# vpc-ccg/circminer

Measured on AMD Instinct MI355X. Metric: paired reads/sec (whole node), hg38 k=20, 2x150 bp; circ_report bit-exact, higher is better.
Workload: dtype int32/u8 (chain scores f64)

## Files before the change

### circminer_amd/csrc/cm_core.h

```cpp
#pragma once
#include <stdint.h>

#include "circminer_hot.h"
#if defined(CM_STAGE2_HOST)
#include <vector>
#endif

#if defined(__HIPCC__)
#define CM_HD __host__ __device__
#define CM_NOINLINE inline
#else
#define CM_HD
#define CM_NOINLINE
#endif

#if !defined(CM_HOOK_DP)
#define CM_HOOK_DP(kind, s, n, t, m) ((void)0)
#endif
#if defined(CM_STATS) && !defined(__HIPCC__)
#if !defined(CM_NSTATS)
#define CM_NSTATS 16
#endif
extern "C" unsigned long long cm_stats[CM_NSTATS];
#define CM_STAT(i, n) ((i) < CM_NSTATS ? (void)(cm_stats[(i) < CM_NSTATS ? (i) : 0] += (unsigned long long)(n)) : (void)0)
// ... 310 lines not shown
        beg = (int)A.iv_bucket[b];
        end = (int)A.iv_bucket[b + 1];
        if (beg > 0) --beg;
        if (end < (int)A.n_iv) ++end;
        if (end <= beg) end = beg + 1;
    }
    while (end - beg > 1) {
        const int mid = (beg + end) / 2;
        if (pos < A.iv[mid].spos) end = mid;
        else beg = mid;
    }
    ind = end - 1;
    if (ind < 0 || A.iv[ind].epos < pos) return -1;
    return ind;
}
CM_HD inline int overlap_ind(const Core &c, uint32_t loc, int &ind) {
    int r = iv_find_ind(c.A, loc, ind);
    if (r < 0 || iv_nseg(c.A, r) == 0) return -1;
    return r;
}
CM_HD inline int overlap(const Core &c, uint32_t loc) { int ind; return overlap_ind(c, loc, ind); }

CM_HD inline uint32_t upper_bound_lookup(const Core &c, uint32_t spos, uint32_t mlen, uint32_t rlen, uint32_t &max_end, int &ol) {
    const AnnotV &A = c.A;
    max_end = 0;
    int it_ind = -1;
    int ov = iv_find_ind(A, spos, it_ind);
    const uint32_t epos = spos + mlen - 1;
    if (ov < 0 || iv_nseg(A, ov) == 0) {
        ol = -1;
        int nx = it_ind + 1;
        max_end = ((nx < 0 || nx >= (int)A.n_iv) ? 0u : A.iv[nx].spos) - 1u;
        if (max_end < epos) return 0;
        return cmin(spos + rlen + (uint32_t)c.P.max_ed, max_end - mlen + 1);
    }
    ol = -1;
    uint32_t min_end = 1000000000u, max_next = 0;
    if (epos > A.iv[ov].epos) {
        const uint32_t n = iv_nseg(A, ov);
        for (uint32_t i = 0; i < n; ++i) {
            uint32_t s = iv_segid(A, ov, i);
            uint32_t e = A.seg[s].end;
            if (e >= epos) {
                max_end = cmax(max_end, e);
                min_end = cmin(min_end, e);
                max_next = cmax(max_next, A.seg[s].next_exon_beg);
            }
        }
    } else {
        max_end = A.iv[ov].max_end;
        min_end = A.iv[ov].min_end;
        max_next = A.iv[ov].max_next_exon;
    }
    if (max_end > 0 && max_end >= epos) {
        ol = ov;
        if (min_end < rlen + epos && max_next != 0) return max_next + mlen - 1;
        return max_end - mlen + 1;
    }
    max_end = 0;
    ol = -1;
    return 0;
}
CM_HD inline uint32_t upper_bound(const Core &c, uint32_t spos, uint32_t mlen, uint32_t rlen, uint32_t &max_end, int &ol) {
    if (bit_at(c.A.near_border_bits, c.A.n_bits, spos)) return upper_bound_lookup(c, spos, mlen, rlen, max_end, ol);
    max_end = 0;
    ol = -1;
    return spos + rlen + (uint32_t)c.P.max_ed;
}
CM_HD inline int chr_row(const Core &c, uint32_t loc) {
    uint32_t i;
    for (i = 1; i < c.A.n_chr; ++i)
        if (loc < c.A.chr_shift[i]) return (int)i - 1;
    return (int)i - 1;
}

struct Event { double score; uint32_t cell; uint32_t pad; };
struct ChainWork {
    CM_G double *dp_score;
    CM_G int32_t *dp_prev;
    CM_G uint8_t *pool;
    unsigned long long pool_bytes;
    CM_G unsigned long long *pool_cursor;
    g_err err;
};

#if defined(__HIP_DEVICE_COMPILE__)
CM_HD inline unsigned long long pool_take(CM_G unsigned long long *cur, unsigned long long n) { return atomicAdd((unsigned long long *)cur, n); }
CM_HD inline void flag_err(g_err e, int bits) { atomicOr((int *)e, bits); }
#else
inline unsigned long long pool_take(unsigned long long *cur, unsigned long long n) { return __sync_fetch_and_add(cur, n); }
inline void flag_err(int *e, int bits) { __sync_fetch_and_or(e, bits); }
#endif

CM_HD inline bool check_junction(const Core &c, uint32_t s1, uint32_t s2, int ol, int kmer, int read_dist, int &trans_dist) {
    trans_dist = INF_I;
    if (ol < 0) return false;
    const uint32_t e1 = s1 + kmer - 1;
    if (s2 <= e1) return false;
    int td2intron = -1;
    const AnnotV &A = c.A;
    const uint32_t n = iv_nseg(A, ol);
    for (uint32_t i = 0; i < n; ++i) {
        const uint32_t s = iv_segid(A, ol, i);
        const int e12end = (int)(A.seg[s].end - e1);
        const int beg2s2 = (int)(s2 - A.seg[s].next_exon_beg);
        if (e12end >= 0 && e12end < read_dist && beg2s2 + kmer < 0) td2intron = (int)(s2 - e1 - 1);
        if (e12end < 0 || beg2s2 < 0) continue;
        trans_dist = e12end + beg2s2;
        if (cabs(trans_dist - read_dist) <= c.P.max_ed) return true;
    }
    if (td2intron != -1) {
        trans_dist = td2intron;
        return true;
    }
    trans_dist = INF_I;
    return false;
}

constexpr int SMALL_W = 32;
struct ChainStoreGlobal {
    ChainWork &w;
    g_u32 POS;
    const uint32_t *start;
    const uint32_t *cnt_;
    const uint32_t *base_;
    uint32_t lb_[MAX_SEEDS];
    CM_G Event *ev;
    uint32_t n_ev, cap_ev;
    bool lost;
    static constexpr uint32_t MASK_CELLS = 128;
    uint64_t imp0_, imp1_;
    bool masked_;
    double init_;
    CM_HD ChainStoreGlobal(ChainWork &ww, g_u32 pos, const uint32_t *st, const uint32_t *cn, const uint32_t *bs)
        : w(ww), POS(pos), start(st), cnt_(cn), base_(bs), ev(nullptr), n_ev(0), cap_ev(0), lost(false), imp0_(0), imp1_(0), masked_(false), init_(0) {}
    CM_HD inline bool stored(uint32_t x) const { return !masked_ || (((x < 64u ? imp0_ : imp1_) >> (x & 63u)) & 1ull); }
    CM_HD inline uint32_t cnt(int s) const { return cnt_[s]; }
    CM_HD inline uint32_t base(int s) const { return base_[s]; }
    CM_HD inline uint32_t total(int kc) const { return base_[kc]; }
    CM_HD inline void lb_reset(int kc) { for (int k = 0; k < kc; ++k) lb_[k] = 0; }
    CM_HD inline uint32_t lb(int s) const { return lb_[s]; }
    CM_HD inline void set_lb(int s, uint32_t v) { lb_[s] = v; }
    CM_HD inline void init(uint32_t n_cells, double v) {
        masked_ = n_cells <= MASK_CELLS;
        init_ = v;
        imp0_ = imp1_ = 0;
        if (masked_) return;
        for (uint32_t x = 0; x < n_cells; ++x) {
            w.dp_score[x] = v;
            w.dp_prev[x] = -1;
        }
    }
    CM_HD inline uint32_t pos(int s, uint32_t i) const { return POS[start[s] + i]; }
    CM_HD inline double score(uint32_t x) const { return stored(x) ? w.dp_score[x] : init_; }
    CM_HD inline int32_t prev(uint32_t x) const { return stored(x) ? w.dp_prev[x] : -1; }
    CM_HD inline void set(uint32_t x, double sc, int32_t pv) {
        w.dp_score[x] = sc;
        w.dp_prev[x] = pv;
        if (masked_) {
            if (x < 64u) imp0_ |= 1ull << x;
            else imp1_ |= 1ull << (x & 63u);
        }
    }
    CM_HD inline void push(double sc, uint32_t cell) {
        if (n_ev == cap_ev && !lost) {
            const uint32_t ncap = cap_ev ? cap_ev * 4u : 32u;
            const unsigned long long bytes = (unsigned long long)ncap * sizeof(Event);
            const unsigned long long off = pool_take(w.pool_cursor, bytes);
            if (off + bytes > w.pool_bytes) {
                lost = true;
                flag_err(w.err, ERR_POOL);
            } else {
                CM_G Event *ne = (CM_G Event *)(w.pool + off);
                for (uint32_t q = 0; q < n_ev; ++q) ne[q] = ev[q];
                ev = ne;
                cap_ev = ncap;
            }
        }
        if (n_ev < cap_ev) {
            ev[n_ev].score = sc;
            ev[n_ev].cell = cell;
            ++n_ev;
        }
    }
    CM_HD inline uint32_t n_events() const { return n_ev; }
    CM_HD inline double ev_score(uint32_t q) const { return ev[q].score; }
    CM_HD inline uint32_t ev_cell(uint32_t q) const { return ev[q].cell; }
};
struct ChainStoreSmall {
    double sc[SMALL_W + 2];
    int32_t pv[SMALL_W + 2];
    uint32_t hp[SMALL_W + 2];
    double es[SMALL_W];
    uint32_t ec[SMALL_W];
    const uint32_t *cnt_;
    const uint32_t *base_;
    uint32_t lb_[MAX_SEEDS];
    uint32_t n_ev;
    CM_HD ChainStoreSmall(g_u32 POS, const uint32_t *start, const uint32_t *cn, const uint32_t *bs, int kc) : cnt_(cn), base_(bs), n_ev(0) {
        for (int s = 0; s < kc; ++s)
            for (uint32_t i = 0; i < cn[s]; ++i) hp[bs[s] + i] = POS[start[s] + i];
    }
    CM_HD inline uint32_t cnt(int s) const { return cnt_[s]; }
    CM_HD inline uint32_t base(int s) const { return base_[s]; }
    CM_HD inline uint32_t total(int kc) const { return base_[kc]; }
    CM_HD inline void lb_reset(int kc) { for (int k = 0; k < kc; ++k) lb_[k] = 0; }
    CM_HD inline uint32_t lb(int s) const { return lb_[s]; }
    CM_HD inline void set_lb(int s, uint32_t v) { lb_[s] = v; }
    CM_HD inline void init(uint32_t n_cells, double v) {
        for (uint32_t x = 0; x < n_cells; ++x) {
            sc[x] = v;
            pv[x] = -1;
        }
    }
    CM_HD inline uint32_t pos(int s, uint32_t i) const { return hp[base_[s] + i]; }
    CM_HD inline double score(uint32_t x) const { return sc[x]; }
    CM_HD inline int32_t prev(uint32_t x) const { return pv[x]; }
    CM_HD inline void set(uint32_t x, double v, int32_t p) {
        sc[x] = v;
        pv[x] = p;
    }
    CM_HD inline void push(double v, uint32_t cell) {
        if (n_ev < (uint32_t)SMALL_W) {
            es[n_ev] = v;
            ec[n_ev] = cell;
            ++n_ev;
        }
    }
    CM_HD inline uint32_t n_events() const { return n_ev; }
    CM_HD inline double ev_score(uint32_t q) const { return es[q]; }
    CM_HD inline uint32_t ev_cell(uint32_t q) const { return ec[q]; }
};

template <class ST>
CM_HD inline int chain_kbest_t(const Core &c, int seq_len, int kc, ST &S, CM_G cm_chain *out) {
    const int kmer = c.P.kmer;
    const uint32_t max_best = (uint32_t)c.P.max_chain_len;
    S.init(S.total(kc), (double)kmer);
    uint32_t max_exon_end = 0;
    int ol = -1;

    for (int ii = kc - 2; ii >= 0; --ii) {
        const uint32_t read_remain = (uint32_t)(seq_len - ii * kmer - kmer);
        S.lb_reset(kc);
        const uint32_t cnt_ii = S.cnt(ii), base_ii = S.base(ii);
        for (uint32_t i = 0; i < cnt_ii; ++i) {
            const int32_t cur_info = (int32_t)S.pos(ii, i);
            const uint32_t seg_start = (uint32_t)cur_info, seg_end = (uint32_t)cur_info + kmer - 1;
            uint32_t max_lpos_lim = MAXUB;
            double my_score = S.score(base_ii + i);
            for (int jj = ii + 1; jj < kc; ++jj) {
                const uint32_t pcn = S.cnt(jj);
                uint32_t lb = S.lb(jj);
                if (pcn == 0 || lb >= pcn) continue;
// ... 1957 lines not shown
```

### circminer_amd/csrc/cm_heavy_pipe.h

```cpp

struct HPair {
    cm_mapped_read mr;
    uint32_t t;
    uint32_t task_off, unp_off;
    uint32_t fp, bp, fun, bun;
    int32_t ntask, exf, exb;
    int32_t min_ret1, min_ret2;
    int16_t len1, len2, nf, nb, nfu, nbu;
    int8_t st, first, over, a, g1, g2, gf, gb, do_f, do_b, pad[2];
};
struct HTask { uint32_t h, e; };
struct HUnp { uint32_t h, x; };
enum { HC_TASKS = 0, HC_Q1 = 1, HC_Q1CUR = 2, HC_UNP = 3, HC_Q2 = 4, HC_Q2CUR = 5, HC_LIST2 = 6, HC_FALL = 7, HC_CUR = 8 , HC_WORDS = 16 };
struct HPipe {
    HPair *hp;
    uint32_t *list2, *fall;
    HTask *T;
    cmc::PreDP *pre;
    uint32_t *q;
    HRes *res;
    HUnp *U;
    cmc::PreDP *pre2;
    uint32_t *q2;
    unsigned int *ctr;
// ... 425 lines not shown
        hp.do_f = do_f ? 1 : 0;
        hp.do_b = do_b ? 1 : 0;
        hp.fun = fun;
        hp.bun = bun;
        hp.nfu = (int16_t)nfu;
        hp.nbu = (int16_t)nbu;
        hp.unp_off = off;
        hp.exf = 99;
        hp.exb = 99;
        hp.gf = 0;
        hp.gb = 0;
    }
}

__global__ void __launch_bounds__(BLK_PAIR, 8) k_hp_unp_req(KCore kc, ReadsDev rd, uint64_t pair0, int attempt, const cm_chain *chains, HPipe P, int str_cap) {
    const int lane = threadIdx.x;
    const Core c = cmc::to_core(kc);
    cmc::DpMem sm{cmc::LBuf{nullptr, str_cap}, cmc::LBuf{nullptr, str_cap}, nullptr};
    const cmc::Ext ext(c, sm);
    const int kmer = c.P.kmer;
    const unsigned int n_unp = P.ctr[HC_UNP] < P.unp_cap ? P.ctr[HC_UNP] : P.unp_cap;
    const unsigned int n_req = 2u * n_unp;
    auto take = [&]() { return (unsigned int)__shfl((int)(lane == 0 ? atomicAdd(&P.ctr[HC_CUR + 2], 64u) : 0u), 0); };
    for (unsigned int r0 = take(); r0 < n_req; r0 = take()) {
        const unsigned int r = r0 + (unsigned int)lane;
        cmc::SV sv{}, tv{};
        int n = 0, m = 0;
        bool have = false, in_range = false;
        if (r < n_req) {
            const HUnp u = P.U[r >> 1];
            if (u.h != 0xffffffffu) {
                in_range = true;
                const HPair &hp = P.hp[u.h];
                const HReadsOf R = hp_reads(rd, pair0, hp.t, (attempt == 0) == (hp.first != 0));
                const bool back = (u.x >> 8) & 1u;
                const int ci = (int)(u.x & 0xFFu);
                const cmc::g_chain chp = (cmc::g_chain)(chains + (uint64_t)(back ? R.bset : R.fset) * CM_BESTCHAINLIM) + ci;
                const cmc::Read rdv{back ? R.bseq : R.fseq, back ? R.blen : R.flen, back ? 1 : 0};
                have = hp_side_views(ext, chp, rdv, (r & 1u) != 0u, kmer, sv, n, tv, m);
            }
        }
        hp_answer_or_queue(sm, in_range, have, sv, n, tv, m, P.pre2 + r, r, P.q2, &P.ctr[HC_Q2], lane);
    }
}
__global__ void __launch_bounds__(BLK_PAIR, CM_PAIR_WAVES) k_hp_unp(KCore kc, ReadsDev rd, uint64_t pair0, int attempt, const cm_chain *chains, HPipe P,
                                                                     uint32_t *pair_err, int str_cap) {
    extern __shared__ uint32_t lds_words[];
    const int lane = threadIdx.x;
    cmc::DpMem sm = lane_dp_mem((CM_S uint8_t *)lds_words, lane, str_cap, nullptr);
    const Core c = cmc::to_core(kc);
    const cmc::Ext ext(c, sm);
    const int kmer = c.P.kmer;
    const unsigned int n_unp = P.ctr[HC_UNP] < P.unp_cap ? P.ctr[HC_UNP] : P.unp_cap;
    auto take = [&]() { return (unsigned int)__shfl((int)(lane == 0 ? atomicAdd(&P.ctr[HC_CUR + 3], 64u) : 0u), 0); };
    for (unsigned int x0 = take(); x0 < n_unp; x0 = take()) {
        const unsigned int x = x0 + (unsigned int)lane;
        if (x >= n_unp) continue;
        const HUnp u = P.U[x];
        if (u.h == 0xffffffffu) continue;
        HPair &hp = P.hp[u.h];
        const HReadsOf R = hp_reads(rd, pair0, hp.t, (attempt == 0) == (hp.first != 0));
        const bool back = (u.x >> 8) & 1u;
        const int ci = (int)(u.x & 0xFFu), k = (int)(u.x >> 16);
        const cmc::CH ch{(cmc::g_chain)(chains + (uint64_t)(back ? R.bset : R.fset) * CM_BESTCHAINLIM) + ci, kmer};
        const cmc::Read frd{R.fseq, R.flen, 0}, brd{R.bseq, R.blen, 1};
        cmc::MM m = cmc::mm_init(c);
        sm.err = (cmc::g_err)(pair_err + hp.t);
        sm.pre = (cmc::g_pre)(P.pre2 + (size_t)x * 2);
        sm.n_pre = 2;
        const int ex = ext.chain_both_sides(ch, back ? brd : frd, m, back ? -1 : 1);
        sm.pre = nullptr;
        sm.n_pre = 0;
        atomicMin(back ? &hp.exb : &hp.exf, ex);
        if (k == 0) {
            cmc::overlap_to_spos(c, m);
            cmc::overlap_to_epos(c, m);
            (back ? hp.gb : hp.gf) = (int8_t)((m.exons_spos >= 0) || (m.exons_epos >= 0));
        }
    }
}

__global__ void __launch_bounds__(BLK_PAIR, 8) k_hp_finish(KCore kc, uint64_t pair0, const uint32_t *lst, const unsigned int *n_lst_p, const unsigned int *n_heavy_p,
                                                          int attempt, HPipe P, cm_mapped_read *state, uint8_t *active, int32_t *cat, int is_last,
                                                          unsigned long long *counters, RetryArgs ra, const int32_t *nchain, int second_to_fall) {
    const Core c = cmc::to_core(kc);
    const unsigned int n_items = attempt == 0 ? *n_heavy_p : *n_lst_p;
    const unsigned int x = blockIdx.x * BLK_PAIR + threadIdx.x;
#if defined(CM_HP_DIAG)
    if (x == 0) {
        unsigned long long *o = counters + CN_HP_ATTEMPT + CN_HP_STRIDE * attempt;
        atomicAdd(&o[0], (unsigned long long)n_items);
        atomicAdd(&o[1], (unsigned long long)P.ctr[HC_TASKS]);
        atomicAdd(&o[2], (unsigned long long)P.ctr[HC_UNP]);
        atomicAdd(&o[3], (unsigned long long)P.ctr[HC_Q1]);
        atomicAdd(&o[4], (unsigned long long)P.ctr[HC_Q2]);
        atomicAdd(&o[5], (unsigned long long)*P.fall_ctr);
    }
#endif
    for (unsigned int y = x; y < n_items; y += gridDim.x * BLK_PAIR) {
        const uint32_t h = attempt == 0 ? y : lst[y];
        HPair &hp = P.hp[h];
        if (hp.over) {
            active[pair0 + hp.t] = 1;
            continue;
        }
        cm_mapped_read mr = hp.mr;
        int st = hp.st;
        if (st < 0) {
            int a = hp.a;
            if (a < 0) {
                int min_ret1 = hp.min_ret1, min_ret2 = hp.min_ret2, g1 = hp.g1, g2 = hp.g2;
                if (hp.do_f) {
                    min_ret1 = hp.exf < min_ret1 ? hp.exf : min_ret1;
                    g1 = hp.gf;
                }
                if (hp.do_b) {
                    min_ret2 = hp.exb < min_ret2 ? hp.exb : min_ret2;
                    g2 = hp.gb;
                }
                cmc::mr_update_type(mr, cmc::leftover_type(min_ret1, min_ret2, g1 != 0, g2 != 0));
                a = mr.type;
            }
            if (c.P.scan_level == 0 && a == CM_CONCRD) st = CM_CONCRD;
            if (st < 0 && attempt == 0) {
                const bool r1_fwd2 = hp.first == 0;
                const uint32_t fs = hp.t * 4u + (r1_fwd2 ? 0u : 2u), bs = hp.t * 4u + (r1_fwd2 ? 3u : 1u);
                if (nchain[fs] == 0 && nchain[bs] == 0) {
                    const bool decided = mr.type == CM_CONCRD || mr.type == CM_DISCRD || mr.type == CM_CHIORF || mr.type == CM_CHIBSJ || mr.type == CM_CHI2BSJ;
                    if (!decided && cmc::leftovers_matter(mr.type, CM_ORPHAN, false, CM_ORPHAN, false))
                        cmc::mr_update_type(mr, cmc::leftover_type(CM_ORPHAN, CM_ORPHAN, false, false));
                    st = (c.P.scan_level == 0 && mr.type == CM_CONCRD) ? CM_CONCRD : mr.type;
                } else if (second_to_fall) {
                    P.fall[atomicAdd(P.fall_ctr, 1u)] = hp.t;
                    hp_count_fall(counters, 0);
                    active[pair0 + hp.t] = 1;
                    continue;
                } else {
                    hp.mr = mr;
                    P.list2[atomicAdd(&P.ctr[HC_LIST2], 1u)] = h;
                    continue;
                }
            }
            if (st < 0) st = mr.type;
        }
        const uint32_t t = hp.t;
        const uint64_t p = pair0 + t;
        if (__hip_atomic_load(ra.pair_err + t, __ATOMIC_RELAXED, __HIP_MEMORY_SCOPE_AGENT) != 0u) {
            ra.list[atomicAdd(ra.count, 1u)] = t;
            active[p] = 1;
        } else {
            uint8_t act = 1;
            cmc::finish_round(c, st, is_last, hp.len1, hp.len2, mr, act);
            state[p] = mr;
            active[p] = act;
            cat[p] = st;
            atomicAdd(&counters[CN_PAIR_ROUNDS], 1ull);
        }
    }
}
__global__ void k_hp_reset(unsigned int *ctr) {
    if (threadIdx.x < HC_WORDS && threadIdx.x != HC_LIST2 && threadIdx.x != HC_FALL) ctr[threadIdx.x] = 0u;
}
```

### circminer_amd/csrc/cm_hot.hip

```cpp
#include <chrono>
#include <hip/hip_runtime.h>
#include <rocprim/device/device_radix_sort.hpp>

#include <algorithm>
#include <atomic>
#include <cstdarg>
#include <cstdio>
#include <cstdlib>
#include <cstring>
#include <string>
#include <functional>
#include <thread>
#include <vector>

#include "circminer_hot.h"
#include "cm_core.h"
#include "cm_aos.h"
#include "cm_index_build.h"
#include "cm_fastq_text.h"
#include "cm_pam_text.h"
#include "cm_remain_order.h"
#include "cm_remain_text.h"
#include "cm_sam_text.h"

using cmc::Core;
using cmc::KCore;

namespace {

constexpr int MAX_SLOTS = 16;
constexpr uint32_t TILE_PAIRS = 1u << 20;
constexpr uint32_t TILE_PAIRS_MAX = 1u << 21;
constexpr int BLK = 256;
constexpr int BLK_CHAIN = 64;
#include "cm_dp_engine.h"

enum ProfClass { PC_NONE = -1, PC_SEED = 0, PC_CHAIN = 1, PC_PAIR = 2, PC_SCAN = 3, PC_HEAVY = 4, PC_ORDER = 5, PC_CHAIN_HEAVY = 6, PC_PREFETCH = 7,
                 PC_ROWS = 7 , PC_COUNT = 8 };
enum Counter {
    CN_PROBES = 0 , CN_PAIR_ROUNDS = 3, CN_RERUN = 4 ,
    CN_FALL = 5, CN_FALL_2ND = 6,
    CN_DEAD_CHAINS = 7,
    CN_CD_LANE = 8, CN_CD_PHASE = 13, CN_CD_WAVE = 16, CN_CD_EVENTS = 20, CN_CD_LEVELS = 21, CN_CD_PROBLEMS = 22, CN_CD_PASSES = 23, CN_CD_CELLS = 24,
    CN_CD_REGLOG = 25, CN_CD_BATCHES = 26, CN_CD_PRE_USED = 27, CN_CD_PRE_UNUSED = 28,
    CN_HP_ATTEMPT = 8, CN_HP_STRIDE = 8, CN_HP_UNPAIRED = 24, CN_HP_CHAINS = 25, CN_HP_SEQ_TASKS = 26, CN_HP_EARLY = 27, CN_HP_EARLY_FIRST = 28,
    CN_WORDS = 32
};
static_assert(CN_CD_CELLS < CN_WORDS && CN_HP_EARLY_FIRST < CN_WORDS && CN_HP_ATTEMPT + CN_HP_STRIDE + 5 < CN_HP_UNPAIRED, "d_counters has CN_WORDS words");
enum Pin {
    PIN_COLLECT_N = 0, PIN_COLLECT_ERR = 1,
    PIN_DEV_ERR = 0,
    PIN_POOL_ERR = 2,
    PIN_HEAVY_LOAD = 4,
    PIN_CELLS = 8,
    PIN_RERUN_N = 12, PIN_FALL_N = 14,
    PIN_TEXT = 16,
    PIN_ROWS = 26,
    PIN_TIES = 28,
    PIN_WORDS = 32
};
constexpr size_t PIN_BYTES = PIN_WORDS * sizeof(unsigned long long);
static_assert(PIN_BYTES == 256 && PIN_FALL_N + 1 < PIN_TEXT && PIN_CELLS + 3 < PIN_RERUN_N && PIN_TEXT + cmft::RES_WORDS <= PIN_ROWS && PIN_ROWS + 1 < PIN_TIES && PIN_TIES + 1 < PIN_WORDS,
              "the landing zone has 32 words");
struct ReadsDev {
    const uint8_t *seq1, *seq2;
    const uint64_t *off1, *off2;
};

__global__ void __launch_bounds__(BLK) k_seed(KCore kc, ReadsDev rd, const uint8_t *active, uint64_t pair0, uint32_t n_tile, int S,
                                              uint32_t *sstart, uint32_t *scnt, uint32_t *sraw, unsigned long long *counters) {
    const Core c = cmc::to_core(kc);
    __shared__ unsigned int sh[3];
    if (threadIdx.x < 3) sh[threadIdx.x] = 0;
    __syncthreads();
    const uint64_t q = (uint64_t)blockIdx.x * BLK + threadIdx.x;
    const uint64_t total = (uint64_t)n_tile * 4u * (uint64_t)S;
    const bool in = q < total;
    const uint64_t qc = in ? q : total - 1;
    uint32_t s;
    uint64_t r;
    if ((total >> 32) == 0) {
        s = (uint32_t)qc % (uint32_t)S;
        r = (uint32_t)qc / (uint32_t)S;
    } else {
        s = (uint32_t)(qc % (uint64_t)S);
        r = qc / (uint64_t)S;
    }
    const int orient = (int)(r & 1u), mate = (int)((r >> 1) & 1u);
    const uint64_t p = pair0 + (r >> 2);
    const uint8_t act = active[p];
    uint64_t o[2];
    __builtin_memcpy(o, (mate ? rd.off2 : rd.off1) + p, sizeof(o));
    const int len = (int)(o[1] - o[0]);
    const int k = c.P.kmer;
    uint32_t st = 0, cn = 0, rw = 0, pt = 0;
    if ((int)in & (int)(act != 0) & (int)((int)(s + 1) * k <= len)) {
        const cmc::Read R{(cmc::g_u8)((mate ? rd.seq2 : rd.seq1) + o[0]), len, orient};
        const cmc::Probe pr = cmc::seed_probe(c, R.view(), (int)s * k);
        st = pr.start;
        rw = pr.raw;
        cn = (pr.raw > (uint32_t)c.P.seed_lim) ? 0u : pr.raw;
        pt = 0x10000u | pr.touches;
    }
    if (in) {
        sstart[q] = st;
        scnt[q] = cn;
        sraw[q] = rw;
    }
    uint32_t a = pt, b = cn;
#define CM_ROW_ADD(v, n) v += (uint32_t)__builtin_amdgcn_update_dpp(0, (int)v, 0x120 | (n), 0xF, 0xF, false)
    CM_ROW_ADD(a, 1); CM_ROW_ADD(b, 1);
    CM_ROW_ADD(a, 2); CM_ROW_ADD(b, 2);
    CM_ROW_ADD(a, 4); CM_ROW_ADD(b, 4);
    CM_ROW_ADD(a, 8); CM_ROW_ADD(b, 8);
#undef CM_ROW_ADD
    uint32_t wa = 0, wb = 0;
#pragma unroll
    for (int row = 0; row < 4; ++row) {
        wa += (uint32_t)__builtin_amdgcn_readlane((int)a, 16 * row);
        wb += (uint32_t)__builtin_amdgcn_readlane((int)b, 16 * row);
    }
    if ((threadIdx.x & 63u) == 0 && wa) {
        atomicAdd(&sh[0], wa >> 16);
        atomicAdd(&sh[1], wa & 0xFFFFu);
        if (wb) atomicAdd(&sh[2], wb);
    }
    __syncthreads();
    if (threadIdx.x < 3 && sh[threadIdx.x]) atomicAdd(&counters[CN_PROBES + threadIdx.x], (unsigned long long)sh[threadIdx.x]);
}

constexpr int SCAN_T = 256;
constexpr int SCAN_ELEMS = 1024;
constexpr int CHAIN_CLS_NONE = -2;
constexpr int CHAIN_CLS_DEAD = -3;
__device__ inline bool quad_dead(uint32_t cells) {
    const uint32_t mate = cells + (uint32_t)__shfl_xor((int)cells, 1);
    const uint32_t other = (uint32_t)__shfl_xor((int)mate, 2);
    return cells > 0 && other == 0;
}
static_assert(SCAN_T % 4 == 0 && SCAN_ELEMS % SCAN_T == 0 && BLK % 4 == 0, "a pair's four problems are one aligned quad of lanes in k_scan_a and k_chain_cls");
__global__ void __launch_bounds__(SCAN_T) k_scan_a(const uint32_t *scnt, int S, uint32_t n, unsigned long long *out, unsigned long long *bsum,
                                                   unsigned int *bmax, int skip_dead) {
    __shared__ unsigned long long sh[SCAN_T];
    __shared__ unsigned int shmax;
    const uint32_t base = blockIdx.x * SCAN_ELEMS;
    unsigned long long run = 0;
    unsigned int my_max = 0;
    if (threadIdx.x == 0) shmax = 0;
#pragma unroll
    for (int k = 0; k < SCAN_ELEMS / SCAN_T; ++k) {
        const uint32_t r = base + k * SCAN_T + threadIdx.x;
        uint32_t c = 0;
        if (r < n)
            for (int s = 0; s < S; ++s) c += scnt[(uint64_t)r * S + s];
        if (skip_dead && quad_dead(c)) c = 0;
        my_max = c > my_max ? c : my_max;
        sh[threadIdx.x] = c;
        __syncthreads();
        for (int d = 1; d < SCAN_T; d <<= 1) {
            const unsigned long long x = (threadIdx.x >= (unsigned)d) ? sh[threadIdx.x - d] : 0ull;
            __syncthreads();
            sh[threadIdx.x] += x;
            __syncthreads();
        }
        if (r < n) out[r] = run + sh[threadIdx.x] - c;
        run += sh[SCAN_T - 1];
        __syncthreads();
    }
    atomicMax(&shmax, my_max);
    __syncthreads();
    if (threadIdx.x == 0) {
        bsum[blockIdx.x] = run;
        bmax[blockIdx.x] = shmax;
    }
}
template <class T, bool WITH_MAX>
__global__ void __launch_bounds__(1024) k_scan_mid(T *bsum, uint32_t nb, T *total, const unsigned int *bmax) {
    __shared__ T part[1024];
    __shared__ unsigned int gmax;
    const uint32_t t = threadIdx.x;
    const uint32_t chunk = (nb + 1023u) / 1024u;
    const uint32_t a = t * chunk, b = (a + chunk < nb) ? a + chunk : nb;
    T s = 0;
    unsigned int m = 0;
    if (WITH_MAX && t == 0) gmax = 0;
    if constexpr (WITH_MAX) __syncthreads();
    for (uint32_t i = a; i < b; ++i) {
        s += bsum[i];
        if constexpr (WITH_MAX) m = bmax[i] > m ? bmax[i] : m;
    }
    if constexpr (WITH_MAX) atomicMax(&gmax, m);
    part[t] = s;
    __syncthreads();
    for (uint32_t d = 1; d < 1024; d <<= 1) {
        const T v = (t >= d) ? part[t - d] : (T)0;
        __syncthreads();
        part[t] += v;
        __syncthreads();
    }
    T run = t ? part[t - 1] : (T)0;
    for (uint32_t i = a; i < b; ++i) {
        const T x = bsum[i];
        bsum[i] = run;
        run += x;
    }
    if (WITH_MAX && t == 1023) {
        total[0] = part[1023];
        total[1] = gmax;
    }
}
__global__ void __launch_bounds__(SCAN_T) k_scan_c(unsigned long long *out, const unsigned long long *bsum, uint32_t n) {
    const uint32_t i = blockIdx.x * SCAN_T + threadIdx.x;
    if (i < n) out[i] += bsum[i / SCAN_ELEMS];
}

__device__ inline int pack_resid(int left, int right) {
    left = left < 0 ? 0 : (left > 255 ? 255 : left);
    right = right < 0 ? 0 : (right > 255 ? 255 : right);
    return left | (right << 8);
}
#ifndef CM_CHAIN_WAVES
#define CM_CHAIN_WAVES 5
#endif
__global__ void __launch_bounds__(BLK_CHAIN, CM_CHAIN_WAVES) k_chain(KCore kc, ReadsDev rd, const uint8_t *active, uint64_t pair0, uint32_t r0, uint32_t r1, int S,
                                                     const uint32_t *sstart, const uint32_t *scnt, const uint32_t *sraw,
                                                     const unsigned long long *celloff, unsigned long long cellbase, double *dp_score,
                                                     int32_t *dp_prev, uint8_t *pool, unsigned long long pool_bytes,
                                                     unsigned long long *pool_cursor, cm_chain *chains, int32_t *nchain, int32_t *high, int *err,
                                                     uint16_t *resid, const uint32_t *perm, const unsigned int *perm_lo, const unsigned int *perm_hi,
                                                     const int8_t *cls) {
    uint32_t r = r0 + blockIdx.x * BLK_CHAIN + threadIdx.x;
    if (perm) {
        r += *perm_lo;
        if (r >= *perm_hi) return;
        r = perm[r];
    } else if (r >= r1 || (cls && cls[r] == CHAIN_CLS_DEAD)) return;
    const Core c = cmc::to_core(kc);
    const uint64_t p = pair0 + (r >> 2);
    int n = 0, hh = 0, rs = 0;
    if (active[p]) {
        const int mate = (int)((r >> 1) & 1u);
        const uint64_t o0 = mate ? rd.off2[p] : rd.off1[p], o1 = mate ? rd.off2[p + 1] : rd.off1[p + 1];
        const int len = (int)(o1 - o0);
        uint32_t st[cmc::MAX_SEEDS], cn[cmc::MAX_SEEDS];
        for (int s = 0; s < S; ++s) {
            st[s] = sstart[(uint64_t)r * S + s];
            cn[s] = scnt[(uint64_t)r * S + s];
            if (sraw[(uint64_t)r * S + s] > 0 && cn[s] == 0) ++hh;
        }
        cmc::ChainWork w;
        w.dp_score = (CM_G double *)(dp_score + (celloff[r] - cellbase));
        w.dp_prev = (CM_G int32_t *)(dp_prev + (celloff[r] - cellbase));
        w.pool = (CM_G uint8_t *)pool;
        w.pool_bytes = pool_bytes;
        w.pool_cursor = (CM_G unsigned long long *)pool_cursor;
        w.err = (cmc::g_err)err;
        n = cmc::chain_kbest(c, len, S, st, cn, w, (CM_G cm_chain *)(chains + (uint64_t)r * CM_BESTCHAINLIM));
        if (n > 0) {
            const cm_chain &b = chains[(uint64_t)r * CM_BESTCHAINLIM];
            rs = pack_resid(b.qpos[0], len - (b.qpos[b.chain_len - 1] + c.P.kmer));
        }
    }
    nchain[r] = n;
    high[r] = hh;
    resid[r] = (uint16_t)rs;
}

struct RetryArgs {
    uint32_t *pair_err;
    uint32_t *list;
    unsigned int *count;
    cmc::MemoSpill *spill;
    int spill_cap;
    int first;
};

template <bool FIRST>
__device__ __forceinline__ void pair_kernel(const KCore &kc, const ReadsDev &rd, uint64_t pair0, uint32_t n_tile, const cm_chain *chains, const int32_t *nchain,
                                            const int32_t *high, cm_mapped_read *state, uint8_t *active, int32_t *cat, int is_last,
                                            int *err, unsigned long long *counters, int str_cap, unsigned long long *lane_clk,
                                            const uint32_t *perm, const unsigned int *n_light, unsigned int *next_chunk,
                                            const RetryArgs &ra) {
    const unsigned long long clk0 = lane_clk ? wall_clock64() : 0ull;
    extern __shared__ uint32_t lds_words[];
#if defined(CM_DIAG)
    __shared__ unsigned long long tick_w[65];
    cmc::Tick tick;
    for (int i = 0; i < 32; ++i) tick.acc[i] = 0;
    tick.last = wall_clock64();
    tick.w = (CM_L unsigned long long *)tick_w;
    tick.wave_on = 1;
    for (int i = threadIdx.x; i < 65; i += BLK_PAIR) tick_w[i] = i == 0 ? tick.last : 0ull;
    __syncthreads();
    cmc::DpMem sm = lane_dp_mem((CM_S uint8_t *)lds_words, threadIdx.x, str_cap, (cmc::g_err)err, &tick);
#else
    cmc::DpMem sm = lane_dp_mem((CM_S uint8_t *)lds_words, threadIdx.x, str_cap, (cmc::g_err)err);
#endif
    if (ra.spill) {
        sm.spill = (cmc::g_spill)(ra.spill + ((size_t)blockIdx.x * BLK_PAIR + threadIdx.x) * (size_t)ra.spill_cap);
        sm.spill_cap = ra.spill_cap;
    }
    const Core c = cmc::to_core(kc);
    const uint32_t n_l = *n_light;
    auto take = [&]() { return (uint32_t)__shfl((int)(threadIdx.x == 0 ? atomicAdd(next_chunk, 1u) : 0u), 0); };
    for (uint32_t chunk = take(); (uint64_t)chunk * BLK_PAIR < n_l; chunk = take()) {
    const uint32_t slot = chunk * BLK_PAIR + threadIdx.x;
    if (slot >= n_l) continue;
    const unsigned long long it0 = lane_clk ? wall_clock64() : 0ull;
    const uint32_t t = perm[slot];
    const uint64_t p = pair0 + t;
    const uint64_t a0 = rd.off1[p], a1 = rd.off1[p + 1], b0 = rd.off2[p], b1 = rd.off2[p + 1];
    cmc::ChainSet sets[4];
    int hh[4];
    for (int x = 0; x < 4; ++x) {
        const uint64_t r = (uint64_t)t * 4 + x;
        sets[x].ch = (cmc::g_chain)(chains + r * CM_BESTCHAINLIM);
        sets[x].n = nchain[r];
        hh[x] = high[r];
    }
    cm_mapped_read mr = state[p];
#if defined(CM_AB_GLOBAL_ERR)
    int *perr = err;
#else
    int *perr = FIRST ? (int *)(ra.pair_err + t) : err;
    sm.err = (cmc::g_err)perr;
#endif
    const int st = cmc::process_read(c, sm, (cmc::g_u8)(rd.seq1 + a0), (int)(a1 - a0), (cmc::g_u8)(rd.seq2 + b0), (int)(b1 - b0), sets, hh, mr, (cmc::g_err)perr);
    bool keep = true;
    if (FIRST) {
        if (__hip_atomic_load(ra.pair_err + t, __ATOMIC_RELAXED, __HIP_MEMORY_SCOPE_AGENT) != 0u) {
            ra.list[atomicAdd(ra.count, 1u)] = t;
            active[pair0 + t] = 1;
            keep = false;
        }
    } else ra.pair_err[t] = 0u;
    if (keep) {
        uint8_t act = 1;
        cmc::finish_round(c, st, is_last, (int)(a1 - a0), (int)(b1 - b0), mr, act);
        state[p] = mr;
        active[p] = act;
        cat[p] = st;
    }
    {
        const unsigned long long m = __ballot(1), mk = __ballot(keep);
        if ((threadIdx.x & 63) == (unsigned)__ffsll((long long)m) - 1 && mk) {
            atomicAdd(&counters[CN_PAIR_ROUNDS], (unsigned long long)__popcll(mk));
            if (!FIRST) atomicAdd(&counters[CN_RERUN], (unsigned long long)__popcll(mk));
        }
    }
#if defined(CM_DIAG)
    CM_TICK(sm, 13);
    if (lane_clk) {
        for (int i = 0; i < 15; ++i) lane_clk[p * 16 + i] = tick.acc[i];
        lane_clk[p * 16 + 15] = wall_clock64() - clk0;
        const unsigned long long m = __ballot(1);
        if ((threadIdx.x & 63) == (unsigned)__ffsll((long long)m) - 1) {
            unsigned long long *wr = lane_clk + (unsigned long long)n_tile * 16 + (unsigned long long)blockIdx.x * 64;
            for (int i = 0; i < 64; ++i) wr[i] = tick_w[1 + i];
        }
    }
#else
    if (lane_clk) lane_clk[slot] = ((wall_clock64() - it0) & 0xFFFFFFFFull) | ((unsigned long long)t << 32);
#endif
    }
}


__global__ void __launch_bounds__(BLK_PAIR, CM_PAIR_WAVES) k_pair(KCore kc, ReadsDev rd, uint64_t pair0, uint32_t n_tile, const cm_chain *chains, const int32_t *nchain,
                                                   const int32_t *high, cm_mapped_read *state, uint8_t *active, int32_t *cat, int is_last,
                                                   int *err, unsigned long long *counters, int str_cap, unsigned long long *lane_clk,
                                                   const uint32_t *perm, const unsigned int *n_light, unsigned int *next_chunk,
                                                   RetryArgs ra) {
    pair_kernel<true>(kc, rd, pair0, n_tile, chains, nchain, high, state, active, cat, is_last, err, counters, str_cap, lane_clk, perm, n_light, next_chunk, ra);
}
__global__ void __launch_bounds__(BLK_PAIR, CM_PAIR_WAVES) k_pair_rerun(KCore kc, ReadsDev rd, uint64_t pair0, uint32_t n_tile, const cm_chain *chains,
                                                         const int32_t *nchain, const int32_t *high, cm_mapped_read *state, uint8_t *active, int32_t *cat,
                                                         int is_last, int *err, unsigned long long *counters, int str_cap,
                                                         unsigned long long *lane_clk, const uint32_t *perm, const unsigned int *n_light,
                                                         unsigned int *next_chunk, RetryArgs ra) {
    pair_kernel<false>(kc, rd, pair0, n_tile, chains, nchain, high, state, active, cat, is_last, err, counters, str_cap, lane_clk, perm, n_light, next_chunk, ra);
}

template <class T> __device__ inline T wave_excl_scan(T v, int lane, T &total) {
    T x = v;
    for (int o = 1; o < 64; o <<= 1) {
        const T y = __shfl_up(x, o);
        if (lane >= o) x += y;
    }
    total = __shfl(x, 63);
    return x - v;
}
#ifndef CM_CHEAVY_LOG_REGS
#define CM_CHEAVY_LOG_REGS 4
#endif
struct HeavyChainCtx {
#if defined(CM_CHAIN_DIAG)
    unsigned long long *tk;
#endif
    const Core *c;
    CM_L const uint32_t *LP;
    CM_L const uint32_t *NB;
    CM_L const uint32_t *IM;
    const uint32_t *base, *cnt;
    int kc, seq_len;
    CM_G double *dps;
    CM_G int32_t *dpp;
};
__device__ inline uint32_t heavy_im_word(uint32_t base_s, uint32_t s) { return 2u * ((base_s >> 6) + s); }
__host__ __device__ inline uint32_t heavy_im_words(uint32_t ncell, uint32_t kc) { return 2u * ((ncell >> 6) + kc + 1u); }
__device__ inline uint32_t heavy_cell(const HeavyChainCtx &h, int ii, uint32_t i, CM_G cmc::Event *ev, double &out_score, int32_t &out_prev,
                                     double &e0, double &e1) {
    const Core &c = *h.c;
    const int kmer = c.P.kmer;
    const uint32_t read_remain = (uint32_t)(h.seq_len - ii * kmer - kmer);
    const int32_t cur_info = (int32_t)h.LP[h.base[ii] + i];
    const uint32_t seg_start = (uint32_t)cur_info, seg_end = (uint32_t)cur_info + kmer - 1;
    uint32_t max_lpos_lim = cmc::MAXUB, max_exon_end = 0;
    int ol = -1;
    double my_score = (double)kmer;
    int32_t my_prev = -1;
    uint32_t n = 0;
    const uint32_t cell = h.base[ii] + i;
    const bool near = (h.NB[cell >> 5] >> (cell & 31)) & 1u;
    uint2 parked = make_uint2(0u, 0u);
    int parked_ol = -1;
    if (near) {
        parked = *(CM_G const uint2 *)(h.dps + cell);
        parked_ol = h.dpp[cell];
    }
#if defined(CM_CHAIN_DIAG)
    if (!ev) h.tk[3] += 1;
#define CD_T0 const unsigned long long cd_t = wall_clock64()
#define CD_ADD(k) h.tk[k] += wall_clock64() - cd_t
#else
#define CD_T0
#define CD_ADD(k)
#endif
    const uint32_t own_lim = seg_start + read_remain + (uint32_t)c.P.max_ed;
    for (int j0 = ii + 1; j0 < h.kc; j0 += 4) {
    uint32_t g_lo[4];
    double g_sc[4];
    bool g_ok[4];
#if defined(CM_CHAIN_DIAG)
    bool g_ld[4];
#endif
#pragma unroll
    for (int g = 0; g < 4; ++g) {
// ... 36 lines not shown
        const int jj = j0 + g;
        const uint32_t pcn = h.cnt[jj];
        CM_L const uint32_t *pp = h.LP + h.base[jj];
        CM_L const uint32_t *im = h.IM + heavy_im_word(h.base[jj], (uint32_t)jj);
        const uint32_t lo = g_lo[g];
#if defined(CM_CHAIN_DIAG)
        bool g_used = false;
#endif
        if (max_lpos_lim == cmc::MAXUB) {
            CD_T0;
            if (near) {
                max_lpos_lim = parked.x;
                max_exon_end = parked.y;
                ol = parked_ol;
            } else {
                max_exon_end = 0;
                ol = -1;
                max_lpos_lim = seg_start + read_remain + (uint32_t)c.P.max_ed;
            }
            CD_ADD(1);
        }
        const int distr = (jj - ii) * kmer - kmer;
        CD_T0;
        for (uint32_t j = lo; j < pcn && pp[j] <= max_lpos_lim; ++j) {
#if defined(CM_CHAIN_DIAG)
            if (!ev) h.tk[4] += 1;
#endif
            const uint32_t pinfo = pp[j];
            int genome_dist, distt, trans_dist;
            if (max_exon_end == 0 || (pinfo + kmer - 1) <= max_exon_end) genome_dist = (int)(pinfo - seg_end - 1);
            else genome_dist = cmc::INF_I;
            if (cmc::cabs(genome_dist - distr) <= c.P.max_ed) distt = genome_dist;
            else if (cmc::check_junction(c, seg_start, pinfo, ol, kmer, distr, trans_dist)) distt = trans_dist;
            else continue;
            const int maxd = distr < distt ? distt : distr, mind = distr < distt ? distr : distt;
            const double beta = 0.1 * (double)(maxd - mind);
            const double alpha = 2e4 * (double)kmer;
            const double prev_score = j == lo ? g_sc[g] : ((im[j >> 5] >> (j & 31)) & 1u) ? h.dps[h.base[jj] + j] : (double)kmer;
#if defined(CM_CHAIN_DIAG)
            if (j == lo) g_used = true;
#endif
            const double t1 = prev_score + alpha;
            const double temp_score = t1 - beta;
            if (temp_score > my_score) {
                my_score = temp_score;
                my_prev = (int32_t)(((uint32_t)jj << 16) | j);
                if (ev) {
                    ev[n].score = temp_score;
                    ev[n].cell = ((uint32_t)ii << 16) | i;
                }
                e1 = n == 1 ? temp_score : e1;
                e0 = n == 0 ? temp_score : e0;
                ++n;
            }
        }
        CD_ADD(2);
#if defined(CM_CHAIN_DIAG)
        if (!ev && g_ld[g]) h.tk[g_used ? 5 : 6] += 1;
#endif
    }
    }
    out_score = my_score;
    out_prev = my_prev;
    return n;
}

struct HeavyBackTrack {
    uint32_t base[cmc::MAX_SEEDS + 1];
    uint32_t cand[CM_BESTCHAINLIM + 2];
    uint16_t cidx[CM_BESTCHAINLIM][CM_MAX_CHAIN_FRAGS];
    uint8_t cbl[CM_BESTCHAINLIM][CM_MAX_CHAIN_FRAGS];
    uint8_t clen[CM_BESTCHAINLIM + 2];
    uint8_t emit[CM_BESTCHAINLIM + 2];
    uint32_t rep[CM_BESTCHAINLIM * (CM_MAX_CHAIN_FRAGS - 1)];
};

#ifndef CM_CHEAVY_WAVES
#define CM_CHEAVY_WAVES 3
#endif
__global__ void __launch_bounds__(64, CM_CHEAVY_WAVES) k_chain_heavy(KCore kc_, ReadsDev rd, uint64_t pair0, int S, const uint32_t *sstart, const uint32_t *scnt,
                                                    const unsigned long long *celloff, double *dp_score, int32_t *dp_prev, uint8_t *pool,
                                                    unsigned long long pool_bytes, unsigned long long *pool_cursor, cm_chain *chains, int32_t *nchain,
                                                    int *err, uint16_t *resid, const uint32_t *perm, const unsigned int *n_perm, unsigned int *next_problem,
                                                    unsigned long long *counters) {
    extern __shared__ uint32_t lds_words[];
    CM_L uint32_t *LP = (CM_L uint32_t *)lds_words;
    __shared__ HeavyBackTrack BT;
    const int lane = threadIdx.x;
    const Core c = cmc::to_core(kc_);
    const int kmer = c.P.kmer;
    const uint32_t max_best = (uint32_t)c.P.max_chain_len;
    const unsigned int n_heavy = *n_perm;
    auto take_raw = [&]() { return lane == 0 ? atomicAdd(next_problem, 1u) : 0u; };
    uint32_t nx_r = 0, nx_st = 0, nx_cn = 0;
    unsigned long long nx_coff = 0, nx_o0 = 0, nx_o1 = 0;
    auto ask_header = [&](uint32_t rr) {
        nx_st = lane < S ? sstart[(uint64_t)rr * S + lane] : 0u;
        nx_cn = lane < S ? scnt[(uint64_t)rr * S + lane] : 0u;
        nx_coff = celloff[rr];
        const uint64_t pp = pair0 + (rr >> 2);
        const uint64_t *of = ((rr >> 1) & 1u) ? rd.off2 : rd.off1;
        nx_o0 = of[pp];
        nx_o1 = of[pp + 1];
    };
    unsigned int hidx = (unsigned int)__builtin_amdgcn_readfirstlane((int)take_raw());
    if (hidx < n_heavy) {
        nx_r = perm[hidx];
        ask_header(nx_r);
    }
    while (hidx < n_heavy) {
        const uint32_t r = (uint32_t)__builtin_amdgcn_readfirstlane((int)nx_r);
        const unsigned int nx_raw = take_raw();
        const int len = __builtin_amdgcn_readfirstlane((int)(nx_o1 - nx_o0));
        const unsigned long long coff = ((unsigned long long)(uint32_t)__builtin_amdgcn_readfirstlane((int)(nx_coff >> 32)) << 32) |
                                        (unsigned long long)(uint32_t)__builtin_amdgcn_readfirstlane((int)nx_coff);
#if defined(CM_CHAIN_DIAG)
        const unsigned long long dg0 = wall_clock64();
#endif
        uint32_t st[cmc::MAX_SEEDS], cn[cmc::MAX_SEEDS], base[cmc::MAX_SEEDS + 1];
        int kc = S;
#pragma unroll
        for (int s = 0; s < cmc::MAX_SEEDS; ++s) {
            st[s] = (uint32_t)__builtin_amdgcn_readlane((int)nx_st, s);
            cn[s] = (uint32_t)__builtin_amdgcn_readlane((int)nx_cn, s);
        }
        while (kc >= 1 && cn[kc - 1] == 0) --kc;
        base[0] = 0;
        for (int s = 0; s < kc; ++s) base[s + 1] = base[s] + cn[s];
        const uint32_t ncell = base[kc];
        CM_G double *dps = (CM_G double *)(dp_score + coff);
        CM_G int32_t *dpp = (CM_G int32_t *)(dp_prev + coff);
        CM_L uint32_t *NB = LP + ncell;
        CM_L uint16_t *Q = (CM_L uint16_t *)(NB + 2 * ((ncell + 63) >> 6));
        CM_L uint32_t *IM = (CM_L uint32_t *)(Q + 320);
        const bool by_entry = c.entry_near != nullptr;
        for (int s = 0; s < kc; ++s)
            for (uint32_t i = lane; i < cn[s]; i += 64) {
                const uint32_t e = st[s] + i;
                uint32_t v = c.X.pos[e];
                if (by_entry && s < kc - 1) v |= (uint32_t)((c.entry_near[e >> 6] >> (e & 63)) & 1ull) << 31;
                LP[base[s] + i] = v;
            }
        for (uint32_t x = lane; x < heavy_im_words(ncell, (uint32_t)kc); x += 64) IM[x] = 0u;
        __threadfence_block();
        __syncthreads();
        {
            const uint32_t n_pre = kc >= 1 ? base[kc - 1] : 0u;
            const unsigned long long lt = (1ull << lane) - 1ull;
            uint32_t qn = 0;
            auto look_up = [&](uint32_t cnt) {
                if ((uint32_t)lane < cnt) {
                    const uint32_t x = Q[lane];
                    int ii = 0;
                    for (int s = 1; s < kc; ++s) ii += x >= base[s] ? 1 : 0;
                    const uint32_t read_remain = (uint32_t)(len - ii * kmer - kmer);
                    uint32_t mx = 0;
                    int ol = -1;
                    const uint32_t lim = cmc::upper_bound_lookup(c, LP[x], (uint32_t)kmer, read_remain, mx, ol);
                    *(CM_G uint2 *)(dps + x) = make_uint2(lim, mx);
                    dpp[x] = ol;
                }
            };
            for (uint32_t x0 = 0; x0 < n_pre; x0 += 256) {
                bool nr[4];
#pragma unroll
                for (int u = 0; u < 4; ++u) {
                    const uint32_t x = x0 + 64 * u + lane;
                    if (by_entry) {
                        nr[u] = x < n_pre && (LP[x] >> 31);
                        if (nr[u]) LP[x] &= 0x7fffffffu;
                    } else nr[u] = x < n_pre && cmc::bit_at(c.A.near_border_bits, c.A.n_bits, LP[x]);
                }
#pragma unroll
                for (int u = 0; u < 4; ++u) {
                    const uint32_t xb = x0 + 64 * u;
                    if (xb >= n_pre) break;
                    const unsigned long long m = __ballot(nr[u]);
                    if (lane == 0) NB[xb >> 5] = (uint32_t)m;
                    if (lane == 32) NB[(xb >> 5) + 1] = (uint32_t)(m >> 32);
                    if (nr[u]) Q[qn + __popcll(m & lt)] = (uint16_t)(xb + lane);
                    qn += (uint32_t)__popcll(m);
                }
                __syncthreads();
                while (qn >= 64) {
                    look_up(64);
                    uint16_t keep[4];
#pragma unroll
                    for (int u = 0; u < 4; ++u) keep[u] = 64u * u + (uint32_t)lane < qn - 64 ? Q[64 + 64 * u + lane] : (uint16_t)0;
                    __syncthreads();
#pragma unroll
                    for (int u = 0; u < 4; ++u)
                        if (64u * u + (uint32_t)lane < qn - 64) Q[64 * u + lane] = keep[u];
                    qn -= 64;
                    __syncthreads();
                }
            }
            if (qn) look_up(qn);
        }
        __threadfence_block();
        __syncthreads();
#if defined(CM_CHAIN_DIAG)
        const unsigned long long dg1 = wall_clock64();
#endif
#if defined(CM_CHAIN_DIAG)
        unsigned long long tk[7] = {0, 0, 0, 0, 0, 0, 0};
        unsigned long long wv[4] = {0, 0, 0, 0};
        HeavyChainCtx H{tk, &c, LP, NB, IM, base, cn, kc, len, dps, dpp};
#else
        HeavyChainCtx H{&c, LP, NB, IM, base, cn, kc, len, dps, dpp};
#endif
        const unsigned int hnext = (unsigned int)__builtin_amdgcn_readfirstlane((int)nx_raw);
        if (hnext < n_heavy) nx_r = perm[hnext];
        CM_G cmc::Event *ev = nullptr;
        uint32_t n_ev = 0, cap_ev = 0;
        bool lost = false;
        double lane_best = -1.0;
        for (int ii = kc - 2; ii >= 0; --ii) {
            for (uint32_t i0 = 0; i0 < cn[ii]; i0 += 64) {
                const uint32_t i = i0 + lane;
                const bool on = i < cn[ii];
                double sc = 0, e0 = 0, e1 = 0;
                int32_t pv = -1;
#if defined(CM_CHAIN_DIAG)
                const unsigned long long w0 = wall_clock64();
#endif
                const uint32_t mine = on ? heavy_cell(H, ii, i, (CM_G cmc::Event *)nullptr, sc, pv, e0, e1) : 0u;
#if defined(CM_CHAIN_DIAG)
                const unsigned long long w1 = wall_clock64();
#endif
                {
                    const unsigned long long m = __ballot(mine > 0u);
                    const uint32_t w = heavy_im_word(base[ii], (uint32_t)ii) + (i0 >> 5);
                    if (lane == 0) IM[w] = (uint32_t)m;
                    if (lane == 32) IM[w + 1] = (uint32_t)(m >> 32);
                }
                uint32_t total;
                const uint32_t off = wave_excl_scan(mine, lane, total);
                if (n_ev + total > cap_ev && !lost) {
                    uint32_t ncap = cap_ev ? cap_ev : 256u;
                    while (ncap < n_ev + total) ncap *= 4u;
                    const unsigned long long bytes = (unsigned long long)ncap * sizeof(cmc::Event);
                    unsigned long long o = 0;
                    if (lane == 0) o = atomicAdd(pool_cursor, bytes);
                    o = ((unsigned long long)__shfl((unsigned int)(o >> 32), 0) << 32) | (unsigned long long)__shfl((unsigned int)o, 0);
                    if (o + bytes > pool_bytes) {
                        lost = true;
                        if (lane == 0) atomicOr(err, cmc::ERR_POOL);
                    } else {
                        CM_G cmc::Event *ne = (CM_G cmc::Event *)((CM_G uint8_t *)pool + o);
                        for (uint32_t q = lane; q < n_ev; q += 64) ne[q] = ev[q];
                        ev = ne;
                        cap_ev = ncap;
                    }
                }
                if (on && mine) {
                    if (!lost) {
                        CM_G cmc::Event *dst = ev + n_ev + off;
                        if (mine <= 2) {
                            dst[0].score = e0;
                            dst[0].cell = ((uint32_t)ii << 16) | i;
                            if (mine == 2) {
                                dst[1].score = e1;
                                dst[1].cell = ((uint32_t)ii << 16) | i;
                            }
                        } else heavy_cell(H, ii, i, dst, sc, pv, e0, e1);
                    }
                    dps[base[ii] + i] = sc;
                    dpp[base[ii] + i] = pv;
                    lane_best = sc > lane_best ? sc : lane_best;
                }
                if (!lost) n_ev += total;
#if defined(CM_CHAIN_DIAG)
                const unsigned long long w3 = wall_clock64();
                wv[0] += w1 - w0;
                wv[2] += w3 - w1;
#endif
            }
#if defined(CM_CHAIN_DIAG)
            const unsigned long long w4 = wall_clock64();
#endif
            __threadfence_block();
            __syncthreads();
#if defined(CM_CHAIN_DIAG)
            wv[3] += wall_clock64() - w4;
#endif
        }
#if defined(CM_CHAIN_DIAG)
        for (int k = 0; k < 5; ++k) atomicAdd(&counters[CN_CD_LANE + k], tk[k]);
        atomicAdd(&counters[CN_CD_PRE_USED], tk[5]);
        atomicAdd(&counters[CN_CD_PRE_UNUSED], tk[6]);
        if (lane == 0)
            for (int k = 0; k < 4; ++k) atomicAdd(&counters[CN_CD_WAVE + k], wv[k]);
#endif
        CM_G cm_chain *out = (CM_G cm_chain *)(chains + (uint64_t)r * CM_BESTCHAINLIM);
        uint32_t best_count = 0;
        int first_q0 = 0, first_qlast = 0;
        if (lane <= kc) BT.base[lane] = base[lane];
        __threadfence_block();
        __syncthreads();
#if defined(CM_CHAIN_DIAG)
        const unsigned long long dg2 = wall_clock64();
#endif
        if (hnext < n_heavy) ask_header((uint32_t)__builtin_amdgcn_readfirstlane((int)nx_r));
        if (n_ev > 0) {
            constexpr int LR = CM_CHEAVY_LOG_REGS;
            constexpr uint32_t CAP = CM_BESTCHAINLIM;
            const unsigned long long lt = (1ull << lane) - 1ull;
            double best_score = lane_best;
            for (int o = 32; o >= 1; o >>= 1) {
                const double u = __shfl_xor(best_score, o);
                best_score = u > best_score ? u : best_score;
            }
            const bool in_regs = n_ev <= 64u * (uint32_t)LR;
            const int n_u = (int)((n_ev + 63u) >> 6);
            double es[LR];
            uint32_t ec[LR];
#pragma unroll
            for (int u = 0; u < LR; ++u) {
                es[u] = -1.0;
                ec[u] = 0u;
                const uint32_t q = (uint32_t)lane + 64u * (uint32_t)u;
                if (in_regs && q < n_ev) {
                    const cmc::Event e = ev[q];
                    es[u] = e.score;
                    ec[u] = e.cell;
                }
            }
            double cur = best_score;
            bool have = true;
            uint32_t n_rep = 0;
// ... 177 lines not shown
            int rs = 0;
            if (best_count > 0) rs = pack_resid(first_q0, len - (first_qlast + kmer));
            resid[r] = (uint16_t)rs;
#if defined(CM_CHAIN_DIAG)
            const unsigned long long dg3 = wall_clock64();
            atomicAdd(&counters[CN_CD_PHASE + 0], dg1 - dg0);
            atomicAdd(&counters[CN_CD_PHASE + 1], dg2 - dg1);
            atomicAdd(&counters[CN_CD_PHASE + 2], dg3 - dg2);
#endif
        }
        __syncthreads();
        hidx = hnext;
    }
}

constexpr int HEAVY_COST = 6;
constexpr int N_BUCKETS = 7;
constexpr int HEAVY_CLS = 15;
__device__ inline int pair_class(const Core &c, const cm_chain *chains, const uint16_t *resid4, const int32_t *nchain,
                                 const uint8_t *active, uint64_t pair0, uint32_t t, int heavy_cost, int *sub) {
    const uint64_t p = pair0 + t;
    if (sub) *sub = 0;
    if (!active[p]) return -2;
    const int32_t *nc = nchain + 4 * (uint64_t)t;
    const int a = nc[0], b = nc[1], cc = nc[2], d = nc[3];
    if ((a + b) > 0 && (cc + d) > 0 && (a * d + cc * b + a + b + cc + d) > heavy_cost) {
        if (sub) {
            const int cost = a * d + cc * b + a + b + cc + d;
            const int lv = cost <= 12 ? 0 : cost <= 16 ? 1 : cost <= 24 ? 2 : cost <= 32 ? 3 : cost <= 48 ? 4 : cost <= 64 ? 5 : cost <= 96 ? 6 : cost <= 128 ? 7
                           : cost <= 192 ? 8 : cost <= 256 ? 9 : cost <= 384 ? 10 : cost <= 512 ? 11 : cost <= 768 ? 12 : 13;
            *sub = lv << 4;
        }
        return HEAVY_CLS;
    }
    if ((a + b) <= 0 || (cc + d) <= 0) return 0;
    const uint16_t *q = resid4 + 4 * (uint64_t)t;
    int resid = 0;
    for (int x = 0; x < 4; ++x) resid += (q[x] & 0xff) + (q[x] >> 8);
    if (sub) {
        const bool main0 = a > 0 && d > 0;
        const uint16_t f = q[main0 ? 0 : 2], bk = q[main0 ? 3 : 1];
        *sub = ((f & 0xff) ? 1 : 0) | ((f >> 8) ? 2 : 0) | ((bk & 0xff) ? 4 : 0) | ((bk >> 8) ? 8 : 0);
        int mx = f & 0xff;
        mx = (f >> 8) > mx ? (f >> 8) : mx;
        mx = (bk & 0xff) > mx ? (bk & 0xff) : mx;
        mx = (bk >> 8) > mx ? (bk >> 8) : mx;
        const int lv = mx < 5 ? 0 : mx < 10 ? 1 : mx < 15 ? 2 : mx < 20 ? 3 : mx < 25 ? 4 : mx < 30 ? 5 : mx < 40 ? 6 : mx < 50 ? 7 : mx < 60 ? 8 : mx < 70 ? 9
                       : mx < 80 ? 10 : mx < 90 ? 11 : mx < 100 ? 12 : mx < 115 ? 13 : mx < 130 ? 14 : 15;
        *sub |= lv << 4;
    }
    const int bucket = resid < 25 ? 0 : resid < 50 ? 1 : resid < 100 ? 2 : resid < 150 ? 3 : resid < 200 ? 4 : resid < 300 ? 5 : 6;
    bool genic = false;
    for (int x = 0; x < 4 && !genic; ++x) {
        if (nc[x] <= 0) continue;
        genic = cmc::overlap(c, chains[((uint64_t)t * 4 + x) * CM_BESTCHAINLIM].rpos[0]) >= 0;
    }
    return (genic ? N_BUCKETS : 0) + bucket;
}
constexpr int CHAIN_LIGHT_CLS = 12;
constexpr int CLS_T = 1024;
constexpr int CLS_W = 256;
constexpr int CLS_REP = CLS_T / CLS_W;
constexpr int N_CLS = 16;
constexpr int CTR_SUM = 16, CTR_BASE = 32, CTR_WORDS = 64;
constexpr int CTR_NEXT = 48;
constexpr int CTR_RETRY = 50;
constexpr int CTR_CHAIN_NEXT = 48;
static_assert(CTR_CHAIN_NEXT >= CTR_BASE + N_CLS && CTR_CHAIN_NEXT < CTR_WORDS && CTR_NEXT >= CTR_BASE + N_CLS && CTR_RETRY + 1 < CTR_WORDS, "spare words");
constexpr unsigned HEAVY_GRID_MAX = 4096;
constexpr int RETRY_GRID = 8;
constexpr int RETRY_SPILL = 2040;
__device__ inline void block_class_ranks(int k, unsigned int (*wcnt)[N_CLS], unsigned int &rank_in_wave, int lane, int wave) {
    rank_in_wave = 0;
#pragma unroll
    for (int c = 0; c < N_CLS; ++c) {
        const unsigned long long m = __ballot(k == c);
        if (lane == 0) wcnt[wave][c] = (unsigned int)__popcll(m);
        if (k == c) rank_in_wave = (unsigned int)__popcll(m & ((1ull << lane) - 1ull));
    }
}
constexpr int HEAVY_COST_WIDE = 16;
constexpr unsigned long long HEAVY_LOAD = 16;
__global__ void __launch_bounds__(BLK) k_pair_cost(const int32_t *nchain, const uint8_t *active, uint64_t pair0, uint32_t n_tile, int base_cost,
                                                  unsigned long long *sum) {
    __shared__ unsigned long long sh[BLK / 64];
    const uint32_t t = blockIdx.x * BLK + threadIdx.x;
    unsigned long long v = 0;
    if (t < n_tile && active[pair0 + t]) {
        const int32_t *nc = nchain + 4 * (uint64_t)t;
        const int a = nc[0], b = nc[1], cc = nc[2], d = nc[3];
        const int cost = a * d + cc * b + a + b + cc + d;
        if ((a + b) > 0 && (cc + d) > 0 && cost > base_cost) v = (unsigned long long)cost;
    }
    for (int o = 32; o >= 1; o >>= 1) v += __shfl_xor(v, o);
    if ((threadIdx.x & 63) == 0) sh[threadIdx.x >> 6] = v;
    __syncthreads();
    if (threadIdx.x == 0) {
        unsigned long long s2 = 0;
        for (int w = 0; w < BLK / 64; ++w) s2 += sh[w];
        if (s2) atomicAdd(sum, s2);
    }
}
__global__ void __launch_bounds__(BLK) k_pair_cls(KCore kc, const cm_chain *chains, const uint16_t *resid, const int32_t *nchain,
                                                 const uint8_t *active, uint64_t pair0, uint32_t n_tile, int8_t *cls, int32_t *cat, int heavy_cost,
                                                 int8_t *cls_sub, int8_t *cls_sub2, uint8_t *act_out, const unsigned long long *heavy_load) {
    const uint32_t t = blockIdx.x * BLK + threadIdx.x;
    if (t >= n_tile) return;
    const Core c = cmc::to_core(kc);
    if (heavy_load && *heavy_load > HEAVY_LOAD * (unsigned long long)n_tile) heavy_cost = HEAVY_COST_WIDE;
    int sub = 0;
    const int k = pair_class(c, chains, resid, nchain, active, pair0, t, heavy_cost, &sub);
    cls[t] = (int8_t)k;
    cls_sub[t] = (int8_t)(k < 0 ? -2 : (k == HEAVY_CLS ? 0 : (sub & 15)));
    cls_sub2[t] = (int8_t)(k < 0 ? -2 : (sub >> 4));
    if (k == -2) {
        cat[pair0 + t] = -1;
        act_out[pair0 + t] = 0;
    }
}
__global__ void __launch_bounds__(BLK) k_chain_cls(const uint32_t *scnt, const uint32_t *sraw, int S, uint32_t n_prob, int8_t *cls, int32_t *high,
                                                  unsigned long long light_w, unsigned int light_cells, int32_t *nchain, uint16_t *resid,
                                                  cm_chain *chains, const uint8_t *active, uint64_t pair0, int skip_dead,
                                                  unsigned long long *counters) {
    __shared__ unsigned int n_dead;
    const uint32_t r = blockIdx.x * BLK + threadIdx.x;
    if (threadIdx.x == 0) n_dead = 0;
    __syncthreads();
    const bool on = r < n_prob && active[pair0 + (r >> 2)];
    if (r < n_prob && !on) {
        high[r] = 0;
        if (nchain) {
            nchain[r] = 0;
            resid[r] = 0;
        }
        cls[r] = CHAIN_CLS_NONE;
    }
    unsigned long long w = 0, suffix = 0;
    int hh = 0;
    if (on)
        for (int s = S - 1; s >= 0; --s) {
            const unsigned long long c = scnt[(uint64_t)r * S + s];
            w += c * suffix;
            suffix += c;
            if (sraw[(uint64_t)r * S + s] > 0 && c == 0) ++hh;
        }
    const bool dead = skip_dead && quad_dead((uint32_t)suffix);
    if (skip_dead) {
        const unsigned long long md = __ballot(dead);
        if ((threadIdx.x & 63) == 0 && md) atomicAdd(&n_dead, (unsigned int)__popcll(md));
        __syncthreads();
        if (threadIdx.x == 0 && n_dead) atomicAdd(&counters[CN_DEAD_CHAINS], (unsigned long long)n_dead);
    }
    if (!on) return;
    high[r] = hh;
    if ((suffix == 0 || dead) && nchain) {
        nchain[r] = dead ? 1 : 0;
        resid[r] = 0;
        if (dead) chains[(uint64_t)r * CM_BESTCHAINLIM].chain_len = 0;
    }
    const bool light = w <= light_w && suffix <= light_cells;
    const unsigned int n = (unsigned int)suffix;
    cls[r] = (int8_t)(suffix == 0 ? CHAIN_CLS_NONE
                      : dead ? CHAIN_CLS_DEAD
                      : light ? (n <= 3 ? 0 : n <= 6 ? 1 : n <= 7 ? 2 : n <= 9 ? 3 : n <= 12 ? 4 : n <= 16 ? 5 : n <= 24 ? 6 : n <= 32 ? 7 : n <= 48 ? 8 : n <= 64 ? 9
                                 : n <= 96 ? 10 : 11)
                      : w <= 4096 ? 12 : w <= 65536 ? 13 : w <= 1048576 ? 14 : 15);
}
__global__ void __launch_bounds__(BLK) k_chain_apply(uint32_t n_prob, const int8_t *cls, const int32_t *thigh, int32_t *high, int32_t *nchain, uint16_t *resid,
                                                    cm_chain *chains) {
    const uint32_t r = blockIdx.x * BLK + threadIdx.x;
    if (r >= n_prob) return;
    high[r] = thigh[r];
    const int k = cls[r];
    if (k == CHAIN_CLS_NONE || k == CHAIN_CLS_DEAD) {
        nchain[r] = k == CHAIN_CLS_DEAD ? 1 : 0;
        resid[r] = 0;
        if (k == CHAIN_CLS_DEAD) chains[(uint64_t)r * CM_BESTCHAINLIM].chain_len = 0;
    }
}
__global__ void __launch_bounds__(CLS_W) k_cls_hist(const int8_t *cls, uint32_t n, unsigned int *blk_cnt, uint32_t nb, const uint32_t *order,
                                                    const unsigned int *n_order) {
    __shared__ unsigned int wcnt[CLS_T / 64][N_CLS];
    const uint32_t lim = n_order ? (*n_order < n || order ? *n_order : n) : n;
    const int lane = threadIdx.x & 63, wave = threadIdx.x >> 6;
// ... 350 lines not shown
                else {
                    const uint32_t fun = ~s.fp & (s.nf >= 32 ? 0xffffffffu : ((1u << s.nf) - 1u));
                    const uint32_t bun = ~s.bp & (s.nb >= 32 ? 0xffffffffu : ((1u << s.nb) - 1u));
                    do_f = min_ret1 != CM_CONCRD && fun != 0;
                    do_b = min_ret2 != CM_CONCRD && bun != 0;
                    if (!cmc::leftovers_matter(mr.type, min_ret1, do_f, min_ret2, do_b)) a = mr.type;
                    else {
                        s.fun = fun;
                        s.bun = bun;
                        s.nfu = (int16_t)(do_f ? __popc(fun) : 0);
                        s.nbu = (int16_t)(do_b ? __popc(bun) : 0);
                        s.exf = 99;
                        s.exb = 99;
                        s.gf = 0;
                        s.gb = 0;
                    }
                }
            }
            __syncthreads();
            pre[0] = 0;
#pragma unroll
            for (int g = 0; g < HG; ++g) pre[g + 1] = pre[g] + S[g].nfu + S[g].nbu;
            for (int x = lane; x < pre[HG]; x += 64) {
                int g, u;
                locate(pre, x, g, u);
                CM_L HSlot &s = S[g];
                const bool back = u >= s.nfu;
                const int k = back ? u - s.nfu : u;
                const int ci = nth_set_bit(back ? s.bun : s.fun, k);
                const cmc::CH ch{(back ? slot_bch(s, chains) : slot_fch(s, chains)) + ci, kmer};
                const cmc::Read frd{s.fseq, s.flen, 0}, brd{s.bseq, s.blen, 1};
                cmc::MM m = cmc::mm_init(c);
                sm.err = slot_perr(s, ra.pair_err);
                const int ex = ext.chain_both_sides(ch, back ? brd : frd, m, back ? -1 : 1);
                atomicMin((int *)(back ? &s.exb : &s.exf), ex);
                if (k == 0) {
                    cmc::overlap_to_spos(c, m);
                    cmc::overlap_to_epos(c, m);
                    (back ? s.gb : s.gf) = (int8_t)((m.exons_spos >= 0) || (m.exons_epos >= 0));
                }
            }
            __syncthreads();
            CM_TICK(sm, 15);
            if (on) {
                if (a < 0) {
                    CM_L HSlot &s = S[lane];
                    if (do_f) {
                        min_ret1 = s.exf < min_ret1 ? s.exf : min_ret1;
                        g1 = s.gf;
                    }
                    if (do_b) {
                        min_ret2 = s.exb < min_ret2 ? s.exb : min_ret2;
                        g2 = s.gb;
                    }
                    cmc::mr_update_type(mr, cmc::leftover_type(min_ret1, min_ret2, g1 != 0, g2 != 0));
                    a = mr.type;
                }
                if (c.P.scan_level == 0 && a == CM_CONCRD) st = CM_CONCRD;
            }
            __syncthreads();
        }
        __threadfence_block();
        if (owner) {
            if (st < 0) st = mr.type;
            if (__hip_atomic_load(ra.pair_err + t, __ATOMIC_RELAXED, __HIP_MEMORY_SCOPE_AGENT) != 0u) {
                ra.list[atomicAdd(ra.count, 1u)] = t;
                active[p] = 1;
            } else {
                uint8_t act = 1;
                cmc::finish_round(c, st, is_last, len1, len2, mr, act);
                state[p] = mr;
                active[p] = act;
                cat[p] = st;
                atomicAdd(&counters[CN_PAIR_ROUNDS], 1ull);
            }
        }
        __syncthreads();
        CM_TICK(sm, 13);
    }
#if defined(CM_DIAG)
    if (dbg_rows && lane == 0)
        for (int i = 0; i < 64; ++i) dbg_rows[(size_t)blockIdx.x * 64 + i] = tick_w[1 + i];
#endif
}

#include "cm_heavy_pipe.h"

__global__ void __launch_bounds__(BLK) k_active_cls(const uint8_t *active, uint64_t n, int8_t *cls) {
    const uint64_t i = (uint64_t)blockIdx.x * BLK + threadIdx.x;
    if (i < n) cls[i] = active[i] ? 0 : -2;
}
__global__ void __launch_bounds__(BLK) k_gather_active(const uint32_t *perm, const unsigned int *count, unsigned long long cap, const cm_mapped_read *state,
                                                       unsigned long long *out_idx, cm_mapped_read *out_state) {
    const uint64_t i = (uint64_t)blockIdx.x * BLK + threadIdx.x;
    if (i >= *count || i >= cap) return;
    const uint32_t p = perm[i];
    out_idx[i] = p;
    out_state[i] = state[p];
}

__global__ void __launch_bounds__(BLK) k_gather_records(const uint32_t *perm, const unsigned int *count, unsigned long long cap, const cm_mapped_read *state,
                                                        unsigned long long index_base, cm_record *out) {
    const uint64_t i = (uint64_t)blockIdx.x * BLK + threadIdx.x;
    if (i >= *count || i >= cap) return;
    const uint32_t p = perm[i];
    out[i].pair = index_base + p;
    out[i].state = state[p];
}

__global__ void __launch_bounds__(BLK) k_type_hist(const cm_mapped_read *state, uint64_t n, unsigned long long *hist) {
    __shared__ unsigned int h[16];
    if (threadIdx.x < 16) h[threadIdx.x] = 0;
    __syncthreads();
    for (uint64_t i = (uint64_t)blockIdx.x * BLK + threadIdx.x; i < n; i += (uint64_t)gridDim.x * BLK) {
        const int t = state[i].type;
        if (t >= 0 && t < 14) atomicAdd(&h[t], 1u);
    }
    __syncthreads();
    if (threadIdx.x < 14 && h[threadIdx.x]) atomicAdd(&hist[threadIdx.x], (unsigned long long)h[threadIdx.x]);
}
__global__ void k_err_clear(int *err, int mask) {
    if (threadIdx.x == 0 && blockIdx.x == 0) atomicAnd(err, ~mask);
}
__global__ void __launch_bounds__(BLK) k_build_desc(const uint32_t *bucket_off, const uint16_t *checksum, uint64_t n_buckets, int kmer, uint32_t *desc) {
    const uint64_t hv = (uint64_t)blockIdx.x * BLK + threadIdx.x;
    if (hv >= n_buckets) return;
    const uint32_t b0 = bucket_off[hv], n = bucket_off[hv + 1] - b0;
    uint32_t out[cmc::DESC_WORDS];
    cmc::desc_pack(b0, n, [&](uint32_t i) { return (uint32_t)checksum[b0 + i]; }, kmer, out);
    uint4 v;
    v.x = out[0]; v.y = out[1]; v.z = out[2]; v.w = out[3];
    ((uint4 *)desc)[hv] = v;
}
constexpr int S32_T = 1024, S32_E = 8, S32_B = S32_T * S32_E;
__global__ void __launch_bounds__(S32_T) k_scan32_a(const uint32_t *in, uint64_t n, uint32_t *out, uint32_t *bsum, uint32_t add, int inclusive) {
    __shared__ uint32_t wsum[S32_T / 64];
    const uint64_t base = (uint64_t)blockIdx.x * S32_B + (uint64_t)threadIdx.x * S32_E;
    uint32_t v[S32_E], run = 0;
#pragma unroll
    for (int k = 0; k < S32_E; ++k) {
        const uint64_t i = base + k;
        v[k] = i < n ? in[i] + add : 0u;
        run += v[k];
    }
    const int lane = threadIdx.x & 63, wave = threadIdx.x >> 6;
    uint32_t incl = run;
    for (int o = 1; o < 64; o <<= 1) {
        const uint32_t y = __shfl_up(incl, o);
        if (lane >= o) incl += y;
    }
    if (lane == 63) wsum[wave] = incl;
    __syncthreads();
    uint32_t wbase = 0;
    for (int w = 0; w < wave; ++w) wbase += wsum[w];
    uint32_t pre = wbase + incl - run;
#pragma unroll
    for (int k = 0; k < S32_E; ++k) {
        const uint64_t i = base + k;
        if (i < n) out[i] = inclusive ? pre + v[k] : pre;
        pre += v[k];
    }
    if (threadIdx.x == S32_T - 1) bsum[blockIdx.x] = pre;
}
__global__ void __launch_bounds__(S32_T) k_scan32_c(uint32_t *out, uint64_t n, const uint32_t *bsum) {
    const uint32_t add = bsum[blockIdx.x];
    const uint64_t base = (uint64_t)blockIdx.x * S32_B + (uint64_t)threadIdx.x * S32_E;
// ... 484 lines not shown
struct RowsBufs {
    ChrColumn<uint8_t> chr_text;
    ChrColumn<uint32_t> chr_off, chr_shift;
    CtxBuf<unsigned long long> total;
    BatchBuf<uint32_t> tmp;
    RowsFileBufs file[2];
    std::vector<uint8_t> h_path;
    BatchBuf<int64_t> keys;
    BatchBuf<uint64_t> rkey0, rkey1;
    BatchBuf<uint32_t> pair0, by_key, heads, gstart, list1, list2;
    BatchBuf<uint8_t> sort_ws;
    CtxBuf<unsigned int> ties;
};

struct Streams {
    hipStream_t B = nullptr;
    hipStream_t B2 = nullptr;
    hipStream_t C = nullptr;
    hipStream_t P = nullptr, P2 = nullptr;
    hipStream_t R = nullptr;
    hipStream_t O = nullptr;
    hipStream_t S = nullptr;
};
enum StreamKind { BLOCKING, NON_BLOCKING, NON_BLOCKING_LOWEST };
struct StreamDef {
    hipStream_t Streams::*st;
    const char *name;
    StreamKind kind;
};
constexpr StreamDef STREAMS[] = {
    {&Streams::B, "main", BLOCKING},           {&Streams::B2, "heavy chains", BLOCKING},     {&Streams::C, "copy", NON_BLOCKING},
    {&Streams::P, "pairs", NON_BLOCKING_LOWEST}, {&Streams::P2, "heavy pairs", NON_BLOCKING}, {&Streams::R, "re-run", NON_BLOCKING},
    {&Streams::O, "pair ordering", NON_BLOCKING}, {&Streams::S, "seeding", NON_BLOCKING},
};
struct Events {
    hipEvent_t fork = nullptr, join = nullptr;
    hipEvent_t join_p = nullptr, tail = nullptr;
    hipEvent_t flags = nullptr;
    hipEvent_t staged = nullptr, retired = nullptr;
    hipEvent_t order[2] = {nullptr, nullptr};
    hipEvent_t seed[2] = {nullptr, nullptr};
    hipEvent_t first[2] = {nullptr, nullptr};
    hipEvent_t prep[2] = {nullptr, nullptr}, pair[2] = {nullptr, nullptr};
    hipEvent_t *begin() { return &fork; }
    hipEvent_t *end() { return begin() + sizeof(Events) / sizeof(hipEvent_t); }
};
static_assert(sizeof(Events) == 17 * sizeof(hipEvent_t), "Events holds events only");

}

struct cm_ctx {
    cm_params P{};
    unsigned id = 0;
    int teardown_errors = 0;
    Streams st;
    Events ev;
    std::vector<DevMem *> bufs[2];
    struct Rerun {
        bool deferred = false;
        cmc::KCore core;
        ReadsDev rd;
        uint64_t p0 = 0;
        uint32_t nt = 0;
        cm_chain *chains = nullptr;
        int32_t *nchain = nullptr, *high = nullptr;
        uint8_t *act_out = nullptr;
        int is_last = 0, cap2 = 0;
        size_t lds2 = 0;
        bool fall = false;
        size_t lds_heavy = 0;
        int str_cap = 0;
        unsigned fall_grid = 0;
    } rerun[2];
    bool pair_pending[2] = {false, false};
    int item_base = 0;
    bool pre_launched = false;
    bool pre_ready = false;
    int pre_slot = -1, pre_b = 0;
    uint64_t pre_gen = 0, pre_n = 0;
    uint32_t pre_nt = 0;
    BatchBuf<uint8_t> d_ones;
    uint64_t ones_cap = 0;
    unsigned long long *h_pin = nullptr;
    uint32_t h_pin_nt = 0;
    std::string err = "";
    Slot slots[MAX_SLOTS];
    uint64_t n_pairs = 0;
    ReadBufs rd;
    BatchBuf<cm_mapped_read> d_state;
    BatchBuf<uint8_t> d_active;
    BatchBuf<uint8_t> d_active_b;
    BatchBuf<int32_t> d_cat;
    int n_seeds = 0, max_len = 0;
    struct Staged {
        bool ready = false, has_prior = false;
        uint64_t n_pairs = 0;
        int max_len = 0;
        ReadBufs rd;
        BatchBuf<cm_mapped_read> prior;
        void reset() { commit(0, 0, false, false), rd.keep_nothing(); }
        void commit(uint64_t n, int len, bool carried, bool is_ready = true) { n_pairs = n, max_len = len, has_prior = carried, ready = is_ready; }
    } staged;
    TextStage ft;
    RowsBufs rows;
    uint32_t tile = 0;
    SeedSet seed[2];
    ChainRecs rec[2];
    PairSetMem pair_mem;
    PairSet pset[2];
    PairSort sort;
    ChainWork dp;
    HeavyPipe hp;
    Collect col;
    BatchBuf<unsigned long long> d_lane_clk;
    BatchBuf<HRes> d_hres;
    BatchBuf<unsigned long long> d_type_hist;
    BatchBuf<unsigned long long> d_heavy_load;
    BatchBuf<cmc::MemoSpill> d_spill;
    CtxBuf<unsigned long long> d_pool_cursor;
    unsigned long long *pool_cursor(int s) const { return d_pool_cursor + s; }
    CtxBuf<int> d_err;
    CtxBuf<unsigned long long> d_counters;
    std::vector<unsigned long long> h_celloff;
    bool prof = false;
    std::vector<ProfRec> recs;
    std::vector<hipEvent_t> ev_free;
    double ms[PC_COUNT] = {};
    uint64_t launches[PC_COUNT] = {};
};

namespace {

int fail(cm_ctx *ctx, int code, const char *fmt, ...) {
    char buf[512];
    va_list ap;
    va_start(ap, fmt);
    vsnprintf(buf, sizeof buf, fmt, ap);
    va_end(ap);
    if (ctx) ctx->err = buf;
    return code;
}
#define HIPCHK(ctx, call)                                                                             \
    do {                                                                                              \
        hipError_t e_ = (call);                                                                       \
        if (e_ != hipSuccess) return fail(ctx, (e_ == hipErrorOutOfMemory) ? CM_ENOMEM : CM_EHIP, "%s: %s", #call, hipGetErrorString(e_)); \
    } while (0)

void report_hip(cm_ctx *ctx, const char *what, hipError_t e) {
    if (e == hipSuccess) return;
    const int k = ctx ? ctx->teardown_errors++ : 0;
    if (k < 8) fprintf(stderr, "[cmhot] context #%u: %s failed: %s (%d)\n", ctx ? ctx->id : 0u, what, hipGetErrorString(e), (int)e);
}

template <class T>
int up(cm_ctx *ctx, std::vector<void *> &allocs, const T *host, size_t n, const T **dev) {
    void *d = nullptr;
    size_t bytes = (n ? n : 1) * sizeof(T);
    HIPCHK(ctx, hipMalloc(&d, bytes));
    allocs.push_back(d);
    if (n) HIPCHK(ctx, hipMemcpyAsync(d, host, n * sizeof(T), hipMemcpyHostToDevice, ctx->st.B));
    *dev = (const T *)d;
    return CM_OK;
}
void free_all(cm_ctx *ctx, std::vector<void *> &v) {
    for (void *p : v) report_hip(ctx, "hipFree", hipFree(p));
    v.clear();
// ... 87 lines not shown
    const unsigned int *n_order = nullptr;
    const unsigned int *n_dev = nullptr;
    uint32_t grid_cap = 0;
};
void counting_sort(cm_ctx *ctx, ProfClass pc, const CountingSort &a) {
    const dim3 grid(a.grid_cap && a.grid_cap < a.nb ? a.grid_cap : a.nb);
    const unsigned int *count = a.order ? a.n_order : a.n_dev;
    launch(ctx, pc, k_cls_hist, grid, dim3(CLS_W), 0, a.st, a.cls, a.n, a.blk, a.nb, a.order, count);
    launch(ctx, pc, k_cls_scan, dim3(1), dim3(SCAN_CLS_T), 0, a.st, a.blk, a.nb, a.ctr, a.separate, a.n_used, a.n_dev);
    launch(ctx, pc, k_cls_place, grid, dim3(CLS_W), 0, a.st, a.cls, a.n, a.blk, a.nb, a.ctr, a.perm, a.hlist, a.order, count);
}

KCore make_core(const cm_ctx *c, const Slot &s) {
    KCore k;
    k.P = c->P;
    k.X = s.X;
    k.A = s.A;
    k.desc = s.d_desc;
    k.entry_near = s.entry_near;
    return k;
}

int check_slot(cm_ctx *ctx, int slot, bool need_annot) {
    if (slot < 0 || slot >= MAX_SLOTS) return fail(ctx, CM_EINVAL, "slot %d out of range", slot);
    if (!ctx->slots[slot].loaded) return fail(ctx, CM_ESTATE, "contig slot %d not loaded", slot);
    if (need_annot && !ctx->slots[slot].has_annot) return fail(ctx, CM_ESTATE, "annotation of slot %d not loaded", slot);
    return CM_OK;
}

ReadsDev reads_dev(const ReadBufs &r) { return ReadsDev{r.file[0].seq(), r.file[1].seq(), r.file[0].off, r.file[1].off}; }
ReadsDev current_reads(const cm_ctx *ctx) { return reads_dev(ctx->rd); }

constexpr unsigned HP_PLAN_GRID = 2048;
static bool heavy_pipeline() {
    static const bool v = !(getenv("CM_HEAVY_PIPELINE") && getenv("CM_HEAVY_PIPELINE")[0] == '0');
    return v;
}
static unsigned long long chain_light_w() {
    static const unsigned long long v = getenv("CM_CHAIN_LIGHT_W") ? strtoull(getenv("CM_CHAIN_LIGHT_W"), nullptr, 10) : 256ull;
    return v;
}
static unsigned int chain_light_cells() {
    static const unsigned int v = getenv("CM_CHAIN_LIGHT_CELLS") ? (unsigned)atoi(getenv("CM_CHAIN_LIGHT_CELLS")) : 96u;
    return v;
}

static bool skip_dead_chains(const cm_ctx *ctx) { return ctx->P.max_chain_len >= 1; }

static int seed_classes(cm_ctx *ctx, uint64_t pair0, uint32_t n_tile, const uint8_t *act, int s, hipStream_t st, const ChainRecs *rb, bool skip_dead,
                        bool defer = false) {
    const int S = ctx->n_seeds;
    const uint32_t n_prob = n_tile * 4u;
    if ((uint64_t)n_prob * (uint64_t)S == 0) return CM_OK;
    const SeedSet &sb = ctx->seed[s];
    if (sb.skip_dead != skip_dead) return fail(ctx, CM_ESTATE, "seed set %d: cell offsets and classes disagree about unchained problems", s);
    Timer t(ctx, PC_ORDER, st);
    launch(ctx, PC_ORDER, k_chain_cls, dim3((n_prob + BLK - 1) / BLK), dim3(BLK), 0, st, sb.scnt, sb.sraw, S, n_prob, sb.cls4, defer ? sb.thigh : rb->high,
           chain_light_w(), chain_light_cells(), defer ? (int32_t *)nullptr : rb->nchain, defer ? (uint16_t *)nullptr : rb->resid,
           defer ? (cm_chain *)nullptr : rb->chains, act, pair0, skip_dead ? 1 : 0, ctx->d_counters);
    ctx->seed[s].cls_deferred = defer;
    counting_sort(ctx, PC_ORDER, {st, sb.cls4, n_prob, sb.cblk, (n_prob + CLS_T - 1) / CLS_T, sb.cctr, sb.perm4});
    HIPCHK(ctx, hipMemsetAsync(ctx->pool_cursor(s), 0, sizeof(unsigned long long), st));
    HIPCHK(ctx, hipMemsetAsync(sb.cctr + CTR_CHAIN_NEXT, 0, sizeof(unsigned int), st));
    HIPCHK(ctx, hipGetLastError());
    return CM_OK;
}
int run_seed_tile(cm_ctx *ctx, const KCore &core, const ReadsDev &rd, uint64_t pair0, uint32_t n_tile, const uint8_t *act, int s, hipStream_t st,
                  const ChainRecs *rb, bool skip_dead, bool defer_rb = false) {
    const int S = ctx->n_seeds;
    const uint64_t total = (uint64_t)n_tile * 4u * (uint64_t)S;
    if (total == 0) return CM_OK;
    const SeedSet &sb = ctx->seed[s];
    {
        Timer t(ctx, PC_SEED, st);
        launch(ctx, PC_SEED, k_seed, dim3((unsigned)((total + BLK - 1) / BLK)), dim3(BLK), 0, st, core, rd, act, pair0, n_tile, S, sb.sstart, sb.scnt, sb.sraw,
               ctx->d_counters);
    }
    const uint32_t n_prob = n_tile * 4u;
    {
        Timer t(ctx, PC_SCAN, st);
        const uint32_t nb = (n_prob + SCAN_ELEMS - 1) / SCAN_ELEMS;
        launch(ctx, PC_SCAN, k_scan_a, dim3(nb), dim3(SCAN_T), 0, st, sb.scnt, S, n_prob, sb.celloff, sb.bsum, sb.bmax, skip_dead ? 1 : 0);
        ctx->seed[s].skip_dead = skip_dead;
        launch(ctx, PC_SCAN, k_scan_mid<unsigned long long, true>, dim3(1), dim3(1024), 0, st, sb.bsum, nb, sb.celloff + n_prob, sb.bmax);
        launch(ctx, PC_SCAN, k_scan_c, dim3((n_prob + SCAN_T - 1) / SCAN_T), dim3(SCAN_T), 0, st, sb.celloff, sb.bsum, n_prob);
    }
    HIPCHK(ctx, hipMemcpyAsync(ctx->h_pin + PIN_CELLS + 2 * s, sb.celloff + n_prob, 2 * sizeof(unsigned long long), hipMemcpyDeviceToHost, st));
    if (rb) {
        const int rc = seed_classes(ctx, pair0, n_tile, act, s, st, rb, skip_dead, defer_rb);
        if (rc) return rc;
    }
    HIPCHK(ctx, hipEventRecord(ctx->ev.seed[s], st));
    HIPCHK(ctx, hipGetLastError());
    return CM_OK;
}

int run_chain_tile(cm_ctx *ctx, const KCore &core, const ReadsDev &rd, uint64_t pair0, uint32_t n_tile, bool parallel_ok, const uint8_t *act,
                   const ChainRecs &rb, int s, const std::function<int()> &after_launch = {}) {
    const int S = ctx->n_seeds;
    const uint32_t n_prob = n_tile * 4u;
    if (n_prob == 0 || S == 0) return after_launch ? after_launch() : CM_OK;
    const SeedSet &sb = ctx->seed[s];
    HIPCHK(ctx, hipStreamWaitEvent(ctx->st.B, ctx->ev.seed[s], 0));
    HIPCHK(ctx, hipEventSynchronize(ctx->ev.seed[s]));
    if (ctx->seed[s].cls_deferred) {
        hipLaunchKernelGGL(k_chain_apply, dim3((n_prob + BLK - 1) / BLK), dim3(BLK), 0, ctx->st.B, n_prob, (const int8_t *)sb.cls4, (const int32_t *)sb.thigh,
                           rb.high, rb.nchain, rb.resid, rb.chains);
        ctx->seed[s].cls_deferred = false;
    }
    const unsigned long long total = ctx->h_pin[PIN_CELLS + 2 * s];
    const unsigned long long max_cells = ctx->h_pin[PIN_CELLS + 2 * s + 1];
    std::vector<std::pair<uint32_t, uint32_t>> ranges;
    if (total <= ctx->dp.cells_cap) {
        ranges.push_back({0u, n_prob});
    } else {
        ctx->h_celloff.resize((size_t)n_prob + 1);
        HIPCHK(ctx, hipMemcpyAsync(ctx->h_celloff.data(), sb.celloff, ((size_t)n_prob + 1) * sizeof(unsigned long long), hipMemcpyDeviceToHost,
                                   ctx->st.B));
        HIPCHK(ctx, hipStreamSynchronize(ctx->st.B));
        uint32_t a = 0;
        while (a < n_prob) {
            uint32_t b = a;
            while (b < n_prob && ctx->h_celloff[b + 1] - ctx->h_celloff[a] <= ctx->dp.cells_cap) ++b;
            if (b == a) return fail(ctx, CM_ELIMIT, "one chaining problem needs %llu DP cells (> workspace %llu)",
                                    ctx->h_celloff[a + 1] - ctx->h_celloff[a], ctx->dp.cells_cap);
            ranges.push_back({a, b});
            a = b;
        }
    }
    const size_t lds_extra = ((size_t)max_cells / 64 + 2) * 8 + 640;
    const size_t lds_need = (size_t)max_cells * sizeof(uint32_t) + lds_extra + (size_t)heavy_im_words((uint32_t)max_cells, (uint32_t)S) * sizeof(uint32_t);
    const size_t heavy_lds = std::max<size_t>(std::min<size_t>((size_t)S * (size_t)ctx->P.seed_lim * sizeof(uint32_t),
                                                               ((size_t)max_cells * sizeof(uint32_t) + 2047) / 2048 * 2048 + 2048) + (lds_extra + 255) / 256 * 256,
                                              (lds_need + 255) / 256 * 256);
#if defined(CM_CHAIN_DIAG)
    fprintf(stderr, "heavy_lds %zu (largest problem %llu cells)\n", heavy_lds, max_cells);
#endif
    const bool split = ranges.size() == 1 && parallel_ok && heavy_lds <= 152u * 1024u;
    bool fresh = true;
    auto launch_group = [&](uint32_t a, uint32_t b, unsigned long long base, bool use_split) -> int {
        const uint32_t n = b - a;
        if (!fresh) {
            HIPCHK(ctx, hipMemsetAsync(ctx->pool_cursor(s), 0, sizeof(unsigned long long), ctx->st.B));
            HIPCHK(ctx, hipMemsetAsync(sb.cctr + CTR_CHAIN_NEXT, 0, sizeof(unsigned int), ctx->st.B));
        }
        fresh = false;
        if (use_split) {
            HIPCHK(ctx, hipEventRecord(ctx->ev.fork, ctx->st.B));
            HIPCHK(ctx, hipStreamWaitEvent(ctx->st.B2, ctx->ev.fork, 0));
            {
            Timer t(ctx, PC_CHAIN_HEAVY, ctx->st.B2);
            static std::atomic<size_t> heavy_attr{64u * 1024u};
            if (heavy_lds > heavy_attr.load()) {
                HIPCHK(ctx, hipFuncSetAttribute((const void *)k_chain_heavy, hipFuncAttributeMaxDynamicSharedMemorySize, (int)heavy_lds));
                heavy_attr.store(heavy_lds);
            }
            const uint32_t hb = n < 8192u ? n : 8192u;
            launch(ctx, PC_CHAIN_HEAVY, k_chain_heavy, dim3(hb), dim3(64), heavy_lds, ctx->st.B2, core, rd, pair0, S, sb.sstart, sb.scnt, sb.celloff,
                   ctx->dp.score, ctx->dp.prev, ctx->dp.pool, ctx->dp.pool_bytes, ctx->pool_cursor(s), rb.chains, rb.nchain, ctx->d_err, rb.resid, sb.perm4,
                   sb.cctr + CTR_BASE + CHAIN_LIGHT_CLS - 1, sb.cctr + CTR_CHAIN_NEXT, ctx->d_counters);
            }
            HIPCHK(ctx, hipEventRecord(ctx->ev.join, ctx->st.B2));
        }
        Timer t(ctx, PC_CHAIN);
        launch(ctx, PC_CHAIN, k_chain, dim3((n + BLK_CHAIN - 1) / BLK_CHAIN), dim3(BLK_CHAIN), 0, ctx->st.B, core, rd, act, pair0, a, b, S, sb.sstart, sb.scnt,
               sb.sraw, sb.celloff, base, ctx->dp.score, ctx->dp.prev, ctx->dp.pool, ctx->dp.pool_bytes, ctx->pool_cursor(s), rb.chains, rb.nchain, rb.high,
               ctx->d_err, rb.resid, use_split ? sb.perm4 : (const uint32_t *)nullptr, sb.cctr + CTR_BASE + CHAIN_LIGHT_CLS - 1, sb.cctr + CTR_SUM,
               sb.skip_dead ? (const int8_t *)sb.cls4 : (const int8_t *)nullptr);
        if (use_split) HIPCHK(ctx, hipStreamWaitEvent(ctx->st.B, ctx->ev.join, 0));
        HIPCHK(ctx, hipGetLastError());
        return CM_OK;
    };
    auto pool_lost = [&](bool *lost) -> int {
        HIPCHK(ctx, hipMemcpyAsync(ctx->h_pin + PIN_POOL_ERR, ctx->d_err, sizeof(int), hipMemcpyDeviceToHost, ctx->st.B));
        HIPCHK(ctx, hipStreamSynchronize(ctx->st.B));
        const int e = *(const int *)(ctx->h_pin + PIN_POOL_ERR);
        *lost = (e & cmc::ERR_POOL) != 0;
        if (*lost) {
            hipLaunchKernelGGL(k_err_clear, dim3(1), dim3(64), 0, ctx->st.B, ctx->d_err, (int)cmc::ERR_POOL);
            HIPCHK(ctx, hipStreamSynchronize(ctx->st.B));
        }
        return CM_OK;
    };
    const unsigned long long pool_max = getenv("CM_POOL_MAX") ? strtoull(getenv("CM_POOL_MAX"), nullptr, 10) : (48ull << 30);
    bool told = false;
    for (auto &rg : ranges) {
        unsigned long long base = 0;
        if (rg.first != 0) base = ctx->h_celloff[rg.first];
        int rc = launch_group(rg.first, rg.second, base, split);
        if (rc) return rc;
        if (!told && after_launch && (rc = after_launch())) return rc;
        told = true;
        bool lost = false;
        if ((rc = pool_lost(&lost))) return rc;
        while (lost && ctx->dp.pool_bytes < pool_max) {
            unsigned long long want = ctx->dp.pool_bytes * 4ull;
            if (want > pool_max) want = pool_max;
            HIPCHK(ctx, hipStreamSynchronize(ctx->st.B2));
            if (ensure(ctx, ctx->dp.pool, want) != hipSuccess) {
                (void)hipGetLastError();
                HIPCHK(ctx, ensure(ctx, ctx->dp.pool, ctx->dp.pool_bytes));
                break;
            }
            ctx->dp.pool_bytes = want;
            if ((rc = launch_group(rg.first, rg.second, base, split))) return rc;
            if ((rc = pool_lost(&lost))) return rc;
        }
        if (lost) {
            std::vector<std::pair<uint32_t, uint32_t>> todo{{rg.first, rg.second}};
            while (!todo.empty()) {
                const auto pc = todo.back();
                todo.pop_back();
                if ((rc = launch_group(pc.first, pc.second, base, false))) return rc;
                if ((rc = pool_lost(&lost))) return rc;
                if (!lost) continue;
                if (pc.second - pc.first <= 1)
                    return fail(ctx, CM_ELIMIT, "one chaining problem's improvement log does not fit %llu bytes", ctx->dp.pool_bytes);
                const uint32_t mid = pc.first + (pc.second - pc.first) / 2;
                todo.push_back({mid, pc.second});
                todo.push_back({pc.first, mid});
            }
        }
    }
    return CM_OK;
}

int check_dev_err(cm_ctx *ctx) {
    HIPCHK(ctx, hipMemcpyAsync(ctx->h_pin + PIN_DEV_ERR, ctx->d_err, sizeof(int), hipMemcpyDeviceToHost, ctx->st.B));
    HIPCHK(ctx, hipStreamSynchronize(ctx->st.B));
    const int e = *(const int *)(ctx->h_pin + PIN_DEV_ERR);
    if (e) {
        (void)hipMemsetAsync(ctx->d_err, 0, sizeof(int), ctx->st.B);
        return fail(ctx, CM_ELIMIT, "device capacity limit hit:%s%s%s", (e & cmc::ERR_POOL) ? " chain improvement-log pool exhausted;" : "",
                    (e & (cmc::ERR_SEEDS | cmc::ERR_BAND)) ? " DP string longer than the staging buffer;" : "",
                    (e & cmc::ERR_MEMO) ? " extension memo overflowed where the reference's memo would have served a colliding key" : "");
    }
    return CM_OK;
}

}

extern "C" {

int cm_create(const cm_params *p, cm_ctx **out) {
    if (!p || !out) return CM_EINVAL;
    *out = nullptr;
    const int c = p->kmer - CM_WINDOW_SIZE;
    if (p->kmer < CM_WINDOW_SIZE || c > 8) return CM_EINVAL;
    if (p->max_chain_len < 1 || p->max_chain_len > CM_BESTCHAINLIM) return CM_EINVAL;
    if (p->band < 0 || p->band > cmc::MAX_BAND) return CM_EINVAL;
    if (p->seed_lim < 1 || p->seed_lim > 65535) return CM_EINVAL;
    if (p->max_ed < 0 || p->max_sc < 0 || p->max_read_len < p->kmer) return CM_EINVAL;
    const char *hwq = getenv("GPU_MAX_HW_QUEUES");
    const bool hwq_low = !hwq || atoi(hwq) < 16;
    setenv("GPU_MAX_HW_QUEUES", "16", 0);
    int ndev = 0;
    if (hipGetDeviceCount(&ndev) != hipSuccess || ndev <= 0) return CM_ENODEV;
    if (p->device < 0 || p->device >= ndev) return CM_ENODEV;
    if (hipSetDevice(p->device) != hipSuccess) return CM_ENODEV;
    cm_ctx *ctx = new cm_ctx();
    ctx->P = *p;
    {
        static std::atomic<unsigned> serial{0};
        ctx->id = ++serial;
    }
    int prio_lo = 0, prio_hi = 0;
    (void)hipDeviceGetStreamPriorityRange(&prio_lo, &prio_hi);
    for (const StreamDef &d : STREAMS) {
        hipStream_t *st = &(ctx->st.*d.st);
        if ((d.kind == BLOCKING              ? hipStreamCreate(st)
             : d.kind == NON_BLOCKING_LOWEST ? hipStreamCreateWithPriority(st, hipStreamNonBlocking, prio_lo)
                                             : hipStreamCreateWithFlags(st, hipStreamNonBlocking)) != hipSuccess) {
            cm_destroy(ctx);
            return CM_EHIP;
        }
    }
    for (hipEvent_t &e : ctx->ev)
        if (hipEventCreateWithFlags(&e, hipEventDisableTiming) != hipSuccess) {
            cm_destroy(ctx);
            return CM_EHIP;
        }
    if (ensure(ctx, ctx->d_pool_cursor, 2 * sizeof(unsigned long long)) != hipSuccess ||
        ensure(ctx, ctx->d_err, sizeof(int)) != hipSuccess ||
        ensure(ctx, ctx->d_counters, CN_WORDS * sizeof(unsigned long long)) != hipSuccess ||
        hipHostMalloc((void **)&ctx->h_pin, PIN_BYTES, hipHostMallocDefault) != hipSuccess) {
        cm_destroy(ctx);
        return CM_ENOMEM;
    }
    memset(ctx->h_pin, 0, PIN_BYTES);
    (void)hipMemsetAsync(ctx->d_err, 0, sizeof(int), ctx->st.B);
    (void)hipMemsetAsync(ctx->d_counters, 0, CN_WORDS * sizeof(unsigned long long), ctx->st.B);
    if (hwq_low) {
        ctx->err = "note: GPU_MAX_HW_QUEUES was " + std::string(hwq ? hwq : "unset") +
                   " when this context was created; if HIP was initialised earlier in this process the seven streams of a context share the "
                   "default 4 hardware queues (pipelined rounds run slower). Export GPU_MAX_HW_QUEUES=16 before the first HIP call.";
        static std::atomic<bool> said{false};
        if (hwq && !said.exchange(true) && !getenv("CM_QUIET")) fprintf(stderr, "[cmhot] %s\n", ctx->err.c_str());
    }
    *out = ctx;
    return CM_OK;
}

void cm_destroy(cm_ctx *ctx) {
    if (!ctx) return;
    report_hip(ctx, "hipSetDevice", hipSetDevice(ctx->P.device));
    for (const StreamDef &d : STREAMS)
        if (ctx->st.*d.st) report_hip(ctx, (std::string("hipStreamSynchronize(") + d.name + ")").c_str(), hipStreamSynchronize(ctx->st.*d.st));
    report_hip(ctx, "hipGetLastError at teardown", hipGetLastError());
    for (auto e : ctx->ev_free) report_hip(ctx, "hipEventDestroy", hipEventDestroy(e));
    ctx->ev_free.clear();
    for (auto &r : ctx->recs) {
        report_hip(ctx, "hipEventDestroy", hipEventDestroy(r.a));
        report_hip(ctx, "hipEventDestroy", hipEventDestroy(r.b));
    }
    ctx->recs.clear();
    free_reads(ctx);
    for (auto &s : ctx->slots) {
        free_all(ctx, s.idx_allocs);
        free_all(ctx, s.ann_allocs);
        drop_entry_near(ctx, s);
    }
    release(ctx, CONTEXT);
    if (ctx->h_pin) report_hip(ctx, "hipHostFree", hipHostFree(ctx->h_pin));
    for (hipEvent_t e : ctx->ev)
        if (e) report_hip(ctx, "hipEventDestroy", hipEventDestroy(e));
    for (const StreamDef &d : STREAMS)
        if (ctx->st.*d.st) report_hip(ctx, "hipStreamDestroy", hipStreamDestroy(ctx->st.*d.st));
    delete ctx;
}

const char *cm_last_error(const cm_ctx *ctx) { return ctx ? ctx->err.c_str() : "null context"; }

static int make_entry_near(cm_ctx *ctx, Slot &s) {
    drop_entry_near(ctx, s);
    if (!s.loaded || !s.has_annot || s.X.n_entries == 0) return CM_OK;
    if (s.X.ref_len > 0x80000000u) return CM_OK;
    const uint64_t n = s.X.n_entries;
    uint64_t *d = nullptr;
    if (hipMalloc((void **)&d, (size_t)((n + 63) / 64) * sizeof(uint64_t)) != hipSuccess) {
        (void)hipGetLastError();
        return CM_OK;
    }
    s.entry_near = d;
    hipLaunchKernelGGL(k_entry_near, dim3((unsigned)((n + BLK - 1) / BLK)), dim3(BLK), 0, ctx->st.B, s.X.pos, n, s.A.near_border_bits, (uint64_t)s.A.n_bits, d);
    hipError_t e = hipGetLastError();
    if (e == hipSuccess) e = hipStreamSynchronize(ctx->st.B);
    if (e != hipSuccess) drop_entry_near(ctx, s);
    HIPCHK(ctx, e);
    return CM_OK;
}

static int finish_contig(cm_ctx *ctx, Slot &s) {
    const size_t nb = ((size_t)1 << (2 * CM_WINDOW_SIZE)) + 1;
    s.d_desc = nullptr;
    static const bool use_desc = !(getenv("CM_SEED_DESC") && getenv("CM_SEED_DESC")[0] == '0');
    if (use_desc) {
        const uint64_t n_buckets = nb - 1;
        uint32_t *d = nullptr;
        if (hipMalloc((void **)&d, n_buckets * cmc::DESC_WORDS * sizeof(uint32_t)) == hipSuccess) {
            s.idx_allocs.push_back(d);
            hipLaunchKernelGGL(k_build_desc, dim3((unsigned)((n_buckets + BLK - 1) / BLK)), dim3(BLK), 0, ctx->st.B, s.X.bucket_off, s.X.checksum, n_buckets,
                               ctx->P.kmer, d);
            HIPCHK(ctx, hipGetLastError());
            s.d_desc = d;
        } else (void)hipGetLastError();
    }
    HIPCHK(ctx, hipStreamSynchronize(ctx->st.B));
    s.loaded = true;
    return make_entry_near(ctx, s);
}

int cm_load_contig(cm_ctx *ctx, int slot, const cm_index_view *iv) {
    if (!ctx || !iv) return CM_EINVAL;
    if (slot < 0 || slot >= MAX_SLOTS) return fail(ctx, CM_EINVAL, "slot %d out of range", slot);
    if (!iv->genome || !iv->bucket_off || !iv->checksum || !iv->pos) return fail(ctx, CM_EINVAL, "null index array");
    HIPCHK(ctx, hipSetDevice(ctx->P.device));
    Slot &s = ctx->slots[slot];
    free_all(ctx, s.idx_allocs);
    drop_entry_near(ctx, s);
    s.d_desc = nullptr;
    s.loaded = false;
    ++s.gen;
    const size_t nb = ((size_t)1 << (2 * CM_WINDOW_SIZE)) + 1;
    s.X = *iv;
    int rc;
    {
        uint8_t *g = nullptr;
        const size_t pad = cmc::CM_STAGE_PAD;
        HIPCHK(ctx, hipMalloc((void **)&g, (size_t)iv->ref_len + 2 * pad));
        s.idx_allocs.push_back(g);
        HIPCHK(ctx, hipMemsetAsync(g, 0, (size_t)iv->ref_len + 2 * pad, ctx->st.B));
        HIPCHK(ctx, hipMemcpyAsync(g + pad, iv->genome, (size_t)iv->ref_len, hipMemcpyHostToDevice, ctx->st.B));
        s.X.genome = g + pad;
    }
    if ((rc = up(ctx, s.idx_allocs, iv->bucket_off, nb, &s.X.bucket_off))) return rc;
    if ((rc = up(ctx, s.idx_allocs, iv->checksum, (size_t)iv->n_entries, &s.X.checksum))) return rc;
    if ((rc = up(ctx, s.idx_allocs, iv->pos, (size_t)iv->n_entries, &s.X.pos))) return rc;
    return finish_contig(ctx, s);
}

static int scan32_on(cm_ctx *ctx, hipStream_t st, const uint32_t *in, uint64_t n, uint32_t *out, uint32_t *tmp, uint32_t add, int inclusive) {
    const uint32_t nb = (uint32_t)((n + S32_B - 1) / S32_B);
    if (nb == 0) return CM_OK;
    hipLaunchKernelGGL(k_scan32_a, dim3(nb), dim3(S32_T), 0, st, in, n, out, tmp, add, inclusive);
    hipLaunchKernelGGL((k_scan_mid<uint32_t, false>), dim3(1), dim3(1024), 0, st, tmp, nb, (uint32_t *)nullptr, (const unsigned int *)nullptr);
    hipLaunchKernelGGL(k_scan32_c, dim3(nb), dim3(S32_T), 0, st, out, n, (const uint32_t *)tmp);
    HIPCHK(ctx, hipGetLastError());
    return CM_OK;
}
static int scan32(cm_ctx *ctx, const uint32_t *in, uint64_t n, uint32_t *out, uint32_t *tmp, uint32_t add, int inclusive) {
    return scan32_on(ctx, ctx->st.B, in, n, out, tmp, add, inclusive);
}

int cm_load_contig_raw(cm_ctx *ctx, int slot, const cm_index_raw *raw) {
    if (!ctx || !raw) return CM_EINVAL;
    if (slot < 0 || slot >= MAX_SLOTS) return fail(ctx, CM_EINVAL, "slot %d out of range", slot);
    if (!raw->genome || (raw->n_buckets && (!raw->hv || !raw->count14 || !raw->table))) return fail(ctx, CM_EINVAL, "null array in the raw record");
    if (raw->table_slots > 0xffffffffull) return fail(ctx, CM_ELIMIT, "table of %llu slots", (unsigned long long)raw->table_slots);
    HIPCHK(ctx, hipSetDevice(ctx->P.device));
    Slot &s = ctx->slots[slot];
    free_all(ctx, s.idx_allocs);
    drop_entry_near(ctx, s);
    s.d_desc = nullptr;
    s.loaded = false;
    ++s.gen;
    const uint64_t n_all = (uint64_t)1 << (2 * CM_WINDOW_SIZE);
    const uint32_t n_b = raw->n_buckets;
    s.X = cm_index_view{};
    s.X.contig_num = raw->contig_num;
    s.X.ref_len = raw->ref_len;
    int rc;
    {
        uint8_t *g = nullptr;
        const size_t pad = cmc::CM_STAGE_PAD;
        HIPCHK(ctx, hipMalloc((void **)&g, (size_t)raw->ref_len + 2 * pad));
        s.idx_allocs.push_back(g);
        HIPCHK(ctx, hipMemsetAsync(g, 0, (size_t)raw->ref_len + 2 * pad, ctx->st.B));
        HIPCHK(ctx, hipMemcpyAsync(g + pad, raw->genome, (size_t)raw->ref_len, hipMemcpyHostToDevice, ctx->st.B));
        s.X.genome = g + pad;
    }
    std::vector<void *> tmp;
    struct FreeTmp {
        cm_ctx *c;
        std::vector<void *> &v;
        ~FreeTmp() { free_all(c, v); }
    } free_tmp{ctx, tmp};
    const RawEntry *d_tab = nullptr;
    const uint32_t *d_hv = nullptr, *d_cnt = nullptr;
    if ((rc = up(ctx, tmp, (const RawEntry *)raw->table, (size_t)raw->table_slots, &d_tab))) return rc;
    if ((rc = up(ctx, tmp, raw->hv, (size_t)n_b, &d_hv))) return rc;
    if ((rc = up(ctx, tmp, raw->count14, (size_t)n_b, &d_cnt))) return rc;
    uint32_t *d_start = nullptr, *d_bs = nullptr, *d_off = nullptr;
    int *d_bad = nullptr;
    HIPCHK(ctx, hipMalloc((void **)&d_start, ((size_t)n_b + 1) * sizeof(uint32_t)));
    tmp.push_back(d_start);
    HIPCHK(ctx, hipMalloc((void **)&d_bs, ((size_t)(n_all / S32_B) + 4) * sizeof(uint32_t)));
    tmp.push_back(d_bs);
    HIPCHK(ctx, hipMalloc((void **)&d_bad, sizeof(int)));
    tmp.push_back(d_bad);
    HIPCHK(ctx, hipMemsetAsync(d_bad, 0, sizeof(int), ctx->st.B));
    HIPCHK(ctx, hipMalloc((void **)&d_off, (n_all + 1) * sizeof(uint32_t)));
    s.idx_allocs.push_back(d_off);
    HIPCHK(ctx, hipMemsetAsync(d_off, 0, (n_all + 1) * sizeof(uint32_t), ctx->st.B));
    if ((rc = scan32(ctx, d_cnt, n_b, d_start, d_bs, 1u, 0))) return rc;
    if (n_b) {
        hipLaunchKernelGGL(k_raw_counts, dim3((n_b + BLK - 1) / BLK), dim3(BLK), 0, ctx->st.B, d_tab, (const uint32_t *)d_start, d_hv, d_cnt, n_b, n_all, d_off, d_bad);
        HIPCHK(ctx, hipGetLastError());
    }
    if ((rc = scan32(ctx, d_off, n_all + 1, d_off, d_bs, 0u, 1))) return rc;
    unsigned long long landing[2] = {0, 0};
    HIPCHK(ctx, hipMemcpyAsync(&landing[0], d_off + n_all, sizeof(uint32_t), hipMemcpyDeviceToHost, ctx->st.B));
    HIPCHK(ctx, hipMemcpyAsync(&landing[1], d_bad, sizeof(int), hipMemcpyDeviceToHost, ctx->st.B));
    HIPCHK(ctx, hipStreamSynchronize(ctx->st.B));
    if ((int)landing[1]) return fail(ctx, CM_EINVAL, "malformed index table: a bucket header is out of range");
    const uint64_t total = (uint32_t)landing[0];
    uint16_t *d_cs = nullptr;
    uint32_t *d_ps = nullptr;
    HIPCHK(ctx, hipMalloc((void **)&d_cs, (total ? total : 1) * sizeof(uint16_t)));
    s.idx_allocs.push_back(d_cs);
    HIPCHK(ctx, hipMalloc((void **)&d_ps, (total ? total : 1) * sizeof(uint32_t)));
    s.idx_allocs.push_back(d_ps);
    if (n_b) {
        hipLaunchKernelGGL(k_raw_scatter, dim3((n_b + BLK - 1) / BLK), dim3(BLK), 0, ctx->st.B, d_tab, (const uint32_t *)d_start, d_hv, n_b, (const uint32_t *)d_off, d_cs, d_ps);
        HIPCHK(ctx, hipGetLastError());
    }
    s.X.bucket_off = d_off;
    s.X.checksum = d_cs;
    s.X.pos = d_ps;
// ... 286 lines not shown
    unsigned started = 1;
    try {
        for (; started < n_thr; ++started) th[started] = std::thread(scan, n * started / n_thr, n * (started + 1) / n_thr, &bd[started], &lg[started]);
    } catch (...) {
    }
    scan(0, n / n_thr, &bd[0], &lg[0]);
    for (unsigned k = started; k < n_thr; ++k) scan(n * k / n_thr, n * (k + 1) / n_thr, &bd[k], &lg[k]);
    for (unsigned k = 1; k < started; ++k) th[k].join();
    for (unsigned k = 0; k < n_thr; ++k) {
        if (bd[k] && !bad) bad = bd[k];
        if (lg[k] > longest) longest = lg[k];
    }
    if (bad) {
        const uint64_t i = bad - 1;
        if (rd->off1[i + 1] < rd->off1[i] || rd->off2[i + 1] < rd->off2[i]) return fail(ctx, CM_EINVAL, "read offsets not monotone at pair %llu", (unsigned long long)i);
        return fail(ctx, CM_EINVAL, "pair %llu longer than max_read_len %d", (unsigned long long)i, ctx->P.max_read_len);
    }
    *max_len_out = (int)longest;
    return check_seeds(ctx, (int)longest);
}

static uint32_t tile_for(uint64_t n) {
    uint32_t tile_cap = TILE_PAIRS;
    if (n > 2ull * TILE_PAIRS) {
        const uint64_t half = ((n + 1) / 2 + 65535) / 65536 * 65536;
        tile_cap = (uint32_t)std::min<uint64_t>(half, TILE_PAIRS_MAX);
    }
    if (const char *e = getenv("CM_TILE_PAIRS")) {
        const long v = atol(e);
        if (v >= 64 && v <= (1l << 24)) tile_cap = (uint32_t)v;
    }
    return (uint32_t)(n < tile_cap ? n : tile_cap);
}

static int prepare_resident(cm_ctx *ctx, uint64_t n, int max_len) {
    ctx->n_seeds = max_len / ctx->P.kmer;
    ctx->max_len = max_len;
    HIPCHK(ctx, ensure(ctx, ctx->d_state, n * sizeof(cm_mapped_read)));
    HIPCHK(ctx, ensure(ctx, ctx->d_active, n));
    HIPCHK(ctx, ensure(ctx, ctx->d_active_b, n));
    HIPCHK(ctx, ensure(ctx, ctx->d_cat, n * sizeof(int32_t)));
    const uint32_t tile = tile_for(n);
    ctx->tile = tile;
    const size_t nprob = (size_t)tile * 4, nprobe = nprob * (size_t)(ctx->n_seeds ? ctx->n_seeds : 1);
    for (SeedSet &sd : ctx->seed) {
        HIPCHK(ctx, ensure(ctx, sd.sstart, nprobe * 4));
        HIPCHK(ctx, ensure(ctx, sd.scnt, nprobe * 4));
        HIPCHK(ctx, ensure(ctx, sd.sraw, nprobe * 4));
        HIPCHK(ctx, ensure(ctx, sd.celloff, (nprob + 2) * 8));
        HIPCHK(ctx, ensure(ctx, sd.bmax, (nprob / SCAN_ELEMS + 2) * 4));
        HIPCHK(ctx, ensure(ctx, sd.bsum, (nprob / SCAN_ELEMS + 2) * 8));
        HIPCHK(ctx, ensure(ctx, sd.cctr, CTR_WORDS * sizeof(unsigned int)));
        HIPCHK(ctx, ensure(ctx, sd.cblk, (size_t)N_CLS * (4 * (size_t)tile / CLS_T + 2) * sizeof(unsigned int)));
        HIPCHK(ctx, ensure(ctx, sd.cls4, (size_t)tile * 4));
        HIPCHK(ctx, ensure(ctx, sd.perm4, (size_t)tile * 4 * 4));
        HIPCHK(ctx, ensure(ctx, sd.thigh, (size_t)tile * 4 * sizeof(int32_t)));
    }
    for (ChainRecs &cr : ctx->rec) {
        HIPCHK(ctx, ensure(ctx, cr.chains, nprob * CM_BESTCHAINLIM * sizeof(cm_chain)));
        HIPCHK(ctx, ensure(ctx, cr.nchain, nprob * 4));
        HIPCHK(ctx, ensure(ctx, cr.high, nprob * 4));
        HIPCHK(ctx, ensure(ctx, cr.resid, (size_t)tile * 4 * sizeof(uint16_t)));
    }
    unsigned long long cap = (unsigned long long)nprob * 64ull;
    const unsigned long long worst = (unsigned long long)ctx->P.seed_lim * (unsigned long long)(ctx->n_seeds ? ctx->n_seeds : 1);
    if (cap < (8ull << 20)) cap = 8ull << 20;
    if (cap < worst) cap = worst;
    if (cap > ctx->dp.cells_cap || !ctx->dp.score) ctx->dp.cells_cap = cap;
    HIPCHK(ctx, ensure(ctx, ctx->dp.score, ctx->dp.cells_cap * sizeof(double)));
    HIPCHK(ctx, ensure(ctx, ctx->dp.prev, ctx->dp.cells_cap * sizeof(int32_t)));
    HIPCHK(ctx, ensure(ctx, ctx->sort.cls, (size_t)tile));
    PairSetMem &pm = ctx->pair_mem;
    HIPCHK(ctx, ensure(ctx, pm.perm, (size_t)tile * 4 * 2));
    HIPCHK(ctx, ensure(ctx, pm.hlist, (size_t)tile * 4 * 2));
    HIPCHK(ctx, ensure(ctx, ctx->d_hres, (size_t)HEAVY_GRID_MAX * (64 * sizeof(HRes) + HEAVY_SCRATCH)));
    if (heavy_pipeline()) {
        const size_t tc = getenv("CM_HP_TASKS_CAP") ? (size_t)std::max(1, atoi(getenv("CM_HP_TASKS_CAP"))) : std::max<size_t>((size_t)tile * 6, 4096);
        const size_t uc = getenv("CM_HP_UNP_CAP") ? (size_t)std::max(1, atoi(getenv("CM_HP_UNP_CAP"))) : std::max<size_t>((size_t)tile * 4, 4096);
        ctx->hp.tasks_cap = (uint32_t)tc;
        ctx->hp.unp_cap = (uint32_t)uc;
        HIPCHK(ctx, ensure(ctx, ctx->hp.pairs, (size_t)tile * sizeof(HPair)));
        HIPCHK(ctx, ensure(ctx, ctx->hp.list2, (size_t)tile * 4));
        HIPCHK(ctx, ensure(ctx, pm.hp_fall, (size_t)tile * 4 * 2));
        HIPCHK(ctx, ensure(ctx, pm.hp_fallctr, 2 * sizeof(unsigned int)));
        HIPCHK(ctx, ensure(ctx, ctx->hp.T, tc * sizeof(HTask)));
        HIPCHK(ctx, ensure(ctx, ctx->hp.tcls, tc));
        HIPCHK(ctx, ensure(ctx, ctx->hp.tperm, tc * 4));
        HIPCHK(ctx, ensure(ctx, ctx->hp.tblk, (size_t)N_CLS * (tc / CLS_T + 2) * sizeof(unsigned int)));
        HIPCHK(ctx, ensure(ctx, ctx->hp.tctr, CTR_WORDS * sizeof(unsigned int)));
        HIPCHK(ctx, ensure(ctx, ctx->hp.pre, tc * 4 * sizeof(cmc::PreDP)));
        HIPCHK(ctx, ensure(ctx, ctx->hp.q, tc * 4 * 4));
        HIPCHK(ctx, ensure(ctx, ctx->hp.res, tc * sizeof(HRes)));
        HIPCHK(ctx, ensure(ctx, ctx->hp.U, uc * sizeof(HUnp)));
        HIPCHK(ctx, ensure(ctx, ctx->hp.pre2, uc * 2 * sizeof(cmc::PreDP)));
        HIPCHK(ctx, ensure(ctx, ctx->hp.q2, uc * 2 * 4));
        HIPCHK(ctx, ensure(ctx, ctx->hp.lists, (size_t)HP_PLAN_GRID * HEAVY_LIST * 2));
        HIPCHK(ctx, ensure(ctx, ctx->hp.ctr, HC_WORDS * sizeof(unsigned int)));
    }
    {
        const uint32_t *before = pm.pair_err;
        HIPCHK(ctx, ensure(ctx, pm.pair_err, (size_t)tile * 4 * 2));
        if (pm.pair_err != before) HIPCHK(ctx, hipMemsetAsync(pm.pair_err, 0, (size_t)tile * 4 * 2, ctx->st.P));
    }
    HIPCHK(ctx, ensure(ctx, pm.retry_list, (size_t)tile * 4 * 2));
    HIPCHK(ctx, ensure(ctx, pm.retry_ctr, 4 * sizeof(unsigned int)));
    HIPCHK(ctx, ensure(ctx, ctx->d_heavy_load, sizeof(unsigned long long)));
    HIPCHK(ctx, ensure(ctx, ctx->d_spill, (size_t)RETRY_GRID * BLK_PAIR * RETRY_SPILL * sizeof(cmc::MemoSpill)));
    HIPCHK(ctx, ensure(ctx, pm.cls_ctr, 2 * CTR_WORDS * sizeof(unsigned int)));
    HIPCHK(ctx, ensure(ctx, ctx->sort.ctr2, CTR_WORDS * sizeof(unsigned int)));
    HIPCHK(ctx, ensure(ctx, ctx->sort.sub, (size_t)tile));
    HIPCHK(ctx, ensure(ctx, ctx->sort.perm1, (size_t)tile * 4));
    HIPCHK(ctx, ensure(ctx, ctx->sort.ctr3, CTR_WORDS * sizeof(unsigned int)));
    HIPCHK(ctx, ensure(ctx, ctx->sort.sub2, (size_t)tile));
    HIPCHK(ctx, ensure(ctx, ctx->sort.perm0, (size_t)tile * 4));
    HIPCHK(ctx, ensure(ctx, ctx->sort.blk_cnt, (size_t)N_CLS * (4 * (size_t)tile / CLS_T + 2) * sizeof(unsigned int)));
    if (getenv("CM_LANE_CLK")) {
#if defined(CM_DIAG)
        const size_t clk_words = 16 * 2 + 1;
#else
        const size_t clk_words = 1;
#endif
        HIPCHK(ctx, ensure(ctx, ctx->d_lane_clk, n * 8 * clk_words));
        HIPCHK(ctx, hipMemsetAsync(ctx->d_lane_clk, 0, n * 8 * clk_words, ctx->st.B));
    }
    unsigned long long pool = (unsigned long long)nprob * 2048ull;
    if (pool < (256ull << 20)) pool = 256ull << 20;
    if (pool > (8ull << 30)) pool = 8ull << 30;
    if (const char *e = getenv("CM_POOL_BYTES")) {
        const unsigned long long v = strtoull(e, nullptr, 10);
        if (v >= 4096 && !ctx->dp.pool) pool = v;
    }
    if (pool > ctx->dp.pool_bytes || !ctx->dp.pool) ctx->dp.pool_bytes = pool;
    HIPCHK(ctx, ensure(ctx, ctx->dp.pool, ctx->dp.pool_bytes));
    for (int b = 0; b < 2; ++b) {
        const size_t at = (size_t)b * tile;
        ctx->pset[b] = PairSet{pm.perm + at,       pm.hlist + at,      pm.cls_ctr + (size_t)b * CTR_WORDS,
                               pm.pair_err + at,   pm.retry_list + at, pm.retry_ctr + 2 * b,
                               pm.hp_fall ? pm.hp_fall + at : nullptr, pm.hp_fallctr ? pm.hp_fallctr + b : nullptr};
    }
    return CM_OK;
}

static int copy_reads(cm_ctx *ctx, const cm_reads *rd, hipStream_t st, ReadBufs &to) {
    const uint64_t n = rd->n_pairs;
    const uint8_t *const seq[2] = {rd->seq1, rd->seq2};
    const uint64_t *const off[2] = {rd->off1, rd->off2};
    const size_t bytes[2] = {(size_t)off[0][n] - (size_t)off[0][0], (size_t)off[1][n] - (size_t)off[1][0]};
    if (off[0][0] != 0 || off[1][0] != 0) return fail(ctx, CM_EINVAL, "read offsets must start at 0");
    const size_t pad = cmc::CM_STAGE_PAD;
    for (int f = 0; f < 2; ++f) HIPCHK(ctx, ensure(ctx, to.file[f].seq_base, bytes[f] + 2 * pad));
    for (int f = 0; f < 2; ++f) HIPCHK(ctx, ensure(ctx, to.file[f].off, (n + 1) * sizeof(uint64_t)));
    for (int f = 0; f < 2; ++f) {
        HIPCHK(ctx, hipMemsetAsync(to.file[f].seq_base, 0, pad, st));
        HIPCHK(ctx, hipMemsetAsync(to.file[f].seq_base + pad + bytes[f], 0, pad, st));
    }
    for (int f = 0; f < 2; ++f)
        if (bytes[f]) HIPCHK(ctx, hipMemcpyAsync(to.file[f].seq(), seq[f], bytes[f], hipMemcpyHostToDevice, st));
    for (int f = 0; f < 2; ++f) HIPCHK(ctx, hipMemcpyAsync(to.file[f].off, off[f], (n + 1) * sizeof(uint64_t), hipMemcpyHostToDevice, st));
    return CM_OK;
}

static int make_resident(cm_ctx *ctx, uint64_t n, int max_len, hipEvent_t after, const cm_mapped_read *prior, hipMemcpyKind kind) {
    if (int rc = prepare_resident(ctx, n, max_len)) return rc;
    ctx->n_pairs = n;
    if (after) HIPCHK(ctx, hipStreamWaitEvent(ctx->st.B, after, 0));
    KCore k{};
    k.P = ctx->P;
    hipLaunchKernelGGL(k_init_state, dim3((unsigned)((n + BLK - 1) / BLK)), dim3(BLK), 0, ctx->st.B, k, ctx->d_state, ctx->d_active, ctx->d_cat, n);
    if (prior) HIPCHK(ctx, hipMemcpyAsync(ctx->d_state, prior, n * sizeof(cm_mapped_read), kind, ctx->st.B));
    return CM_OK;
}

int cm_reads_upload(cm_ctx *ctx, const cm_reads *rd, const cm_mapped_read *prior) {
    if (!ctx || !rd) return CM_EINVAL;
    HIPCHK(ctx, hipSetDevice(ctx->P.device));
    HIPCHK(ctx, hipStreamSynchronize(ctx->st.B));
    const uint64_t n = rd->n_pairs;
    ctx->pre_ready = false;
    ctx->n_pairs = 0;
    ctx->tile = 0;
    if (n == 0) {
        free_reads(ctx);
        return CM_OK;
    }
    int max_len = 0, rc = check_reads(ctx, rd, &max_len);
    if (rc) return rc;
    ctx->rd.keep_nothing();
    if ((rc = copy_reads(ctx, rd, ctx->st.B, ctx->rd)) || (rc = make_resident(ctx, n, max_len, nullptr, prior, hipMemcpyHostToDevice))) return rc;
    HIPCHK(ctx, hipStreamSynchronize(ctx->st.B));
    return CM_OK;
}

static int stage_open(cm_ctx *ctx) {
    HIPCHK(ctx, hipStreamSynchronize(ctx->st.C));
    ctx->staged.reset();
    ctx->pre_launched = false;
    return CM_OK;
}

int cm_reads_stage(cm_ctx *ctx, const cm_reads *rd, const cm_mapped_read *prior) {
    if (!ctx || !rd) return CM_EINVAL;
    HIPCHK(ctx, hipSetDevice(ctx->P.device));
    if (rd->n_pairs == 0) return fail(ctx, CM_EINVAL, "cm_reads_stage: empty batch");
    int max_len = 0, rc = check_reads(ctx, rd, &max_len);
    if (rc || (rc = stage_open(ctx)) || (rc = copy_reads(ctx, rd, ctx->st.C, ctx->staged.rd))) return rc;
    if (prior) {
        HIPCHK(ctx, ensure(ctx, ctx->staged.prior, rd->n_pairs * sizeof(cm_mapped_read)));
        HIPCHK(ctx, hipMemcpyAsync(ctx->staged.prior, prior, rd->n_pairs * sizeof(cm_mapped_read), hipMemcpyHostToDevice, ctx->st.C));
    }
    HIPCHK(ctx, hipEventRecord(ctx->ev.staged, ctx->st.C));
    ctx->staged.commit(rd->n_pairs, max_len, prior != nullptr);
    return CM_OK;
}

static int ft_begin(cm_ctx *ctx, const cmft::Sizes &S, const uint8_t *const text[2], const uint64_t len[2]) {
    TextStage &T = ctx->ft;
    const size_t words = (size_t)S.nb + 1;
    for (int f = 0; f < 2; ++f) HIPCHK(ctx, ensure(ctx, ctx->staged.rd.file[f].seq_base, len[f] + 2 * cmc::CM_STAGE_PAD));
    for (int f = 0; f < 2; ++f) HIPCHK(ctx, ensure(ctx, ctx->staged.rd.file[f].off, words * sizeof(uint64_t)));
    HIPCHK(ctx, ensure(ctx, T.res, cmft::RES_WORDS * sizeof(unsigned long long)));
    for (int f = 0; f < 2; ++f) {
// ... 173 lines not shown
    HIPCHK(ctx, hipStreamWaitEvent(ctx->st.C, ctx->ev.retired, 0));
    HIPCHK(ctx, hipGetLastError());
    return CM_OK;
}

static int launch_rerun(cm_ctx *ctx, int b) {
    const cm_ctx::Rerun &q = ctx->rerun[b];
    const PairSet &ps = ctx->pset[b];
    const RetryArgs ra2{ps.pair_err, ps.retry_list, ps.retry_ctr, ctx->d_spill, RETRY_SPILL, 0};
    hipLaunchKernelGGL(k_pair_rerun, dim3(RETRY_GRID), dim3(BLK_PAIR), q.lds2, ctx->st.R, q.core, q.rd, q.p0, q.nt, q.chains, q.nchain, q.high,
                       ctx->d_state, q.act_out, ctx->d_cat, q.is_last, ctx->d_err, ctx->d_counters, q.cap2, (unsigned long long *)nullptr,
                       (const uint32_t *)ps.retry_list, (const unsigned int *)ps.retry_ctr, ps.retry_ctr + 1, ra2);
    HIPCHK(ctx, hipGetLastError());
    return CM_OK;
}
static int launch_fall_back(cm_ctx *ctx, int b, hipStream_t st) {
    const cm_ctx::Rerun &q = ctx->rerun[b];
    const PairSet &ps = ctx->pset[b];
    const RetryArgs ra1{ps.pair_err, ps.retry_list, ps.retry_ctr, nullptr, 0, 1};
    launch(ctx, PC_HEAVY, k_pair_heavy, dim3(q.fall_grid), dim3(BLK_PAIR), q.lds_heavy, st, q.core, q.rd, q.p0, ps.hp_fall, ps.hp_fallctr, q.chains, q.nchain, q.high,
           ctx->d_state, q.act_out, ctx->d_cat, q.is_last, ctx->d_err, ctx->d_counters, q.str_cap, nullptr, ctx->d_hres, ps.cls_ctr + CTR_NEXT + 1, ra1);
    HIPCHK(ctx, hipGetLastError());
    return CM_OK;
}
static int settle_pair(cm_ctx *ctx, int b, bool wait = true) {
    if (!ctx->rerun[b].deferred) return CM_OK;
    ctx->rerun[b].deferred = false;
    if (wait) HIPCHK(ctx, hipEventSynchronize(ctx->ev.first[b]));
    HIPCHK(ctx, hipStreamWaitEvent(ctx->st.R, ctx->ev.first[b], 0));
    bool fell = false;
    if (ctx->rerun[b].fall && (!wait || *(const volatile unsigned int *)(ctx->h_pin + PIN_FALL_N + b) != 0u)) {
        const int rc = launch_fall_back(ctx, b, ctx->st.R);
        if (rc) return rc;
        fell = true;
    }
    if (!wait || fell || *(const volatile unsigned int *)(ctx->h_pin + PIN_RERUN_N + b) != 0u) {
        const int rc = launch_rerun(ctx, b);
        if (rc) return rc;
    }
    HIPCHK(ctx, hipEventRecord(ctx->ev.pair[b], ctx->st.R));
    return CM_OK;
}

static int run_pair_tile(cm_ctx *ctx, const KCore &core, uint64_t p0, uint32_t nt, int is_last_round, const uint8_t *act_in, uint8_t *act_out,
                         const ChainRecs &rb, int b, bool same_tile_as_prev, bool defer) {
    const ReadsDev rd = current_reads(ctx);
    hipStream_t sp = ctx->st.P, sp2 = ctx->st.P2, sp3 = ctx->st.R;
    {
        int rc;
        if ((rc = settle_pair(ctx, b))) return rc;
        if (same_tile_as_prev && (rc = settle_pair(ctx, b ^ 1))) return rc;
    }
    hipStream_t so = ctx->st.O;
    HIPCHK(ctx, hipStreamWaitEvent(so, ctx->ev.prep[b], 0));
    if (same_tile_as_prev && ctx->pair_pending[b ^ 1]) HIPCHK(ctx, hipStreamWaitEvent(so, ctx->ev.pair[b ^ 1], 0));
    const PairSet &ps = ctx->pset[b];
    uint32_t *const perm = ps.perm, *const hlist = ps.hlist, *const pair_err = ps.pair_err;
    unsigned int *const cls_ctr = ps.cls_ctr, *const retry_ctr = ps.retry_ctr;
    constexpr int str_slack = 4;
    const int str_cap = ((ctx->max_len - ctx->P.kmer + ctx->P.band + str_slack + 7) / 8) * 8;
    constexpr unsigned slots_per_simd = 4;
    const size_t lds_bytes = (size_t)2 * lbuf_bytes(str_cap) * BLK_PAIR;
    const size_t lds_heavy = lds_bytes + HG * sizeof(HSlot);
    const int cap2 = std::min(((2 * ctx->max_len + 64 + 7) / 8) * 8, 1016);
    const size_t lds2 = (size_t)2 * lbuf_bytes(cap2) * BLK_PAIR;
    {
        static std::atomic<size_t> lim[3] = {{48u * 1024u}, {48u * 1024u}, {48u * 1024u}};
        const void *fn[3] = {(const void *)k_pair, (const void *)k_pair_rerun, (const void *)k_pair_heavy};
        const size_t want[3] = {lds_bytes, lds2, lds_heavy};
        for (int k = 0; k < 3; ++k)
            if (want[k] > lim[k].load()) {
                HIPCHK(ctx, hipFuncSetAttribute(fn[k], hipFuncAttributeMaxDynamicSharedMemorySize, (int)want[k]));
                lim[k].store(want[k]);
            }
    }
    {
        Timer t(ctx, PC_ORDER, so);
        const uint32_t nbk = (nt + CLS_T - 1) / CLS_T;
        static const bool fixed_cost = getenv("CM_HEAVY_COST") != nullptr;
        static const int heavy_cost = fixed_cost ? atoi(getenv("CM_HEAVY_COST")) : HEAVY_COST;
        unsigned long long *load = nullptr;
        if (!fixed_cost) {
            load = ctx->d_heavy_load;
            HIPCHK(ctx, hipMemsetAsync(load, 0, sizeof(unsigned long long), so));
            launch(ctx, PC_NONE, k_pair_cost, dim3((nt + BLK - 1) / BLK), dim3(BLK), 0, so, rb.nchain, act_in, p0, nt, HEAVY_COST, load);
            HIPCHK(ctx, hipMemcpyAsync((void *)(ctx->h_pin + PIN_HEAVY_LOAD), load, sizeof(unsigned long long), hipMemcpyDeviceToHost, so));
            ctx->h_pin_nt = nt;
        }
        launch(ctx, PC_ORDER, k_pair_cls, dim3((nt + BLK - 1) / BLK), dim3(BLK), 0, so, core, rb.chains, rb.resid, rb.nchain, act_in, p0, nt, ctx->sort.cls, ctx->d_cat,
               heavy_cost, ctx->sort.sub, ctx->sort.sub2, act_out, load);
        const PairSort &w = ctx->sort;
        counting_sort(ctx, PC_ORDER, {so, w.sub2, nt, w.blk_cnt, nbk, w.ctr3, w.perm0});
        counting_sort(ctx, PC_ORDER, {so, w.sub, nt, w.blk_cnt, nbk, w.ctr2, w.perm1, N_CLS, nullptr, -1, w.perm0, w.ctr3 + CTR_SUM});
        counting_sort(ctx, PC_ORDER, {so, w.cls, nt, w.blk_cnt, nbk, cls_ctr, perm, N_CLS, hlist, 1 << HEAVY_CLS, w.perm1, w.ctr2 + CTR_SUM});
    }
    HIPCHK(ctx, hipMemsetAsync(cls_ctr + CTR_NEXT, 0, 2 * sizeof(unsigned int), so));
    HIPCHK(ctx, hipMemsetAsync(retry_ctr, 0, 2 * sizeof(unsigned int), so));
    HIPCHK(ctx, hipEventRecord(ctx->ev.order[b], so));
    HIPCHK(ctx, hipStreamWaitEvent(sp, ctx->ev.prep[b], 0));
    HIPCHK(ctx, hipStreamWaitEvent(sp, ctx->ev.order[b], 0));
    const RetryArgs ra1{pair_err, ps.retry_list, retry_ctr, nullptr, 0, 1};
    {
        cm_ctx::Rerun &q = ctx->rerun[b];
        q.core = core; q.rd = rd; q.p0 = p0; q.nt = nt;
        q.chains = rb.chains; q.nchain = rb.nchain; q.high = rb.high;
        q.act_out = act_out; q.is_last = is_last_round; q.cap2 = cap2; q.lds2 = lds2;
        q.fall = false;
    }
    HIPCHK(ctx, hipStreamWaitEvent(sp2, ctx->ev.prep[b], 0));
    HIPCHK(ctx, hipStreamWaitEvent(sp2, ctx->ev.order[b], 0));
    {
        Timer t(ctx, PC_HEAVY, sp2);
        const unsigned cap = 256u * 4u * slots_per_simd;
        const volatile unsigned long long *seen = (const volatile unsigned long long *)(ctx->h_pin + PIN_HEAVY_LOAD);
        const bool loaded_run = ctx->h_pin_nt && *seen > HEAVY_LOAD * (unsigned long long)ctx->h_pin_nt;
        const unsigned heavy_cap = cap / (loaded_run ? 1u : 2u);
        const unsigned heavy_lim = std::min(heavy_cap, HEAVY_GRID_MAX);
        const unsigned heavy_grid = nt < heavy_lim ? (nt ? nt : 1u) : heavy_lim;
        if (heavy_pipeline() && ctx->P.band == 3) {
            const HPipe hp{ctx->hp.pairs, ctx->hp.list2, ps.hp_fall, ctx->hp.T, ctx->hp.pre, ctx->hp.q, ctx->hp.res, ctx->hp.U, ctx->hp.pre2,
                           ctx->hp.q2, ctx->hp.ctr, ctx->hp.tasks_cap, ctx->hp.unp_cap, ps.hp_fallctr, ctx->hp.tcls};
            const unsigned int *n_heavy = cls_ctr + HEAVY_CLS, *n_list2 = ctx->hp.ctr + HC_LIST2;
            constexpr unsigned pipe_grid = 2048u;
            const size_t lds_slots = HG * sizeof(HSlot);
            HIPCHK(ctx, hipMemsetAsync(ctx->hp.ctr, 0, HC_WORDS * sizeof(unsigned int), sp2));
            HIPCHK(ctx, hipMemsetAsync(ps.hp_fallctr, 0, sizeof(unsigned int), sp2));
            const dim3 g(pipe_grid), wg(BLK_PAIR);
            static const bool task_order = !(getenv("CM_HP_TASK_ORDER") && getenv("CM_HP_TASK_ORDER")[0] == '0');
            static const int n_attempts = (getenv("CM_HP_ATTEMPTS") && atoi(getenv("CM_HP_ATTEMPTS")) == 1) ? 1 : 2;
            for (int attempt = 0; attempt < n_attempts; ++attempt) {
                if (attempt) launch(ctx, PC_HEAVY, k_hp_reset, dim3(1), dim3(64), 0, sp2, ctx->hp.ctr);
                else ++ctx->launches[PC_HEAVY];
                launch(ctx, PC_HEAVY, k_hp_plan, dim3(HP_PLAN_GRID), wg, lds_slots, sp2, core, rd, p0, hlist, n_heavy, ctx->hp.list2, n_list2, attempt,
                       rb.chains, rb.nchain, rb.high, ctx->d_state, hp, ctx->hp.lists, str_cap, ctx->d_counters);
                launch(ctx, PC_HEAVY, k_hp_dp, g, wg, lds_bytes, sp2, core, rd, p0, attempt, hp, 0, str_cap);
                const bool ordered = task_order && attempt == 0;
                if (ordered) {
                    const unsigned int *n_t = ctx->hp.ctr + HC_TASKS;
                    CountingSort ts{sp2, ctx->hp.tcls, ctx->hp.tasks_cap, ctx->hp.tblk, (ctx->hp.tasks_cap + CLS_T - 1) / CLS_T, ctx->hp.tctr, ctx->hp.tperm};
                    ts.n_dev = n_t, ts.grid_cap = 2048u;
                    counting_sort(ctx, PC_NONE, ts);
                }
                launch(ctx, PC_HEAVY, k_hp_tasks, g, wg, lds_bytes, sp2, core, rd, p0, attempt, rb.chains, rb.nchain, hp, pair_err, str_cap, ordered ? (uint32_t *)ctx->hp.tperm : nullptr,
                     ctx->hp.tctr + CTR_SUM);
                launch(ctx, PC_HEAVY, k_hp_fold, g, wg, 0, sp2, core, p0, ctx->hp.list2, n_list2, n_heavy, attempt, hp, ctx->d_counters);
                launch(ctx, PC_HEAVY, k_hp_unp_req, g, wg, 0, sp2, core, rd, p0, attempt, rb.chains, hp, str_cap);
                launch(ctx, PC_HEAVY, k_hp_dp, g, wg, lds_bytes, sp2, core, rd, p0, attempt, hp, 1, str_cap);
                launch(ctx, PC_HEAVY, k_hp_unp, g, wg, lds_bytes, sp2, core, rd, p0, attempt, rb.chains, hp, pair_err, str_cap);
                launch(ctx, PC_HEAVY, k_hp_finish, g, wg, 0, sp2, core, p0, ctx->hp.list2, n_list2, n_heavy, attempt, hp, ctx->d_state, act_out, ctx->d_cat, is_last_round, ctx->d_counters, ra1,
                     rb.nchain, n_attempts == 1 ? 1 : 0);
            }
            HIPCHK(ctx, hipMemcpyAsync((void *)(ctx->h_pin + PIN_FALL_N + b), ps.hp_fallctr, sizeof(unsigned int), hipMemcpyDeviceToHost, sp2));
            {
                cm_ctx::Rerun &q = ctx->rerun[b];
                q.fall = true;
                q.lds_heavy = lds_heavy;
                q.str_cap = str_cap;
                q.fall_grid = std::min(heavy_grid, 256u);
            }
            if (!defer) {
                int rc;
                if ((rc = launch_fall_back(ctx, b, sp2))) return rc;
                ctx->rerun[b].fall = false;
            }
        } else {
            launch(ctx, PC_HEAVY, k_pair_heavy, dim3(heavy_grid), dim3(BLK_PAIR), lds_heavy, sp2, core, rd, p0, hlist, cls_ctr + HEAVY_CLS, rb.chains, rb.nchain, rb.high,
                   ctx->d_state, act_out, ctx->d_cat, is_last_round, ctx->d_err, ctx->d_counters, str_cap,
                   ctx->d_lane_clk ? ctx->d_lane_clk + (size_t)nt * 16 + (size_t)(nt / 64 + 1) * 64 : nullptr, ctx->d_hres, cls_ctr + CTR_NEXT + 1, ra1);
        }
    }
    HIPCHK(ctx, hipEventRecord(ctx->ev.join_p, sp2));
    {
        Timer t(ctx, PC_PAIR, sp);
        const unsigned want = (nt + BLK_PAIR - 1) / BLK_PAIR, cap = (heavy_pipeline() && ctx->P.band == 3) ? 2048u
                                                                                                           : 256u * 4u * slots_per_simd;
        launch(ctx, PC_PAIR, k_pair, dim3(want < cap ? want : cap), dim3(BLK_PAIR), lds_bytes, sp, core, rd, p0, nt, rb.chains, rb.nchain, rb.high, ctx->d_state,
               act_out, ctx->d_cat, is_last_round, ctx->d_err, ctx->d_counters, str_cap, ctx->d_lane_clk, perm, cls_ctr + CTR_SUM, cls_ctr + CTR_NEXT, ra1);
        HIPCHK(ctx, hipStreamWaitEvent(sp, ctx->ev.join_p, 0));
    }
    HIPCHK(ctx, hipMemcpyAsync((void *)(ctx->h_pin + PIN_RERUN_N + b), retry_ctr, sizeof(unsigned int), hipMemcpyDeviceToHost, sp));
    HIPCHK(ctx, hipEventRecord(ctx->ev.first[b], sp));
    ctx->rerun[b].deferred = defer;
    if (!defer) {
        HIPCHK(ctx, hipStreamWaitEvent(sp3, ctx->ev.first[b], 0));
        int rc;
        if ((rc = launch_rerun(ctx, b))) return rc;
        HIPCHK(ctx, hipEventRecord(ctx->ev.pair[b], sp3));
    }
    ctx->pair_pending[b] = true;
    HIPCHK(ctx, hipGetLastError());
    return CM_OK;
}

static int map_rounds_issue(cm_ctx *ctx, const int *slots, int n_rounds, int last_is_final, int *items_done, int *rounds_done) {
    int rc;
    const bool prefetch = last_is_final && ctx->staged.ready && ctx->staged.n_pairs <= ctx->n_pairs && ctx->staged.max_len <= ctx->max_len;
    if (prefetch && ctx->ones_cap < ctx->staged.n_pairs) {
        HIPCHK(ctx, ensure(ctx, ctx->d_ones, ctx->n_pairs));
        HIPCHK(ctx, hipMemsetAsync(ctx->d_ones, 1, ctx->n_pairs, ctx->st.B));
        ctx->ones_cap = ctx->n_pairs;
    }
    HIPCHK(ctx, hipEventRecord(ctx->ev.tail, ctx->st.B));
    HIPCHK(ctx, hipStreamWaitEvent(ctx->st.P, ctx->ev.tail, 0));
    HIPCHK(ctx, hipStreamWaitEvent(ctx->st.S, ctx->ev.tail, 0));
    HIPCHK(ctx, hipStreamWaitEvent(ctx->st.O, ctx->ev.tail, 0));
    HIPCHK(ctx, hipEventRecord(ctx->ev.flags, ctx->st.B));
    uint8_t *A[2] = {ctx->d_active, ctx->d_active_b};
    struct Item { uint64_t p0; uint32_t nt; int r; };
    std::vector<Item> items;
    const uint64_t n_tiles = (ctx->n_pairs + ctx->tile - 1) / ctx->tile;
    const bool round_major = n_tiles >= 2;
    auto tile_nt = [&](uint64_t t) { return (uint32_t)((ctx->n_pairs - t * ctx->tile < ctx->tile) ? ctx->n_pairs - t * ctx->tile : ctx->tile); };
    if (round_major) {
        for (int r = 0; r < n_rounds; ++r)
            for (uint64_t t = 0; t < n_tiles; ++t) items.push_back(Item{t * ctx->tile, tile_nt(t), r});
    } else {
        for (uint64_t t = 0; t < n_tiles; ++t)
            for (int r = 0; r < n_rounds; ++r) items.push_back(Item{t * ctx->tile, tile_nt(t), r});
    }
    const int n_items = (int)items.size();
    std::vector<int> tiles_of_round((size_t)n_rounds, 0);
    const bool use_pre = ctx->pre_ready && slots[0] == ctx->pre_slot && ctx->slots[slots[0]].gen == ctx->pre_gen && ctx->n_pairs == ctx->pre_n &&
                         items[0].nt == ctx->pre_nt && (ctx->item_base & 1) == ctx->pre_b;
    ctx->pre_ready = ctx->pre_launched = false;
    if (use_pre) ++ctx->launches[PC_PREFETCH];
    const ReadsDev rd_cur = current_reads(ctx);
    auto prep_flags = [&](int i) -> const uint8_t * {
        const int r = items[i].r;
        return round_major ? A[r & 1] : ((r == 0) ? A[0] : A[(r - 1) & 1]);
    };
    std::vector<char> seeded((size_t)n_items, 0);
    bool pre_seeded = false;
    const bool early_ok = round_major;
    auto issue_seed_early = [&](int i) -> int {
        HIPCHK(ctx, hipStreamWaitEvent(ctx->st.S, ctx->ev.flags, 0));
        if (n_tiles == 2 && i >= 2) HIPCHK(ctx, hipStreamWaitEvent(ctx->st.S, ctx->ev.first[(ctx->item_base + i) & 1], 0));
        const ChainRecs &rbe = ctx->rec[(ctx->item_base + i) & 1];
        const int e = run_seed_tile(ctx, make_core(ctx, ctx->slots[slots[items[i].r]]), rd_cur, items[i].p0, items[i].nt, prep_flags(i), i & 1, ctx->st.S, &rbe, skip_dead_chains(ctx), true);
        seeded[(size_t)i] = 1;
        return e;
    };
    auto issue_seed = [&](int i, hipStream_t st) -> int {
        const int b = (ctx->item_base + i) & 1;
        int e;
        if ((e = settle_pair(ctx, b))) return e;
        if (ctx->pair_pending[b]) HIPCHK(ctx, hipStreamWaitEvent(st, ctx->ev.pair[b], 0));
        const ChainRecs &rbi = ctx->rec[b];
        e = run_seed_tile(ctx, make_core(ctx, ctx->slots[slots[items[i].r]]), rd_cur, items[i].p0, items[i].nt, prep_flags(i), i & 1, st, &rbi, skip_dead_chains(ctx));
        seeded[(size_t)i] = 1;
        return e;
    };
    for (int i = 0; i < n_items; ++i) {
        const uint64_t p0 = items[i].p0;
        const uint32_t nt = items[i].nt;
        const int r = items[i].r, b = (ctx->item_base + i) & 1;
        const Slot &sl = ctx->slots[slots[r]];
        const KCore core = make_core(ctx, sl);
        const ChainRecs &rb = ctx->rec[b];
        const uint8_t *act_prep = prep_flags(i);
        auto ahead = [&]() -> int {
            if (i + 1 >= n_items || seeded[(size_t)i + 1]) return CM_OK;
            if (early_ok) return issue_seed_early(i + 1);
            const int bn = (ctx->item_base + i + 1) & 1;
// ... 559 lines not shown

int cm_map_batch(cm_ctx *ctx, int slot, int is_last_round, const cm_reads *reads, const cm_mapped_read *prior, cm_mapped_read *out_state,
                 int32_t *out_category) {
    int rc = cm_reads_upload(ctx, reads, prior);
    if (rc) return rc;
    if ((rc = cm_map_round(ctx, slot, is_last_round))) return rc;
    return cm_reads_download(ctx, out_state, out_category, nullptr);
}

int cm_seed_batch(cm_ctx *ctx, int slot, uint32_t *out_start, uint32_t *out_cnt, uint32_t *out_raw, uint32_t cap_probes, uint32_t *out_n_slots) {
    if (!ctx || !out_start || !out_cnt || !out_raw || !out_n_slots) return CM_EINVAL;
    int rc = check_slot(ctx, slot, false);
    if (rc) return rc;
    HIPCHK(ctx, hipSetDevice(ctx->P.device));
    *out_n_slots = (uint32_t)ctx->n_seeds;
    const uint64_t need = ctx->n_pairs * 4ull * (uint64_t)ctx->n_seeds;
    if (need > cap_probes) return fail(ctx, CM_EINVAL, "cm_seed_batch: need room for %llu probes", (unsigned long long)need);
    const KCore core = make_core(ctx, ctx->slots[slot]);
    for (uint64_t p0 = 0; p0 < ctx->n_pairs; p0 += ctx->tile) {
        const uint32_t nt = (uint32_t)((ctx->n_pairs - p0 < ctx->tile) ? ctx->n_pairs - p0 : ctx->tile);
        if ((rc = run_seed_tile(ctx, core, current_reads(ctx), p0, nt, ctx->d_active, 0, ctx->st.B, nullptr, false))) return rc;
        const size_t cnt = (size_t)nt * 4 * ctx->n_seeds, o = (size_t)p0 * 4 * ctx->n_seeds;
        HIPCHK(ctx, hipMemcpyAsync(out_start + o, ctx->seed[0].sstart, cnt * 4, hipMemcpyDeviceToHost, ctx->st.B));
        HIPCHK(ctx, hipMemcpyAsync(out_cnt + o, ctx->seed[0].scnt, cnt * 4, hipMemcpyDeviceToHost, ctx->st.B));
        HIPCHK(ctx, hipMemcpyAsync(out_raw + o, ctx->seed[0].sraw, cnt * 4, hipMemcpyDeviceToHost, ctx->st.B));
        HIPCHK(ctx, hipStreamSynchronize(ctx->st.B));
    }
    return CM_OK;
}

int cm_chain_batch(cm_ctx *ctx, int slot, cm_chain *out_chains, int32_t *out_nchain, int32_t *out_high) {
    if (!ctx || !out_chains || !out_nchain || !out_high) return CM_EINVAL;
    int rc = check_slot(ctx, slot, true);
    if (rc) return rc;
    HIPCHK(ctx, hipSetDevice(ctx->P.device));
    const KCore core = make_core(ctx, ctx->slots[slot]);
    for (uint64_t p0 = 0; p0 < ctx->n_pairs; p0 += ctx->tile) {
        const uint32_t nt = (uint32_t)((ctx->n_pairs - p0 < ctx->tile) ? ctx->n_pairs - p0 : ctx->tile);
        HIPCHK(ctx, hipMemsetAsync(ctx->rec[0].chains, 0, (size_t)nt * 4 * CM_BESTCHAINLIM * sizeof(cm_chain), ctx->st.B));
        const ChainRecs &rb0 = ctx->rec[0];
        if ((rc = run_seed_tile(ctx, core, current_reads(ctx), p0, nt, ctx->d_active, 0, ctx->st.B, &rb0, false))) return rc;
        if ((rc = run_chain_tile(ctx, core, current_reads(ctx), p0, nt, ctx->slots[slot].chain_parallel_ok, ctx->d_active, rb0, 0))) return rc;
        const size_t np = (size_t)nt * 4, o = (size_t)p0 * 4;
        HIPCHK(ctx, hipMemcpyAsync(out_chains + o * CM_BESTCHAINLIM, ctx->rec[0].chains, np * CM_BESTCHAINLIM * sizeof(cm_chain), hipMemcpyDeviceToHost,
                                   ctx->st.B));
        HIPCHK(ctx, hipMemcpyAsync(out_nchain + o, ctx->rec[0].nchain, np * 4, hipMemcpyDeviceToHost, ctx->st.B));
        HIPCHK(ctx, hipMemcpyAsync(out_high + o, ctx->rec[0].high, np * 4, hipMemcpyDeviceToHost, ctx->st.B));
        HIPCHK(ctx, hipStreamSynchronize(ctx->st.B));
    }
    return check_dev_err(ctx);
}

extern "C" int cm_dp_probe_run(hipStream_t so, const cm_params *P, const uint8_t *arena, uint64_t arena_len, const cm_dp_req *req, uint32_t n_req,
                               int str_cap, uint32_t lds_fill, int arrangement, uint32_t grid, cm_dp_res *out, char *err, size_t err_cap);
int cm_dp_batch(cm_ctx *ctx, const cm_params *P, const uint8_t *arena, uint64_t arena_len, const cm_dp_req *req, uint32_t n_req, int str_cap,
                uint32_t lds_fill, int arrangement, uint32_t grid, cm_dp_res *out) {
    if (!ctx) return CM_EINVAL;
    HIPCHK(ctx, hipSetDevice(ctx->P.device));
    char msg[256] = "";
    const int rc = cm_dp_probe_run(ctx->st.B, P, arena, arena_len, req, n_req, str_cap, lds_fill, arrangement, grid, out, msg, sizeof msg);
    return rc == CM_OK ? CM_OK : fail(ctx, rc, "cm_dp_batch: %s", msg);
}

extern "C" int cm_annot_probe_run(hipStream_t so, const cm_params *P, const void *annot, size_t annot_bytes, const cm_annot_req *req, uint32_t n_req,
                                  cm_annot_res *out, uint32_t *out_tids, char *err, size_t err_cap);
int cm_annot_batch(cm_ctx *ctx, int slot, const cm_params *P, const cm_annot_req *req, uint32_t n_req, cm_annot_res *out, uint32_t *out_tids) {
    if (!ctx) return CM_EINVAL;
    if (slot < 0 || slot >= MAX_SLOTS) return fail(ctx, CM_EINVAL, "slot %d out of range", slot);
    if (!ctx->slots[slot].has_annot) return fail(ctx, CM_ESTATE, "annotation of slot %d not loaded", slot);
    HIPCHK(ctx, hipSetDevice(ctx->P.device));
    char msg[256] = "";
    const int rc = cm_annot_probe_run(ctx->st.B, P, &ctx->slots[slot].A, sizeof(cmc::AnnotDev), req, n_req, out, out_tids, msg, sizeof msg);
    return rc == CM_OK ? CM_OK : fail(ctx, rc, "cm_annot_batch: %s", msg);
}

int cm_debug_counters(cm_ctx *ctx, unsigned long long *out) {
    if (!ctx || !out) return CM_EINVAL;
    HIPCHK(ctx, hipSetDevice(ctx->P.device));
    HIPCHK(ctx, hipMemcpyAsync(out, ctx->d_counters, CN_WORDS * sizeof(unsigned long long), hipMemcpyDeviceToHost, ctx->st.B));
    HIPCHK(ctx, hipStreamSynchronize(ctx->st.B));
    return CM_OK;
}

int cm_debug_lane_clk(cm_ctx *ctx, unsigned long long *out) {
    if (!ctx || !out || !ctx->d_lane_clk) return CM_EINVAL;
#if defined(CM_DIAG)
    HIPCHK(ctx, hipMemcpy(out, ctx->d_lane_clk, ctx->n_pairs * 8 * 33, hipMemcpyDeviceToHost));
#else
    HIPCHK(ctx, hipMemcpy(out, ctx->d_lane_clk, ctx->n_pairs * 8, hipMemcpyDeviceToHost));
#endif
    return CM_OK;
}

int cm_prof_enable(cm_ctx *ctx, int on) {
    if (!ctx) return CM_EINVAL;
    ctx->prof = on != 0;
    return CM_OK;
}

int cm_prof_reset(cm_ctx *ctx) {
    if (!ctx) return CM_EINVAL;
    HIPCHK(ctx, hipSetDevice(ctx->P.device));
    HIPCHK(ctx, hipStreamSynchronize(ctx->st.B));
    for (auto &r : ctx->recs) {
        ctx->ev_free.push_back(r.a);
        ctx->ev_free.push_back(r.b);
    }
    ctx->recs.clear();
    for (int i = 0; i < PC_COUNT; ++i) {
        ctx->ms[i] = 0;
        ctx->launches[i] = 0;
    }
    HIPCHK(ctx, hipMemsetAsync(ctx->d_counters, 0, CN_WORDS * sizeof(unsigned long long), ctx->st.B));
    HIPCHK(ctx, hipStreamSynchronize(ctx->st.B));
    return CM_OK;
}

int cm_prof_get(cm_ctx *ctx, double ms[8], uint64_t launches[8]) {
    if (!ctx || !ms || !launches) return CM_EINVAL;
    HIPCHK(ctx, hipSetDevice(ctx->P.device));
    HIPCHK(ctx, hipStreamSynchronize(ctx->st.B));
    for (auto &r : ctx->recs) {
        float t = 0;
        if (hipEventElapsedTime(&t, r.a, r.b) == hipSuccess) ctx->ms[r.cls] += (double)t;
        ctx->ev_free.push_back(r.a);
        ctx->ev_free.push_back(r.b);
    }
    ctx->recs.clear();
    for (int i = 0; i < PC_COUNT; ++i) {
        ms[i] = ctx->ms[i];
        launches[i] = ctx->launches[i];
    }
    return CM_OK;
}

int cm_prof_counters(cm_ctx *ctx, uint64_t c[8]) {
    if (!ctx || !c) return CM_EINVAL;
    HIPCHK(ctx, hipSetDevice(ctx->P.device));
    unsigned long long h[8] = {0, 0, 0, 0, 0, 0, 0, 0};
    HIPCHK(ctx, hipMemcpyAsync(h, ctx->d_counters, sizeof h, hipMemcpyDeviceToHost, ctx->st.B));
    HIPCHK(ctx, hipStreamSynchronize(ctx->st.B));
    for (int i = 0; i < 8; ++i) c[i] = h[i];
    c[CN_DEAD_CHAINS] = 0;
    return CM_OK;
}

}
```

### circminer_amd/lib.py

```python
from __future__ import annotations

import ctypes as C
import os

import numpy as np

HERE = os.path.dirname(os.path.abspath(__file__))
LIB_PATH = os.environ.get("CM_LIB") or os.path.join(HERE, "csrc", "libcmhot.so")

CM_BESTCHAINLIM = 30
CM_MAX_CHAIN_FRAGS = 16
CM_CONTIG_SIZE = 1_100_000_000

CAT = dict(CONCRD=0, DISCRD=1, CHIORF=2, CHIBSJ=3, CHI2BSJ=4, CONGEN=5, CHIFUS=6, CONGNM=7, OEA2=8,
           CANDID=9, OEANCH=10, ORPHAN=11, NOPROC_MANYHIT=12, NOPROC_NOMATCH=13)

u8p, u16p, u32p, u64p, i32p = (C.POINTER(t) for t in (C.c_uint8, C.c_uint16, C.c_uint32, C.c_uint64, C.c_int32))


class Params(C.Structure):
    _fields_ = [(n, C.c_int32) for n in ("kmer", "seed_lim", "max_read_len", "scan_level", "max_ed", "max_sc", "band",
                                         "max_tlen", "max_intron", "max_chain_len", "device", "reserved")]


# ... 114 lines not shown
class Reads(C.Structure):
    _fields_ = [("n_pairs", C.c_uint64), ("seq1", u8p), ("off1", u64p), ("seq2", u8p), ("off2", u64p)]


class ChrInfo(C.Structure):
    _fields_ = [("name", C.c_char_p), ("contig_id", C.c_uint32), ("start_pos", C.c_uint32), ("len", C.c_uint32)]


class FastqBatch(C.Structure):
    _fields_ = [("reads", Reads), ("qual1", u8p), ("qual2", u8p), ("names1", C.c_void_p), ("names2", C.c_void_p),
                ("name_off1", u64p), ("name_off2", u64p), ("prior", C.c_void_p)]


def ptr(a: np.ndarray, t):
    return a.ctypes.data_as(t)


class ReadBatch:

    def __init__(self, seq1: np.ndarray, seq2: np.ndarray, len1=None, len2=None):
        if seq1.ndim == 2:
            n, L1 = seq1.shape
            L2 = seq2.shape[1]
            self.off1 = (np.arange(n + 1, dtype=np.uint64) * L1)
            self.off2 = (np.arange(n + 1, dtype=np.uint64) * L2)
            self.seq1 = np.ascontiguousarray(seq1, dtype=np.uint8).reshape(-1)
            self.seq2 = np.ascontiguousarray(seq2, dtype=np.uint8).reshape(-1)
        else:
            self.seq1 = np.ascontiguousarray(seq1, dtype=np.uint8)
            self.seq2 = np.ascontiguousarray(seq2, dtype=np.uint8)
            self.off1 = np.concatenate([[0], np.cumsum(len1)]).astype(np.uint64)
            self.off2 = np.concatenate([[0], np.cumsum(len2)]).astype(np.uint64)
            n = len(self.off1) - 1
        if self.seq1.size == 0:
            self.seq1 = np.zeros(1, np.uint8)
        if self.seq2.size == 0:
            self.seq2 = np.zeros(1, np.uint8)
        self.n = int(n)
        self.c = Reads(self.n, ptr(self.seq1, u8p), ptr(self.off1, u64p), ptr(self.seq2, u8p), ptr(self.off2, u64p))

    def max_len(self) -> int:
        if self.n == 0:
            return 0
        return int(max(np.diff(self.off1).max(), np.diff(self.off2).max()))


_lib = None


RELEASE_HOOK = C.CFUNCTYPE(None, C.c_void_p, C.c_void_p, C.c_uint64)


vp = C.c_void_p
pp = C.POINTER
SIGNATURES = {
    "cm_create": (C.c_int, [pp(Params), pp(vp)]),
    "cm_destroy": (None, [vp]),
    "cm_last_error": (C.c_char_p, [vp]),
    "cm_load_contig": (C.c_int, [vp, C.c_int, pp(IndexView)]),
    "cm_load_annotation": (C.c_int, [vp, C.c_int, pp(AnnotView)]),
    "cm_load_contig_raw": (C.c_int, [vp, C.c_int, pp(IndexRaw)]),
    "cm_host_next_contig_raw": (C.c_int, [vp, C.c_int, pp(IndexRaw), pp(C.c_int)]),
    "cm_build_contig": (C.c_int, [vp, C.c_int, C.c_int32, u8p, C.c_uint32, pp(BuildStats)]),
    "cm_index_download": (C.c_int, [vp, C.c_int, vp, vp, vp, C.c_uint64, pp(C.c_uint64)]),
    "cm_unload_contig": (C.c_int, [vp, C.c_int]),
    "cm_reads_upload": (C.c_int, [vp, pp(Reads), vp]),
    "cm_reads_stage": (C.c_int, [vp, pp(Reads), vp]),
    "cm_reads_swap": (C.c_int, [vp]),
    "cm_reads_stage_text": (C.c_int, [vp, vp, C.c_uint64, vp, C.c_uint64, C.c_uint64, C.c_uint32, vp, vp, pp(TextBatch)]),
    "cm_reads_peek": (C.c_int, [vp, vp, C.c_uint64, vp, vp, C.c_uint64, vp, pp(C.c_uint64)]),
    "cm_fastq_next_text": (C.c_int, [vp, C.c_uint64, pp(vp), pp(C.c_uint64), pp(C.c_int), pp(vp), pp(C.c_uint64), pp(C.c_int)]),
    "cm_fastq_text_consumed": (C.c_int, [vp, C.c_uint64, C.c_uint64]),
    "cm_write_remain_text": (C.c_int, [vp, vp, vp, vp, vp, vp, C.c_uint64]),
    "cm_format_pam": (C.c_int, [vp, pp(ChrInfo), C.c_uint32, C.c_uint64, C.c_uint64, vp, C.c_uint64, pp(C.c_uint64), pp(C.c_uint64)]),
    "cm_format_sam": (C.c_int, [vp, pp(ChrInfo), C.c_uint32, C.c_uint64, C.c_uint64, vp, C.c_uint64, pp(C.c_uint64), pp(C.c_uint64)]),
    "cm_format_remain": (C.c_int, [vp, pp(ChrInfo), C.c_uint32, C.c_uint64, C.c_uint64, vp, C.c_uint64, vp, C.c_uint64, pp(C.c_uint64), vp, pp(C.c_uint64),
                                   pp(C.c_uint64)]),
    "cm_format_remain_sorted": (C.c_int, [vp, pp(ChrInfo), C.c_uint32, C.c_uint64, C.c_uint64, vp, C.c_uint64, vp, C.c_uint64, pp(C.c_uint64), vp, vp, vp,
                                          pp(C.c_uint64), pp(C.c_uint64)]),
    "cm_quals_peek": (C.c_int, [vp, vp, C.c_uint64, vp, C.c_uint64]),
    "cm_state_poke": (C.c_int, [vp, vp]),
    "cm_debug_lane_clk": (C.c_int, [vp, vp]),
    "cm_debug_counters": (C.c_int, [vp, vp]),
    "cm_write_bytes": (C.c_int, [vp, vp, C.c_uint64]),
    "cm_map_round": (C.c_int, [vp, C.c_int, C.c_int]),
    "cm_map_rounds": (C.c_int, [vp, i32p, C.c_int, C.c_int]),
    "cm_reads_download": (C.c_int, [vp, vp, vp, vp]),
    "cm_map_batch": (C.c_int, [vp, C.c_int, C.c_int, pp(Reads), vp, vp, vp]),
    "cm_sync": (C.c_int, [vp]),
    "cm_reads_reset": (C.c_int, [vp]),
    "cm_collect_active": (C.c_int, [vp, C.c_uint64, vp, vp, pp(C.c_uint64)]),
    "cm_collect_records": (C.c_int, [vp, C.c_uint64, C.c_uint64, vp, pp(C.c_uint64)]),
    "cm_collect_records_device": (C.c_int, [vp, C.c_uint64, C.c_uint64, vp, pp(C.c_uint64)]),
    "cm_host_alloc": (C.c_int, [vp, C.c_uint64, pp(vp)]),
    "cm_host_free": (C.c_int, [vp, vp]),
    "cm_host_register": (C.c_int, [vp, vp, C.c_uint64]),
    "cm_host_unregister": (C.c_int, [vp, vp]),
    "cm_type_histogram": (C.c_int, [vp, pp(C.c_uint64)]),
    "cm_seed_batch": (C.c_int, [vp, C.c_int, vp, vp, vp, C.c_uint32, pp(C.c_uint32)]),
    "cm_chain_batch": (C.c_int, [vp, C.c_int, vp, vp, vp]),
    "cm_dp_batch": (C.c_int, [vp, pp(Params), vp, C.c_uint64, vp, C.c_uint32, C.c_int, C.c_uint32, C.c_int, C.c_uint32, vp]),
    "cm_annot_batch": (C.c_int, [vp, C.c_int, pp(Params), vp, C.c_uint32, vp, vp]),
    "cm_prof_enable": (C.c_int, [vp, C.c_int]),
    "cm_prof_reset": (C.c_int, [vp]),
    "cm_prof_get": (C.c_int, [vp, pp(C.c_double), pp(C.c_uint64)]),
    "cm_prof_counters": (C.c_int, [vp, pp(C.c_uint64)]),
    "cm_host_build_index": (C.c_int, [u8p, C.c_uint32, C.c_int32, C.c_int32, C.c_int, pp(IndexView)]),
    "cm_host_free_index": (None, [pp(IndexView)]),
    "cm_host_index_stats": (C.c_int, [pp(IndexView), C.c_int32, C.c_int, pp(C.c_uint64)]),
    "cm_host_build_annotation": (C.c_int, [C.c_char_p, pp(ChrInfo), C.c_uint32, u32p, C.c_uint32, C.c_int32,
                                           pp(AnnotView)]),
    "cm_host_free_annotation": (None, [pp(AnnotView), C.c_uint32]),
    "cm_host_pack_genome": (C.c_int, [C.c_char_p, C.c_char_p, C.c_char_p, C.c_uint32]),
    "cm_host_read_index_info": (C.c_int, [C.c_char_p, pp(pp(ChrInfo)), pp(C.c_uint32)]),
    "cm_host_free_index_info": (None, [pp(ChrInfo), C.c_uint32]),
    "cm_host_write_index": (C.c_int, [C.c_char_p, C.c_char_p, C.c_int32, C.c_int, C.c_int]),
    "cm_host_open_index": (C.c_int, [C.c_char_p, pp(vp), pp(C.c_int32), pp(C.c_int32), pp(C.c_uint32)]),
    "cm_host_next_contig": (C.c_int, [vp, C.c_int, pp(IndexView), pp(C.c_int)]),
    "cm_host_next_contig_genome": (C.c_int, [vp, pp(IndexView), pp(C.c_int)]),
    "cm_host_free_loaded_contig": (None, [pp(IndexView)]),
    "cm_host_close_index": (None, [vp]),
    "cm_fastq_open": (C.c_int, [C.c_char_p, C.c_char_p, pp(ChrInfo), C.c_uint32, C.c_int32, pp(vp)]),
    "cm_fastq_open_shard": (C.c_int, [C.c_char_p, C.c_char_p, pp(ChrInfo), C.c_uint32, C.c_int32, C.c_int32, C.c_int32, C.c_int, pp(vp),
                                      pp(C.c_uint64), pp(C.c_uint64)]),
    "cm_merge_parts": (C.c_int, [C.c_char_p, C.c_int32, C.c_int32, C.c_int32]),
    "cm_fastq_next": (C.c_int, [vp, C.c_uint64, pp(FastqBatch)]),
    "cm_fastq_close": (None, [vp]),
    "cm_fastq_set_release_hook": (None, [vp, RELEASE_HOOK, vp]),
    "cm_writer_open": (C.c_int, [C.c_char_p, C.c_char_p, pp(ChrInfo), C.c_uint32, pp(vp)]),
    "cm_write_remain": (C.c_int, [vp, pp(FastqBatch), vp, vp, C.c_uint64]),
    "cm_write_remain_records": (C.c_int, [vp, pp(FastqBatch), vp, C.c_uint64]),
    "cm_write_pam": (C.c_int, [vp, pp(FastqBatch), vp, vp, C.c_uint64]),
    "cm_host_gene_overlap": (C.c_int, [pp(AnnotView), C.c_uint32, pp(u32p), pp(C.c_uint32)]),
    "cm_sort_remain": (C.c_int, [C.c_char_p, C.c_char_p]),
    "cm_remain_runs_open": (C.c_int, [C.c_char_p, C.c_char_p, pp(vp)]),
    "cm_remain_runs_add": (C.c_int, [vp, vp, vp, vp, vp, vp, C.c_uint64]),
    "cm_remain_runs_add_unsorted": (C.c_int, [vp, vp, C.c_uint64, vp, C.c_uint64]),
    "cm_remain_runs_finish": (C.c_int, [vp]),
    "cm_remain_runs_close": (None, [vp]),
    "cm_regional_table_build": (C.c_int, [vp, C.c_uint32, C.c_int32, C.c_int32, pp(u32p), pp(u32p)]),
    "cm_regional_table_free": (None, [u32p, u32p]),
    "cm_circ_report": (C.c_int, [pp(CircRes), C.c_uint64, C.c_char_p]),
    "cm_mapping_run": (C.c_int, [pp(MappingArgs), pp(MappingStats), C.c_char_p, C.c_uint64]),
    "cm_circ_call": (C.c_int, [pp(Params), C.c_int32, C.c_uint32, pp(IndexView), pp(AnnotView), pp(ChrInfo), C.c_uint32, pp(FastqBatch),
                               C.c_char_p, C.c_char_p, pp(CircStats)]),
    "cm_circ_run": (C.c_int, [pp(CircArgs), pp(CircStats), C.c_char_p, C.c_uint64]),
    "cm_write_sam_header": (C.c_int, [vp]),
    "cm_write_sam": (C.c_int, [vp, pp(FastqBatch), vp, vp, C.c_uint64]),
    "cm_writer_flush": (C.c_int, [vp]),
    "cm_writer_close": (None, [vp]),
    "cm_abi_sizes": (C.c_int, [pp(C.c_uint32), C.c_uint32]),
}
EXPORTED_SYMBOLS = sorted(SIGNATURES)
SIGNATURES_NUMBERED = {"cm_write_bytes2": (C.c_int, [vp, vp, C.c_uint64])}


def load(path: str = LIB_PATH) -> C.CDLL:
    global _lib
    if _lib is not None:
        return _lib
    if not os.path.exists(path):
        raise RuntimeError(f"{path} is missing: run `python -c 'import __graft_entry__ as g; g.build()'` "
                           "(the hot path is HIP-only; there is no CPU fallback)")
    L = C.CDLL(path)
    for name, (res, args) in list(SIGNATURES.items()) + list(SIGNATURES_NUMBERED.items()):
        fn = getattr(L, name)
# ... 671 lines not shown
```

### include/circminer_hot.h

```cpp
#ifndef CIRCMINER_HOT_H
#define CIRCMINER_HOT_H

#include <stddef.h>
#include <stdint.h>

#ifdef __cplusplus
extern "C" {
#endif

enum {
    CM_CONCRD = 0, CM_DISCRD = 1, CM_CHIORF = 2, CM_CHIBSJ = 3, CM_CHI2BSJ = 4, CM_CONGEN = 5,
    CM_CHIFUS = 6, CM_CONGNM = 7, CM_OEA2 = 8, CM_CANDID = 9, CM_OEANCH = 10, CM_ORPHAN = 11,
    CM_NOPROC_MANYHIT = 12, CM_NOPROC_NOMATCH = 13
};

enum {
    CM_OK = 0,
    CM_EINVAL = -1,
    CM_ENODEV = -2,
    CM_ENOMEM = -3,
    CM_EHIP = -4,
    CM_ESTATE = -5,
    CM_ELIMIT = -6,
    CM_EIO = -7
// ... 104 lines not shown
    uint32_t reserved;
    uint64_t buckets_by_path[3];
    double ms_device;
} cm_build_stats;
int cm_build_contig(cm_ctx *ctx, int slot, int32_t contig_num, const uint8_t *genome, uint32_t ref_len,
                    cm_build_stats *stats );
int cm_index_download(cm_ctx *ctx, int slot, uint32_t *bucket_off, uint16_t *checksum, uint32_t *pos,
                      uint64_t cap_entries, uint64_t *n_entries);
int cm_unload_contig(cm_ctx *ctx, int slot);

int cm_reads_upload(cm_ctx *ctx, const cm_reads *reads, const cm_mapped_read *prior);

int cm_reads_stage(cm_ctx *ctx, const cm_reads *reads, const cm_mapped_read *prior);
int cm_reads_swap(cm_ctx *ctx);

typedef struct cm_text_batch {
    uint64_t n_pairs;
    uint64_t used1, used2;
    int32_t  max_len;
    int32_t  reserved;
} cm_text_batch;
int cm_reads_stage_text(cm_ctx *ctx, const uint8_t *text1, uint64_t len1, const uint8_t *text2, uint64_t len2,
                        uint64_t max_pairs, uint32_t flags, uint64_t *rec1, uint64_t *rec2, cm_text_batch *out);

int cm_map_round(cm_ctx *ctx, int slot, int is_last_round);

int cm_map_rounds(cm_ctx *ctx, const int *slots, int n_rounds, int last_is_final);

int cm_reads_download(cm_ctx *ctx, cm_mapped_read *out_state, int32_t *out_category, uint8_t *out_active);

int cm_map_batch(cm_ctx *ctx, int slot, int is_last_round, const cm_reads *reads,
                 const cm_mapped_read *prior, cm_mapped_read *out_state, int32_t *out_category);

int cm_sync(cm_ctx *ctx);

int cm_reads_reset(cm_ctx *ctx);

int cm_collect_active(cm_ctx *ctx, uint64_t cap, uint64_t *out_idx, cm_mapped_read *out_state, uint64_t *out_n);
typedef struct cm_record {
    uint64_t pair;
    cm_mapped_read state;
} cm_record;
int cm_collect_records(cm_ctx *ctx, uint64_t index_base, uint64_t cap, cm_record *out, uint64_t *out_n);
int cm_collect_records_device(cm_ctx *ctx, uint64_t index_base, uint64_t cap, void *d_out, uint64_t *out_n);

int cm_host_alloc(cm_ctx *ctx, uint64_t bytes, void **out);
int cm_host_register(cm_ctx *ctx, void *p, uint64_t bytes);
int cm_host_unregister(cm_ctx *ctx, void *p);
int cm_type_histogram(cm_ctx *ctx, uint64_t out[14]);
int cm_host_free(cm_ctx *ctx, void *p);

int cm_seed_batch(cm_ctx *ctx, int slot, uint32_t *out_start, uint32_t *out_cnt, uint32_t *out_raw,
                  uint32_t cap_probes, uint32_t *out_n_slots);
int cm_chain_batch(cm_ctx *ctx, int slot, cm_chain *out_chains, int32_t *out_nchain, int32_t *out_high);
typedef struct cm_dp_req {
    int32_t kind;
    int32_t s_off, s_step, s_mode, n;
    int32_t t_off, t_step, t_mode, m;
    int32_t arg;
} cm_dp_req;
typedef struct cm_dp_res {
    int32_t ret, sc_len, indel, score;
    int32_t err;
} cm_dp_res;
int cm_dp_batch(cm_ctx *ctx, const cm_params *P, const uint8_t *arena, uint64_t arena_len, const cm_dp_req *req, uint32_t n_req,
                int str_cap, uint32_t lds_fill, int arrangement, uint32_t grid, cm_dp_res *out);
typedef struct cm_annot_req {
    int32_t kind;
    uint32_t p0, p1, p2, p3;
    int32_t i0, i1, i2;
} cm_annot_req;
typedef struct cm_annot_res {
    int32_t ret, aux;
    uint32_t u0, u1;
} cm_annot_res;
int cm_annot_batch(cm_ctx *ctx, int slot, const cm_params *P, const cm_annot_req *req, uint32_t n_req, cm_annot_res *out, uint32_t *out_tids);

int cm_reads_peek(cm_ctx *ctx, uint8_t *seq1, uint64_t cap1, uint64_t *off1, uint8_t *seq2, uint64_t cap2, uint64_t *off2,
                  uint64_t *n_pairs);
int cm_quals_peek(cm_ctx *ctx, uint8_t *qual1, uint64_t cap1, uint8_t *qual2, uint64_t cap2);
int cm_state_poke(cm_ctx *ctx, const cm_mapped_read *states);
int cm_debug_lane_clk(cm_ctx *ctx, unsigned long long *out);
int cm_debug_counters(cm_ctx *ctx, unsigned long long *out);

int cm_prof_enable(cm_ctx *ctx, int on);
int cm_prof_reset(cm_ctx *ctx);
int cm_prof_get(cm_ctx *ctx, double ms[8], uint64_t launches[8]);
int cm_prof_counters(cm_ctx *ctx, uint64_t c[8]);

int cm_host_build_index(const uint8_t *genome, uint32_t ref_len, int32_t kmer, int32_t contig_num,
                        int n_threads, cm_index_view *out);
void cm_host_free_index(cm_index_view *iv);
int cm_host_index_stats(const cm_index_view *iv, int32_t seed_lim, int n_threads, uint64_t out[4]);

typedef struct cm_chr_info {
    const char *name;
    uint32_t contig_id;
    uint32_t start_pos;
    uint32_t len;
} cm_chr_info;
int cm_host_build_annotation(const char *gtf_path, const cm_chr_info *chrs, uint32_t n_chr,
                             const uint32_t *contig_len, uint32_t n_contigs, int32_t max_read_len,
                             cm_annot_view *out);
void cm_host_free_annotation(cm_annot_view *av, uint32_t n_contigs);
int cm_host_gene_overlap(const cm_annot_view *av, uint32_t pos, const uint32_t **genes, uint32_t *n_genes);

int cm_host_pack_genome(const char *fasta_path, const char *packed_fa_path, const char *index_info_path,
                        uint32_t contig_size);
int cm_host_read_index_info(const char *path, cm_chr_info **out, uint32_t *n);
void cm_host_free_index_info(cm_chr_info *chrs, uint32_t n);
int cm_host_write_index(const char *packed_fa_path, const char *index_path, int32_t kmer, int compact,
                        int n_threads);
typedef struct cm_index_file cm_index_file;
int cm_host_open_index(const char *index_path, cm_index_file **out, int32_t *kmer, int32_t *is_full,
                       uint32_t *n_records);
int cm_host_next_contig(cm_index_file *f, int n_threads, cm_index_view *out, int *loaded);
typedef struct cm_index_raw {
    int32_t contig_num;
    uint32_t ref_len;
    const uint8_t *genome;
    uint32_t n_buckets;
    const uint32_t *hv;
    const uint32_t *count14;
    const void *table;
    uint64_t table_slots;
} cm_index_raw;
int cm_host_next_contig_raw(cm_index_file *f, int n_threads, cm_index_raw *out, int *loaded);
int cm_host_next_contig_genome(cm_index_file *f, cm_index_view *out, int *loaded);
void cm_host_free_loaded_contig(cm_index_view *iv);
void cm_host_close_index(cm_index_file *f);

typedef struct cm_fastq_batch {
    cm_reads reads;
    const uint8_t *qual1, *qual2;
    const char *names1, *names2;
    const uint64_t *name_off1, *name_off2;
    const cm_mapped_read *prior;
} cm_fastq_batch;
typedef struct cm_fastq cm_fastq;
int cm_fastq_open(const char *r1_path, const char *r2_path, const cm_chr_info *chrs, uint32_t n_chr, int32_t max_ed,
                  cm_fastq **out);
int cm_fastq_open_shard(const char *r1_path, const char *r2_path, const cm_chr_info *chrs, uint32_t n_chr, int32_t max_ed,
                        int32_t rank, int32_t world, int n_threads, cm_fastq **out, uint64_t *first_pair, uint64_t *n_pairs);
int cm_fastq_next(cm_fastq *f, uint64_t max_pairs, cm_fastq_batch *out);
void cm_fastq_set_release_hook(cm_fastq *f, void (*fn)(void *user, const void *ptr, uint64_t bytes), void *user);
int cm_fastq_next_text(cm_fastq *f, uint64_t want_bytes, const uint8_t **text1, uint64_t *len1, int *eof1,
                       const uint8_t **text2, uint64_t *len2, int *eof2);
int cm_fastq_text_consumed(cm_fastq *f, uint64_t used1, uint64_t used2);
void cm_fastq_close(cm_fastq *f);

typedef struct cm_writer cm_writer;
int cm_writer_open(const char *path1, const char *path2, const cm_chr_info *chrs, uint32_t n_chr, cm_writer **out);
int cm_write_remain(cm_writer *w, const cm_fastq_batch *b, const cm_mapped_read *states, const uint64_t *sel, uint64_t n_sel);
int cm_write_remain_records(cm_writer *w, const cm_fastq_batch *batch, const cm_record *recs, uint64_t n);
int cm_write_remain_text(cm_writer *w, const uint8_t *text1, const uint64_t *rec1, const uint8_t *text2, const uint64_t *rec2,
                         const cm_record *recs, uint64_t n_rec);
int cm_write_pam(cm_writer *w, const cm_fastq_batch *b, const cm_mapped_read *states, const uint64_t *sel, uint64_t n_sel);
int cm_format_pam(cm_ctx *ctx, const cm_chr_info *chrs, uint32_t n_chr, uint64_t first, uint64_t count,
                  void *out, uint64_t cap, uint64_t *out_bytes, uint64_t stats[4] );
int cm_format_sam(cm_ctx *ctx, const cm_chr_info *chrs, uint32_t n_chr, uint64_t first, uint64_t count,
                  void *out, uint64_t cap, uint64_t *out_bytes, uint64_t stats[4] );
int cm_format_remain(cm_ctx *ctx, const cm_chr_info *chrs, uint32_t n_chr, uint64_t first, uint64_t count,
                     void *out1, uint64_t cap1, void *out2, uint64_t cap2, uint64_t out_bytes[2], int64_t *out_keys,
                     uint64_t *n_records, uint64_t stats[4] );
int cm_format_remain_sorted(cm_ctx *ctx, const cm_chr_info *chrs, uint32_t n_chr, uint64_t first, uint64_t count,
                            void *out1, uint64_t cap1, void *out2, uint64_t cap2, uint64_t out_bytes[2], int64_t *out_keys,
// ... 72 lines not shown
```

Before: 30.78 million.

## Publish scalar counters to pinned host memory from kernels instead of async D2H copies

Several small device-to-host hipMemcpyAsync calls are replaced. These covered the scan totals, heavy load, rerun and fall counts, and the pool-error flag. Kernels now write the values straight into mapped pinned host memory, using a last-block ticket (pin_last) plus system fences. The pool-lost check reads a host word that device code sets, instead of copying d_err back. The aim is to remove per-round copy commands and their queue latency, at the cost of extra ticket atomics, fences, and memsets, and it relies on system-scope visibility being correct.

```diff
diff --git a/circminer_amd/csrc/cm_core.h b/circminer_amd/csrc/cm_core.h
--- a/circminer_amd/csrc/cm_core.h
+++ b/circminer_amd/csrc/cm_core.h
@@ -416,6 +416,7 @@
     unsigned long long pool_bytes;
     CM_G unsigned long long *pool_cursor;
     g_err err;
+    CM_G unsigned long long *pool_lost = nullptr;
 };
 
 #if defined(__HIP_DEVICE_COMPILE__)
@@ -425,6 +426,10 @@
 inline unsigned long long pool_take(unsigned long long *cur, unsigned long long n) { return __sync_fetch_and_add(cur, n); }
 inline void flag_err(int *e, int bits) { __sync_fetch_and_or(e, bits); }
 #endif
+CM_HD inline void flag_pool_lost(ChainWork &w) {
+    flag_err(w.err, ERR_POOL);
+    if (w.pool_lost) *(volatile CM_G unsigned long long *)w.pool_lost = 1ull;
+}
 
 CM_HD inline bool check_junction(const Core &c, uint32_t s1, uint32_t s2, int ol, int kmer, int read_dist, int &trans_dist) {
     trans_dist = INF_I;
@@ -503,7 +508,7 @@
             const unsigned long long off = pool_take(w.pool_cursor, bytes);
             if (off + bytes > w.pool_bytes) {
                 lost = true;
-                flag_err(w.err, ERR_POOL);
+                flag_pool_lost(w);
             } else {
                 CM_G Event *ne = (CM_G Event *)(w.pool + off);
                 for (uint32_t q = 0; q < n_ev; ++q) ne[q] = ev[q];
diff --git a/circminer_amd/csrc/cm_heavy_pipe.h b/circminer_amd/csrc/cm_heavy_pipe.h
--- a/circminer_amd/csrc/cm_heavy_pipe.h
+++ b/circminer_amd/csrc/cm_heavy_pipe.h
@@ -531,7 +531,8 @@
 
 __global__ void __launch_bounds__(BLK_PAIR, 8) k_hp_finish(KCore kc, uint64_t pair0, const uint32_t *lst, const unsigned int *n_lst_p, const unsigned int *n_heavy_p,
                                                           int attempt, HPipe P, cm_mapped_read *state, uint8_t *active, int32_t *cat, int is_last,
-                                                          unsigned long long *counters, RetryArgs ra, const int32_t *nchain, int second_to_fall) {
+                                                          unsigned long long *counters, RetryArgs ra, const int32_t *nchain, int second_to_fall,
+                                                          PinLast fall_last) {
     const Core c = cmc::to_core(kc);
     const unsigned int n_items = attempt == 0 ? *n_heavy_p : *n_lst_p;
     const unsigned int x = blockIdx.x * BLK_PAIR + threadIdx.x;
@@ -606,6 +607,8 @@
             atomicAdd(&counters[CN_PAIR_ROUNDS], 1ull);
         }
     }
+    pin_last(P.fall_ctr, fall_last);
+    pin_last(ra.count, ra.last);
 }
 __global__ void k_hp_reset(unsigned int *ctr) {
     if (threadIdx.x < HC_WORDS && threadIdx.x != HC_LIST2 && threadIdx.x != HC_FALL) ctr[threadIdx.x] = 0u;
diff --git a/circminer_amd/csrc/cm_hot.hip b/circminer_amd/csrc/cm_hot.hip
--- a/circminer_amd/csrc/cm_hot.hip
+++ b/circminer_amd/csrc/cm_hot.hip
@@ -50,7 +50,8 @@
 enum Pin {
     PIN_COLLECT_N = 0, PIN_COLLECT_ERR = 1,
     PIN_DEV_ERR = 0,
-    PIN_POOL_ERR = 2,
+    PIN_POOL_LOST = 2,
+    PIN_POOL_SEEN = 3,
     PIN_HEAVY_LOAD = 4,
     PIN_CELLS = 8,
     PIN_RERUN_N = 12, PIN_FALL_N = 14,
@@ -66,6 +67,26 @@
     const uint8_t *seq1, *seq2;
     const uint64_t *off1, *off2;
 };
+
+__device__ inline void pin_store(unsigned long long *pin, unsigned long long v) {
+    *(volatile unsigned long long *)pin = v;
+    __threadfence_system();
+}
+struct PinLast {
+    unsigned int *ticket;
+    unsigned int n;
+    unsigned long long *pin;
+};
+template <class T>
+__device__ inline void pin_last(const T *count, const PinLast &pl) {
+    if (!pl.pin) return;
+    __syncthreads();
+    if (threadIdx.x != 0) return;
+    __threadfence();
+    if (atomicAdd(pl.ticket, 1u) + 1u != pl.n) return;
+    __threadfence();
+    pin_store(pl.pin, (unsigned long long)__hip_atomic_load(count, __ATOMIC_RELAXED, __HIP_MEMORY_SCOPE_AGENT));
+}
 
 __global__ void __launch_bounds__(BLK) k_seed(KCore kc, ReadsDev rd, const uint8_t *active, uint64_t pair0, uint32_t n_tile, int S,
                                               uint32_t *sstart, uint32_t *scnt, uint32_t *sraw, unsigned long long *counters) {
@@ -175,7 +196,7 @@
     }
 }
 template <class T, bool WITH_MAX>
-__global__ void __launch_bounds__(1024) k_scan_mid(T *bsum, uint32_t nb, T *total, const unsigned int *bmax) {
+__global__ void __launch_bounds__(1024) k_scan_mid(T *bsum, uint32_t nb, T *total, const unsigned int *bmax, unsigned long long *pin) {
     __shared__ T part[1024];
     __shared__ unsigned int gmax;
     const uint32_t t = threadIdx.x;
@@ -207,6 +228,10 @@
     if (WITH_MAX && t == 1023) {
         total[0] = part[1023];
         total[1] = gmax;
+        if (pin) {
+            *(volatile unsigned long long *)pin = (unsigned long long)part[1023];
+            pin_store(pin + 1, gmax);
+        }
     }
 }
 __global__ void __launch_bounds__(SCAN_T) k_scan_c(unsigned long long *out, const unsigned long long *bsum, uint32_t n) {
@@ -228,7 +253,7 @@
                                                      int32_t *dp_prev, uint8_t *pool, unsigned long long pool_bytes,
                                                      unsigned long long *pool_cursor, cm_chain *chains, int32_t *nchain, int32_t *high, int *err,
                                                      uint16_t *resid, const uint32_t *perm, const unsigned int *perm_lo, const unsigned int *perm_hi,
-                                                     const int8_t *cls) {
+                                                     const int8_t *cls, unsigned long long *pool_lost) {
     uint32_t r = r0 + blockIdx.x * BLK_CHAIN + threadIdx.x;
     if (perm) {
         r += *perm_lo;
@@ -255,6 +280,7 @@
         w.pool_bytes = pool_bytes;
         w.pool_cursor = (CM_G unsigned long long *)pool_cursor;
         w.err = (cmc::g_err)err;
+        w.pool_lost = (CM_G unsigned long long *)pool_lost;
         n = cmc::chain_kbest(c, len, S, st, cn, w, (CM_G cm_chain *)(chains + (uint64_t)r * CM_BESTCHAINLIM));
         if (n > 0) {
             const cm_chain &b = chains[(uint64_t)r * CM_BESTCHAINLIM];
@@ -273,6 +299,7 @@
     cmc::MemoSpill *spill;
     int spill_cap;
     int first;
+    PinLast last;
 };
 
 template <bool FIRST>
@@ -363,6 +390,7 @@
     if (lane_clk) lane_clk[slot] = ((wall_clock64() - it0) & 0xFFFFFFFFull) | ((unsigned long long)t << 32);
 #endif
     }
+    if (FIRST) pin_last(ra.count, ra.last);
 }
 
 
@@ -565,7 +593,7 @@
                                                     const unsigned long long *celloff, double *dp_score, int32_t *dp_prev, uint8_t *pool,
                                                     unsigned long long pool_bytes, unsigned long long *pool_cursor, cm_chain *chains, int32_t *nchain,
                                                     int *err, uint16_t *resid, const uint32_t *perm, const unsigned int *n_perm, unsigned int *next_problem,
-                                                    unsigned long long *counters) {
+                                                    unsigned long long *counters, unsigned long long *pool_lost) {
     extern __shared__ uint32_t lds_words[];
     CM_L uint32_t *LP = (CM_L uint32_t *)lds_words;
     __shared__ HeavyBackTrack BT;
@@ -728,7 +756,10 @@
                     o = ((unsigned long long)__shfl((unsigned int)(o >> 32), 0) << 32) | (unsigned long long)__shfl((unsigned int)o, 0);
                     if (o + bytes > pool_bytes) {
                         lost = true;
-                        if (lane == 0) atomicOr(err, cmc::ERR_POOL);
+                        if (lane == 0) {
+                            atomicOr(err, cmc::ERR_POOL);
+                            if (pool_lost) *(volatile unsigned long long *)pool_lost = 1ull;
+                        }
                     } else {
                         CM_G cmc::Event *ne = (CM_G cmc::Event *)((CM_G uint8_t *)pool + o);
                         for (uint32_t q = lane; q < n_ev; q += 64) ne[q] = ev[q];
@@ -1072,7 +1103,7 @@
 constexpr int HEAVY_COST_WIDE = 16;
 constexpr unsigned long long HEAVY_LOAD = 16;
 __global__ void __launch_bounds__(BLK) k_pair_cost(const int32_t *nchain, const uint8_t *active, uint64_t pair0, uint32_t n_tile, int base_cost,
-                                                  unsigned long long *sum) {
+                                                  unsigned long long *sum, PinLast last) {
     __shared__ unsigned long long sh[BLK / 64];
     const uint32_t t = blockIdx.x * BLK + threadIdx.x;
     unsigned long long v = 0;
@@ -1090,6 +1121,7 @@
         for (int w = 0; w < BLK / 64; ++w) s2 += sh[w];
         if (s2) atomicAdd(sum, s2);
     }
+    pin_last(sum, last);
 }
 __global__ void __launch_bounds__(BLK) k_pair_cls(KCore kc, const cm_chain *chains, const uint16_t *resid, const int32_t *nchain,
                                                  const uint8_t *active, uint64_t pair0, uint32_t n_tile, int8_t *cls, int32_t *cat, int heavy_cost,
@@ -1606,6 +1638,7 @@
     if (dbg_rows && lane == 0)
         for (int i = 0; i < 64; ++i) dbg_rows[(size_t)blockIdx.x * 64 + i] = tick_w[1 + i];
 #endif
+    pin_last(ra.count, ra.last);
 }
 
 #include "cm_heavy_pipe.h"
@@ -2256,6 +2289,7 @@
     BatchBuf<uint8_t> d_ones;
     uint64_t ones_cap = 0;
     unsigned long long *h_pin = nullptr;
+    unsigned long long *d_pin = nullptr;
     uint32_t h_pin_nt = 0;
     std::string err = "";
     Slot slots[MAX_SLOTS];
@@ -2509,10 +2543,10 @@
         const uint32_t nb = (n_prob + SCAN_ELEMS - 1) / SCAN_ELEMS;
         launch(ctx, PC_SCAN, k_scan_a, dim3(nb), dim3(SCAN_T), 0, st, sb.scnt, S, n_prob, sb.celloff, sb.bsum, sb.bmax, skip_dead ? 1 : 0);
         ctx->seed[s].skip_dead = skip_dead;
-        launch(ctx, PC_SCAN, k_scan_mid<unsigned long long, true>, dim3(1), dim3(1024), 0, st, sb.bsum, nb, sb.celloff + n_prob, sb.bmax);
+        launch(ctx, PC_SCAN, k_scan_mid<unsigned long long, true>, dim3(1), dim3(1024), 0, st, sb.bsum, nb, sb.celloff + n_prob, sb.bmax,
+               ctx->d_pin + PIN_CELLS + 2 * s);
         launch(ctx, PC_SCAN, k_scan_c, dim3((n_prob + SCAN_T - 1) / SCAN_T), dim3(SCAN_T), 0, st, sb.celloff, sb.bsum, n_prob);
     }
-    HIPCHK(ctx, hipMemcpyAsync(ctx->h_pin + PIN_CELLS + 2 * s, sb.celloff + n_prob, 2 * sizeof(unsigned long long), hipMemcpyDeviceToHost, st));
     if (rb) {
         const int rc = seed_classes(ctx, pair0, n_tile, act, s, st, rb, skip_dead, defer_rb);
         if (rc) return rc;
@@ -2585,7 +2619,7 @@
             const uint32_t hb = n < 8192u ? n : 8192u;
             launch(ctx, PC_CHAIN_HEAVY, k_chain_heavy, dim3(hb), dim3(64), heavy_lds, ctx->st.B2, core, rd, pair0, S, sb.sstart, sb.scnt, sb.celloff,
                    ctx->dp.score, ctx->dp.prev, ctx->dp.pool, ctx->dp.pool_bytes, ctx->pool_cursor(s), rb.chains, rb.nchain, ctx->d_err, rb.resid, sb.perm4,
-                   sb.cctr + CTR_BASE + CHAIN_LIGHT_CLS - 1, sb.cctr + CTR_CHAIN_NEXT, ctx->d_counters);
+                   sb.cctr + CTR_BASE + CHAIN_LIGHT_CLS - 1, sb.cctr + CTR_CHAIN_NEXT, ctx->d_counters, ctx->d_pin + PIN_POOL_LOST);
             }
             HIPCHK(ctx, hipEventRecord(ctx->ev.join, ctx->st.B2));
         }
@@ -2593,17 +2627,18 @@
         launch(ctx, PC_CHAIN, k_chain, dim3((n + BLK_CHAIN - 1) / BLK_CHAIN), dim3(BLK_CHAIN), 0, ctx->st.B, core, rd, act, pair0, a, b, S, sb.sstart, sb.scnt,
                sb.sraw, sb.celloff, base, ctx->dp.score, ctx->dp.prev, ctx->dp.pool, ctx->dp.pool_bytes, ctx->pool_cursor(s), rb.chains, rb.nchain, rb.high,
                ctx->d_err, rb.resid, use_split ? sb.perm4 : (const uint32_t *)nullptr, sb.cctr + CTR_BASE + CHAIN_LIGHT_CLS - 1, sb.cctr + CTR_SUM,
-               sb.skip_dead ? (const int8_t *)sb.cls4 : (const int8_t *)nullptr);
+               sb.skip_dead ? (const int8_t *)sb.cls4 : (const int8_t *)nullptr, ctx->d_pin + PIN_POOL_LOST);
         if (use_split) HIPCHK(ctx, hipStreamWaitEvent(ctx->st.B, ctx->ev.join, 0));
         HIPCHK(ctx, hipGetLastError());
         return CM_OK;
     };
     auto pool_lost = [&](bool *lost) -> int {
-        HIPCHK(ctx, hipMemcpyAsync(ctx->h_pin + PIN_POOL_ERR, ctx->d_err, sizeof(int), hipMemcpyDeviceToHost, ctx->st.B));
         HIPCHK(ctx, hipStreamSynchronize(ctx->st.B));
-        const int e = *(const int *)(ctx->h_pin + PIN_POOL_ERR);
-        *lost = (e & cmc::ERR_POOL) != 0;
+        volatile unsigned long long *word = ctx->h_pin + PIN_POOL_LOST;
+        *lost = *word != 0ull;
         if (*lost) {
+            *word = 0ull;
+            ++ctx->h_pin[PIN_POOL_SEEN];
             hipLaunchKernelGGL(k_err_clear, dim3(1), dim3(64), 0, ctx->st.B, ctx->d_err, (int)cmc::ERR_POOL);
             HIPCHK(ctx, hipStreamSynchronize(ctx->st.B));
         }
@@ -2715,6 +2750,10 @@
         return CM_ENOMEM;
     }
     memset(ctx->h_pin, 0, PIN_BYTES);
+    if (hipHostGetDevicePointer((void **)&ctx->d_pin, ctx->h_pin, 0) != hipSuccess) {
+        cm_destroy(ctx);
+        return CM_EHIP;
+    }
     (void)hipMemsetAsync(ctx->d_err, 0, sizeof(int), ctx->st.B);
     (void)hipMemsetAsync(ctx->d_counters, 0, CN_WORDS * sizeof(unsigned long long), ctx->st.B);
     if (hwq_low) {
@@ -2830,7 +2869,8 @@
     const uint32_t nb = (uint32_t)((n + S32_B - 1) / S32_B);
     if (nb == 0) return CM_OK;
     hipLaunchKernelGGL(k_scan32_a, dim3(nb), dim3(S32_T), 0, st, in, n, out, tmp, add, inclusive);
-    hipLaunchKernelGGL((k_scan_mid<uint32_t, false>), dim3(1), dim3(1024), 0, st, tmp, nb, (uint32_t *)nullptr, (const unsigned int *)nullptr);
+    hipLaunchKernelGGL((k_scan_mid<uint32_t, false>), dim3(1), dim3(1024), 0, st, tmp, nb, (uint32_t *)nullptr, (const unsigned int *)nullptr,
+                       (unsigned long long *)nullptr);
     hipLaunchKernelGGL(k_scan32_c, dim3(nb), dim3(S32_T), 0, st, out, n, (const uint32_t *)tmp);
     HIPCHK(ctx, hipGetLastError());
     return CM_OK;
@@ -3283,7 +3323,7 @@
         HIPCHK(ctx, ensure(ctx, ctx->hp.pairs, (size_t)tile * sizeof(HPair)));
         HIPCHK(ctx, ensure(ctx, ctx->hp.list2, (size_t)tile * 4));
         HIPCHK(ctx, ensure(ctx, pm.hp_fall, (size_t)tile * 4 * 2));
-        HIPCHK(ctx, ensure(ctx, pm.hp_fallctr, 2 * sizeof(unsigned int)));
+        HIPCHK(ctx, ensure(ctx, pm.hp_fallctr, 4 * sizeof(unsigned int)));
         HIPCHK(ctx, ensure(ctx, ctx->hp.T, tc * sizeof(HTask)));
         HIPCHK(ctx, ensure(ctx, ctx->hp.tcls, tc));
         HIPCHK(ctx, ensure(ctx, ctx->hp.tperm, tc * 4));
@@ -3304,8 +3344,8 @@
         if (pm.pair_err != before) HIPCHK(ctx, hipMemsetAsync(pm.pair_err, 0, (size_t)tile * 4 * 2, ctx->st.P));
     }
     HIPCHK(ctx, ensure(ctx, pm.retry_list, (size_t)tile * 4 * 2));
-    HIPCHK(ctx, ensure(ctx, pm.retry_ctr, 4 * sizeof(unsigned int)));
-    HIPCHK(ctx, ensure(ctx, ctx->d_heavy_load, sizeof(unsigned long long)));
+    HIPCHK(ctx, ensure(ctx, pm.retry_ctr, 8 * sizeof(unsigned int)));
+    HIPCHK(ctx, ensure(ctx, ctx->d_heavy_load, 2 * sizeof(unsigned long long)));
     HIPCHK(ctx, ensure(ctx, ctx->d_spill, (size_t)RETRY_GRID * BLK_PAIR * RETRY_SPILL * sizeof(cmc::MemoSpill)));
     HIPCHK(ctx, ensure(ctx, pm.cls_ctr, 2 * CTR_WORDS * sizeof(unsigned int)));
     HIPCHK(ctx, ensure(ctx, ctx->sort.ctr2, CTR_WORDS * sizeof(unsigned int)));
@@ -3336,8 +3376,8 @@
     for (int b = 0; b < 2; ++b) {
         const size_t at = (size_t)b * tile;
         ctx->pset[b] = PairSet{pm.perm + at,       pm.hlist + at,      pm.cls_ctr + (size_t)b * CTR_WORDS,
-                               pm.pair_err + at,   pm.retry_list + at, pm.retry_ctr + 2 * b,
-                               pm.hp_fall ? pm.hp_fall + at : nullptr, pm.hp_fallctr ? pm.hp_fallctr + b : nullptr};
+                               pm.pair_err + at,   pm.retry_list + at, pm.retry_ctr + 4 * b,
+                               pm.hp_fall ? pm.hp_fall + at : nullptr, pm.hp_fallctr ? pm.hp_fallctr + 2 * b : nullptr};
     }
     return CM_OK;
 }
@@ -3677,9 +3717,10 @@
         unsigned long long *load = nullptr;
         if (!fixed_cost) {
             load = ctx->d_heavy_load;
-            HIPCHK(ctx, hipMemsetAsync(load, 0, sizeof(unsigned long long), so));
-            launch(ctx, PC_NONE, k_pair_cost, dim3((nt + BLK - 1) / BLK), dim3(BLK), 0, so, rb.nchain, act_in, p0, nt, HEAVY_COST, load);
-            HIPCHK(ctx, hipMemcpyAsync((void *)(ctx->h_pin + PIN_HEAVY_LOAD), load, sizeof(unsigned long long), hipMemcpyDeviceToHost, so));
+            HIPCHK(ctx, hipMemsetAsync(load, 0, 2 * sizeof(unsigned long long), so));
+            const unsigned cost_grid = (nt + BLK - 1) / BLK;
+            launch(ctx, PC_NONE, k_pair_cost, dim3(cost_grid), dim3(BLK), 0, so, rb.nchain, act_in, p0, nt, HEAVY_COST, load,
+                   PinLast{(unsigned int *)(load + 1), cost_grid, ctx->d_pin + PIN_HEAVY_LOAD});
             ctx->h_pin_nt = nt;
         }
         launch(ctx, PC_ORDER, k_pair_cls, dim3((nt + BLK - 1) / BLK), dim3(BLK), 0, so, core, rb.chains, rb.resid, rb.nchain, act_in, p0, nt, ctx->sort.cls, ctx->d_cat,
@@ -3690,11 +3731,24 @@
         counting_sort(ctx, PC_ORDER, {so, w.cls, nt, w.blk_cnt, nbk, cls_ctr, perm, N_CLS, hlist, 1 << HEAVY_CLS, w.perm1, w.ctr2 + CTR_SUM});
     }
     HIPCHK(ctx, hipMemsetAsync(cls_ctr + CTR_NEXT, 0, 2 * sizeof(unsigned int), so));
-    HIPCHK(ctx, hipMemsetAsync(retry_ctr, 0, 2 * sizeof(unsigned int), so));
+    HIPCHK(ctx, hipMemsetAsync(retry_ctr, 0, 3 * sizeof(unsigned int), so));
     HIPCHK(ctx, hipEventRecord(ctx->ev.order[b], so));
     HIPCHK(ctx, hipStreamWaitEvent(sp, ctx->ev.prep[b], 0));
     HIPCHK(ctx, hipStreamWaitEvent(sp, ctx->ev.order[b], 0));
+    const bool pipeline = heavy_pipeline() && ctx->P.band == 3;
+    const unsigned cap = 256u * 4u * slots_per_simd;
+    const volatile unsigned long long *seen = (const volatile unsigned long long *)(ctx->h_pin + PIN_HEAVY_LOAD);
+    const bool loaded_run = ctx->h_pin_nt && *seen > HEAVY_LOAD * (unsigned long long)ctx->h_pin_nt;
+    const unsigned heavy_cap = cap / (loaded_run ? 1u : 2u);
+    const unsigned heavy_lim = std::min(heavy_cap, HEAVY_GRID_MAX);
+    const unsigned heavy_grid = nt < heavy_lim ? (nt ? nt : 1u) : heavy_lim;
+    constexpr unsigned pipe_grid = 2048u;
+    const unsigned light_want = (nt + BLK_PAIR - 1) / BLK_PAIR, light_cap = pipeline ? 2048u
+                                                                                   : cap;
+    const unsigned light_grid = light_want < light_cap ? light_want : light_cap;
     const RetryArgs ra1{pair_err, ps.retry_list, retry_ctr, nullptr, 0, 1};
+    const RetryArgs ra_last{pair_err, ps.retry_list, retry_ctr, nullptr, 0, 1,
+                            PinLast{retry_ctr + 2, light_grid + (pipeline ? pipe_grid : heavy_grid), ctx->d_pin + PIN_RERUN_N + b}};
     {
         cm_ctx::Rerun &q = ctx->rerun[b];
         q.core = core; q.rd = rd; q.p0 = p0; q.nt = nt;
@@ -3706,20 +3760,13 @@
     HIPCHK(ctx, hipStreamWaitEvent(sp2, ctx->ev.order[b], 0));
     {
         Timer t(ctx, PC_HEAVY, sp2);
-        const unsigned cap = 256u * 4u * slots_per_simd;
-        const volatile unsigned long long *seen = (const volatile unsigned long long *)(ctx->h_pin + PIN_HEAVY_LOAD);
-        const bool loaded_run = ctx->h_pin_nt && *seen > HEAVY_LOAD * (unsigned long long)ctx->h_pin_nt;
-        const unsigned heavy_cap = cap / (loaded_run ? 1u : 2u);
-        const unsigned heavy_lim = std::min(heavy_cap, HEAVY_GRID_MAX);
-        const unsigned heavy_grid = nt < heavy_lim ? (nt ? nt : 1u) : heavy_lim;
-        if (heavy_pipeline() && ctx->P.band == 3) {
+        if (pipeline) {
             const HPipe hp{ctx->hp.pairs, ctx->hp.list2, ps.hp_fall, ctx->hp.T, ctx->hp.pre, ctx->hp.q, ctx->hp.res, ctx->hp.U, ctx->hp.pre2,
                            ctx->hp.q2, ctx->hp.ctr, ctx->hp.tasks_cap, ctx->hp.unp_cap, ps.hp_fallctr, ctx->hp.tcls};
             const unsigned int *n_heavy = cls_ctr + HEAVY_CLS, *n_list2 = ctx->hp.ctr + HC_LIST2;
-            constexpr unsigned pipe_grid = 2048u;
             const size_t lds_slots = HG * sizeof(HSlot);
             HIPCHK(ctx, hipMemsetAsync(ctx->hp.ctr, 0, HC_WORDS * sizeof(unsigned int), sp2));
-            HIPCHK(ctx, hipMemsetAsync(ps.hp_fallctr, 0, sizeof(unsigned int), sp2));
+            HIPCHK(ctx, hipMemsetAsync(ps.hp_fallctr, 0, 2 * sizeof(unsigned int), sp2));
             const dim3 g(pipe_grid), wg(BLK_PAIR);
             static const bool task_order = !(getenv("CM_HP_TASK_ORDER") && getenv("CM_HP_TASK_ORDER")[0] == '0');
             static const int n_attempts = (getenv("CM_HP_ATTEMPTS") && atoi(getenv("CM_HP_ATTEMPTS")) == 1) ? 1 : 2;
@@ -3742,10 +3789,11 @@
                 launch(ctx, PC_HEAVY, k_hp_unp_req, g, wg, 0, sp2, core, rd, p0, attempt, rb.chains, hp, str_cap);
                 launch(ctx, PC_HEAVY, k_hp_dp, g, wg, lds_bytes, sp2, core, rd, p0, attempt, hp, 1, str_cap);
                 launch(ctx, PC_HEAVY, k_hp_unp, g, wg, lds_bytes, sp2, core, rd, p0, attempt, rb.chains, hp, pair_err, str_cap);
-                launch(ctx, PC_HEAVY, k_hp_finish, g, wg, 0, sp2, core, p0, ctx->hp.list2, n_list2, n_heavy, attempt, hp, ctx->d_state, act_out, ctx->d_cat, is_last_round, ctx->d_counters, ra1,
-                     rb.nchain, n_attempts == 1 ? 1 : 0);
+                const bool last = attempt == n_attempts - 1;
+                launch(ctx, PC_HEAVY, k_hp_finish, g, wg, 0, sp2, core, p0, ctx->hp.list2, n_list2, n_heavy, attempt, hp, ctx->d_state, act_out, ctx->d_cat, is_last_round, ctx->d_counters,
+                       last ? ra_last : ra1, rb.nchain, n_attempts == 1 ? 1 : 0,
+                       last ? PinLast{ps.hp_fallctr + 1, pipe_grid, ctx->d_pin + PIN_FALL_N + b} : PinLast{});
             }
-            HIPCHK(ctx, hipMemcpyAsync((void *)(ctx->h_pin + PIN_FALL_N + b), ps.hp_fallctr, sizeof(unsigned int), hipMemcpyDeviceToHost, sp2));
             {
                 cm_ctx::Rerun &q = ctx->rerun[b];
                 q.fall = true;
@@ -3761,19 +3809,16 @@
         } else {
             launch(ctx, PC_HEAVY, k_pair_heavy, dim3(heavy_grid), dim3(BLK_PAIR), lds_heavy, sp2, core, rd, p0, hlist, cls_ctr + HEAVY_CLS, rb.chains, rb.nchain, rb.high,
                    ctx->d_state, act_out, ctx->d_cat, is_last_round, ctx->d_err, ctx->d_counters, str_cap,
-                   ctx->d_lane_clk ? ctx->d_lane_clk + (size_t)nt * 16 + (size_t)(nt / 64 + 1) * 64 : nullptr, ctx->d_hres, cls_ctr + CTR_NEXT + 1, ra1);
+                   ctx->d_lane_clk ? ctx->d_lane_clk + (size_t)nt * 16 + (size_t)(nt / 64 + 1) * 64 : nullptr, ctx->d_hres, cls_ctr + CTR_NEXT + 1, ra_last);
         }
     }
     HIPCHK(ctx, hipEventRecord(ctx->ev.join_p, sp2));
     {
         Timer t(ctx, PC_PAIR, sp);
-        const unsigned want = (nt + BLK_PAIR - 1) / BLK_PAIR, cap = (heavy_pipeline() && ctx->P.band == 3) ? 2048u
-                                                                                                           : 256u * 4u * slots_per_simd;
-        launch(ctx, PC_PAIR, k_pair, dim3(want < cap ? want : cap), dim3(BLK_PAIR), lds_bytes, sp, core, rd, p0, nt, rb.chains, rb.nchain, rb.high, ctx->d_state,
-               act_out, ctx->d_cat, is_last_round, ctx->d_err, ctx->d_counters, str_cap, ctx->d_lane_clk, perm, cls_ctr + CTR_SUM, cls_ctr + CTR_NEXT, ra1);
+        launch(ctx, PC_PAIR, k_pair, dim3(light_grid), dim3(BLK_PAIR), lds_bytes, sp, core, rd, p0, nt, rb.chains, rb.nchain, rb.high, ctx->d_state,
+               act_out, ctx->d_cat, is_last_round, ctx->d_err, ctx->d_counters, str_cap, ctx->d_lane_clk, perm, cls_ctr + CTR_SUM, cls_ctr + CTR_NEXT, ra_last);
         HIPCHK(ctx, hipStreamWaitEvent(sp, ctx->ev.join_p, 0));
     }
-    HIPCHK(ctx, hipMemcpyAsync((void *)(ctx->h_pin + PIN_RERUN_N + b), retry_ctr, sizeof(unsigned int), hipMemcpyDeviceToHost, sp));
     HIPCHK(ctx, hipEventRecord(ctx->ev.first[b], sp));
     ctx->rerun[b].deferred = defer;
     if (!defer) {
@@ -4499,6 +4544,14 @@
     return CM_OK;
 }
 
+int cm_debug_pin(cm_ctx *ctx, unsigned long long *out) {
+    if (!ctx || !out) return CM_EINVAL;
+    HIPCHK(ctx, hipSetDevice(ctx->P.device));
+    HIPCHK(ctx, hipStreamSynchronize(ctx->st.B));
+    for (int i = 0; i < PIN_WORDS; ++i) out[i] = ((const volatile unsigned long long *)ctx->h_pin)[i];
+    return CM_OK;
+}
+
 int cm_debug_lane_clk(cm_ctx *ctx, unsigned long long *out) {
     if (!ctx || !out || !ctx->d_lane_clk) return CM_EINVAL;
 #if defined(CM_DIAG)
diff --git a/circminer_amd/lib.py b/circminer_amd/lib.py
--- a/circminer_amd/lib.py
+++ b/circminer_amd/lib.py
@@ -220,6 +220,7 @@
     "cm_state_poke": (C.c_int, [vp, vp]),
     "cm_debug_lane_clk": (C.c_int, [vp, vp]),
     "cm_debug_counters": (C.c_int, [vp, vp]),
+    "cm_debug_pin": (C.c_int, [vp, vp]),
     "cm_write_bytes": (C.c_int, [vp, vp, C.c_uint64]),
     "cm_map_round": (C.c_int, [vp, C.c_int, C.c_int]),
     "cm_map_rounds": (C.c_int, [vp, i32p, C.c_int, C.c_int]),
diff --git a/include/circminer_hot.h b/include/circminer_hot.h
--- a/include/circminer_hot.h
+++ b/include/circminer_hot.h
@@ -210,6 +210,7 @@
 int cm_state_poke(cm_ctx *ctx, const cm_mapped_read *states);
 int cm_debug_lane_clk(cm_ctx *ctx, unsigned long long *out);
 int cm_debug_counters(cm_ctx *ctx, unsigned long long *out);
+int cm_debug_pin(cm_ctx *ctx, unsigned long long *out);
 
 int cm_prof_enable(cm_ctx *ctx, int on);
 int cm_prof_reset(cm_ctx *ctx);
```

New measurement: 30.26 million. -1.7%, worse.
